# facebookresearch/multipathnet

Hardware: NVIDIA H100
Metric: proposals/sec (higher is better)
Workload: dtype fp32 (wgmma split emulation, fp32 accumulate: 3 bf16 products per MAC, 2 fp16 products in fc6/fc7)

## Files before the change

### include/mpn_abi.h

```cpp
#ifndef MPN_ABI_H
#define MPN_ABI_H
#include <stdint.h>
#ifdef __cplusplus
extern "C" {
#endif

typedef struct mpn_ctx mpn_ctx;
typedef struct mpn_model mpn_model;

int mpn_ctx_create(int device, void *cuda_stream, mpn_ctx **out);
int mpn_ctx_create_stream(int device, int priority, mpn_ctx **out);
void *mpn_ctx_stream(const mpn_ctx *ctx);
int mpn_ctx_wait_ctx(mpn_ctx *ctx, mpn_ctx *other);
void mpn_ctx_destroy(mpn_ctx *ctx);
const char *mpn_last_error(const mpn_ctx *ctx);
int mpn_ctx_synchronize(mpn_ctx *ctx);
int64_t mpn_ctx_launch_count(const mpn_ctx *ctx);
const char *mpn_version(void);
int mpn_ctx_set_option(mpn_ctx *ctx, const char *name, int64_t value);
int mpn_ctx_profile_begin(mpn_ctx *ctx);
int mpn_ctx_profile_end(mpn_ctx *ctx, double *ms_by_cat, int64_t *launches_by_cat);
int mpn_ctx_timeline_begin(mpn_ctx *ctx, int32_t max_launches);
int mpn_ctx_timeline_end(mpn_ctx *ctx, uint64_t *stamps_min, uint64_t *stamps_max, int32_t *n_launches);

int mpn_nms(mpn_ctx *ctx, const float *scored_boxes, int64_t N, float thr,
            int32_t *keep_idx, int64_t *n_keep);
int mpn_nms_batched(mpn_ctx *ctx, const float *scored_boxes, const int64_t *seg_offsets,
                    int64_t nseg, float thr, int32_t *keep_idx, int64_t *keep_counts);
int mpn_nms_batched_dev(mpn_ctx *ctx, const float *scored_boxes_dev, const int64_t *seg_offsets,
                        int64_t nseg, float thr, int32_t *keep_idx_dev, int32_t *keep_counts_dev);
int mpn_nms_dense(mpn_ctx *ctx, const float *scored_boxes, int64_t N, float thr,
                  int32_t *pick_idx, int64_t *n_pick);
int mpn_bbox_vote(mpn_ctx *ctx, const float *nms_boxes, int64_t K, const float *scored_boxes,
                  int64_t N, float thr, float *res);

int mpn_foveal(mpn_ctx *ctx, const float *rois, int64_t R, float *out);
int mpn_context_region(mpn_ctx *ctx, const float *rois, int64_t R, float scale, float *out);
int mpn_bbox_norm(mpn_ctx *ctx, float *deltas, int64_t R, int64_t C4, const float *mean4,
                  const float *std4);
int mpn_foveal_dev(mpn_ctx *ctx, const float *rois_dev, int64_t R, float *out_dev);
int mpn_context_region_dev(mpn_ctx *ctx, const float *rois_dev, int64_t R, float scale, float *out_dev);
int mpn_bbox_norm_dev(mpn_ctx *ctx, float *deltas_dev, int64_t R, int64_t C4, const float *mean4,
                      const float *std4);
int mpn_bbox_decode(mpn_ctx *ctx, const float *deltas, const float *boxes, int64_t R, int64_t C,
                    float *out);

int mpn_roi_pool(mpn_ctx *ctx, const float *fmap, int64_t N, int64_t C, int64_t H, int64_t W,
                 const float *rois, int64_t R, int32_t PW, int32_t PH, float spatial_scale,
                 int32_t variant, float *out, int32_t *argmax);
int mpn_roi_pool_dev(mpn_ctx *ctx, const float *fmap_dev, int64_t N, int64_t C, int64_t H,
                     int64_t W, const float *rois_dev, int64_t R, int32_t PW, int32_t PH,
                     float spatial_scale, int32_t variant, float *out_dev, int32_t *argmax_dev);
int mpn_roi_pool_backward(mpn_ctx *ctx, const float *grad_out, const int32_t *argmax, int64_t N,
                          int64_t C, int64_t H, int64_t W, const float *rois, int64_t R, int32_t PW,
                          int32_t PH, float spatial_scale, int32_t variant, float *grad_data);
int mpn_roi_pool_backward_dev(mpn_ctx *ctx, const float *grad_out_dev, const int32_t *argmax_dev,
                              int64_t N, int64_t C, int64_t H, int64_t W, const float *rois_dev,
                              int64_t R, int32_t PW, int32_t PH, float spatial_scale, int32_t variant,
                              float *grad_data_dev);

enum {
  MPN_LAYER_CONV = 1,
  MPN_LAYER_MAXPOOL = 2,
  MPN_LAYER_AVGPOOL = 3,
  MPN_LAYER_FLATTEN = 4
};
typedef struct mpn_layer {
  int32_t kind;
  int32_t in_slot, out_slot;
  int32_t cin, cout, kh, kw, stride, pad;
  int32_t relu;
  int32_t residual_slot;
  int32_t ceil_mode;
  int32_t weight, bias;
} mpn_layer;

typedef struct mpn_tower {
  int32_t region;
  int32_t n_levels;
  int32_t level_slot[3];
  float   level_scale[3];
  int32_t pooled_w, pooled_h;
  int32_t normalize;
  int32_t n_layers;
  int32_t first_layer;
  int32_t out_slot;
} mpn_tower;

typedef struct mpn_head {
  int32_t col_begin, col_len;
  int32_t cout;
  int32_t weight, bias;
} mpn_head;

typedef struct mpn_model_desc {
  int32_t n_trunk_layers;  const mpn_layer *trunk_layers;
  int32_t n_towers;        const mpn_tower *towers;
  int32_t n_tower_layers;  const mpn_layer *tower_layers;
  int32_t n_cls_heads;     const mpn_head *cls_heads;
  mpn_head bbox_head;
  int32_t num_classes;
  int32_t roi_variant;
  int32_t no_softmax;
  int32_t has_bbox_norm;
  float bbox_mean[4], bbox_std[4];
  int32_t max_rois;
  int32_t max_h, max_w;
} mpn_model_desc;

int mpn_model_create(mpn_ctx *ctx, const mpn_model_desc *desc, const float *const *weights,
                     const int64_t *n_elem, int32_t n_weights, mpn_model **out);
void mpn_model_destroy(mpn_model *m);

int mpn_model_trunk(mpn_model *m, const float *image, int32_t H, int32_t W);
int mpn_model_trunk_dev(mpn_model *m, const float *image_dev, int32_t H, int32_t W);
typedef struct mpn_image_transform {
  int32_t swap[3];
  float scale;
  float mean[3];
  float std[3];
  int32_t has_std;
} mpn_image_transform;
int mpn_get_images_size(int32_t H0, int32_t W0, double scale, double max_size, int32_t *h, int32_t *w, double *im_scale);
int mpn_get_images(mpn_ctx *ctx, const float *im, int32_t H0, int32_t W0, const mpn_image_transform *tf,
                   int32_t h, int32_t w, float *out);
int mpn_get_images_dev(mpn_ctx *ctx, const float *im_dev, int32_t H0, int32_t W0, const mpn_image_transform *tf,
                       int32_t h, int32_t w, float *out_dev);
int mpn_get_images_u8(mpn_ctx *ctx, const uint8_t *im_hwc, int32_t H0, int32_t W0, const mpn_image_transform *tf,
                      int32_t h, int32_t w, float *out);
int mpn_get_images_u8_dev(mpn_ctx *ctx, const uint8_t *im_hwc_dev, int32_t H0, int32_t W0, const mpn_image_transform *tf,
                          int32_t h, int32_t w, float *out_dev);
int mpn_get_images_u8_flip(mpn_ctx *ctx, const uint8_t *im_hwc, int32_t H0, int32_t W0, const mpn_image_transform *tf,
                           int32_t h, int32_t w, int32_t flip, float *out);
int mpn_get_images_u8_flip_dev(mpn_ctx *ctx, const uint8_t *im_hwc_dev, int32_t H0, int32_t W0, const mpn_image_transform *tf,
                               int32_t h, int32_t w, int32_t flip, float *out_dev);
int mpn_model_trunk_image(mpn_model *m, const float *im, int32_t H0, int32_t W0, const mpn_image_transform *tf,
                          double scale, double max_size, double *im_scale, int32_t *h, int32_t *w);
int mpn_model_heads(mpn_model *m, const float *rois, int64_t R, float *cls_out, float *bbox_out);
int mpn_model_heads_dev(mpn_model *m, const float *rois_dev, int64_t R, float *cls_out_dev,
                        float *bbox_out_dev);

int mpn_model_detect(mpn_model *m, const float *image, int32_t H, int32_t W, const float *boxes,
                     int64_t R, float im_scale, int32_t recompute_features, float *scores,
                     float *bboxes);
int mpn_model_detect_nms(mpn_model *m, const float *image, int32_t H, int32_t W,
                         const float *boxes, int64_t R, float im_scale, float W0, float H0,
                         float score_thresh, float nms_thr, float *scores, float *bboxes,
                         int32_t *keep_idx, int32_t *keep_counts);
int mpn_model_detect_nms_submit(mpn_model *m, const float *image, int32_t H, int32_t W,
                                const float *boxes, int64_t R, float im_scale, float W0, float H0,
                                float score_thresh, float nms_thr, float *scores, float *bboxes,
                                int32_t *keep_idx, int32_t *keep_counts, int32_t *ticket);
int mpn_model_detect_nms_submit_u8(mpn_model *m, const uint8_t *im_hwc, int32_t H0, int32_t W0,
                                   const mpn_image_transform *tf, double scale, double max_size, const float *boxes,
                                   int64_t R, float score_thresh, float nms_thr, float *scores, float *bboxes,
                                   int32_t *keep_idx, int32_t *keep_counts, int32_t *ticket);
int mpn_model_detect_nms_wait(mpn_model *m, int32_t ticket);
typedef struct mpn_test_opts {
  int32_t num_iter;
  int32_t use_rbox_scores;
  int32_t bbox_voting;
  float score_thresh;
  float nms_thr;
  float vote_thr;
  float vote_score_pow;
} mpn_test_opts;
int mpn_model_test_one(mpn_model *m, const float *image, int32_t H, int32_t W, const float *boxes, int64_t R,
                       float im_scale, float W0, float H0, const mpn_test_opts *opts, float *scores, float *bboxes,
                       int32_t *keep_idx, int32_t *keep_counts, float *voted);
int mpn_model_detect_nms_dev(mpn_model *m, const float *image_dev, int32_t H, int32_t W,
                             const float *boxes_dev, int64_t R, float im_scale, float W0, float H0,
                             float score_thresh, float nms_thr, float *scores_dev,
                             float *bboxes_dev, int32_t *keep_idx_dev, int32_t *keep_counts_dev);

int mpn_post_detect_dev(mpn_ctx *ctx, const float *scores_dev, const float *deltas_dev, const float *boxes_dev, int64_t R,
                        int32_t C, const float *mean4, const float *std4, float W0, float H0, float score_thresh,
                        float nms_thr, int32_t c_begin, int32_t c_end, float *bboxes_dev, int32_t *keep_idx_dev,
                        int32_t *keep_counts_dev);

enum { MPN_MAX_DET = 128, MPN_REC_FLOATS = 769, MPN_DIST_ID_BYTES = 128 };
int mpn_pack_detections_dev(mpn_ctx *ctx, const float *scores_dev, const float *bboxes_dev, int64_t R, int32_t C,
                            const int32_t *keep_idx_dev, const int32_t *keep_counts_dev, int64_t cap, int32_t top_k,
                            float *record_dev);
int mpn_pack_detections(mpn_ctx *ctx, const float *scores, const float *bboxes, int64_t R, int32_t C,
                        const int32_t *keep_idx, const int32_t *keep_counts, int64_t cap, int32_t top_k, float *record);
int mpn_select_boxes(mpn_ctx *ctx, const float *classes, const float *ys, int64_t R, int32_t C, const float *mean4,
                     const float *std4, float *out);
int mpn_select_boxes_dev(mpn_ctx *ctx, const float *classes_dev, const float *ys_dev, int64_t R, int32_t C,
                         const float *mean4, const float *std4, float *out_dev);
int mpn_model_set_detection_sink(mpn_model *m, float *records_dev, int64_t capacity, int32_t top_k);
int mpn_model_detection_sink_count(const mpn_model *m, int64_t *n_records);

int mpn_dist_unique_id(mpn_ctx *ctx, uint8_t *id);
int mpn_dist_init(mpn_ctx *ctx, const uint8_t *id, int32_t rank, int32_t world);
int mpn_dist_world(const mpn_ctx *ctx, int32_t *rank, int32_t *world);
int mpn_dist_all_gather_dev(mpn_ctx *ctx, const float *send_dev, int64_t n_floats, float *recv_dev);
int mpn_dist_all_gather(mpn_ctx *ctx, const float *send_dev, int64_t n_floats, float *recv_host);
int mpn_dist_destroy(mpn_ctx *ctx);
int mpn_dist_nccl_version(mpn_ctx *ctx, int32_t *version);

int mpn_coco_eval(mpn_ctx *ctx, int32_t n_images, const int64_t *image_ids, int32_t n_cats, const int64_t *cat_ids,
                  int64_t G, const int32_t *gt_img, const int32_t *gt_cat, const double *gt_box, const double *gt_area,
                  const int32_t *gt_crowd, int64_t D, const float *dets, double *precision, double *recall,
                  double *stats);

int mpn_model_get_pooled(mpn_model *m, int32_t tower, int64_t r0, int64_t n, float *out, int64_t capacity,
                         int64_t *R_total, int32_t *bins, int32_t *Ctot);
int mpn_model_get_trunk_slot(mpn_model *m, int32_t slot, float *out_nchw, int64_t capacity,
                             int32_t *C, int32_t *H, int32_t *W);
int mpn_model_get_slot_planes(mpn_model *m, int32_t tower, int32_t slot, int64_t r0, int64_t n, uint16_t *hi,
                              uint16_t *lo, uint8_t *q8, int32_t *e8, int64_t capacity, int32_t *fmt, int64_t *dims);
int mpn_model_get_head_outputs(mpn_model *m, float *cls_logits, float *bbox_raw, int64_t *R, int32_t *K);
int mpn_debug_detect_tail(mpn_ctx *ctx, const float *logits, int32_t K, int64_t R, int32_t C, int32_t do_softmax, const float *deltas,
                          const float *boxes, int32_t do_clamp, float W0, float H0, int32_t has_norm, const float *mean4,
                          const float *std4, float *scores, float *bboxes);
int mpn_model_set_conv_impl(mpn_model *m, int32_t impl);
int mpn_model_last_flops(const mpn_model *m, double *trunk_flops, double *head_flops);

int mpn_gemm_check(mpn_ctx *ctx, const float *A, const float *B, const float *bias, int64_t M,
                   int64_t N, int64_t K, int32_t relu, int32_t impl, float *C);
int mpn_gemm_bench(mpn_ctx *ctx, int64_t M, int64_t N, int64_t K, int32_t iters, double *ms_per_launch,
                   int32_t *bn, int32_t *cta_group, int32_t *splitk);
int mpn_conv_bench(mpn_ctx *ctx, int64_t N, int64_t Cin, int64_t H, int64_t W, int64_t Cout, int32_t k, int32_t stride,
                   int32_t pad, int32_t iters, double *ms_per_launch, int32_t *bn, int32_t *cta_group, int32_t *mode,
                   uint64_t *dbg16);
int mpn_debug_plan(int64_t N, int64_t Cin, int64_t H, int64_t W, int64_t Cout, int32_t k, int32_t stride, int32_t pad,
                   int32_t per_roi, int32_t sm_count, int32_t *out);
int mpn_debug_fp8(const float *h, int64_t n_samples, int64_t sample_elems, int32_t *e_out, uint8_t *q_out);
int mpn_conv_check(mpn_ctx *ctx, const float *x, int64_t N, int64_t Cin, int64_t H, int64_t W,
                   const float *w, const float *bias, int64_t Cout, int32_t kh, int32_t kw,
                   int32_t stride, int32_t pad, int32_t relu, int32_t impl, float *y);

typedef struct mpn_train_config {
  float lr, momentum, dampening, weight_decay;
  float dropout;
  float bbox_regression;
  uint64_t seed;
} mpn_train_config;
int mpn_train_check_fixed_bn(const mpn_model_desc *d, int32_t trunk_from, int32_t integral, int32_t n, const int32_t *weight,
                             char *msg, int32_t msg_cap);
int mpn_model_train_begin_fixed_bn(mpn_model *m, const mpn_train_config *cfg, int32_t trunk_from, int32_t integral, int32_t n,
                                   const int32_t *weight, const float *const *scale);
int mpn_train_check_desc(const mpn_model_desc *d, char *msg, int32_t msg_cap);
int mpn_train_check_trunk(const mpn_model_desc *d, int32_t trunk_from, char *msg, int32_t msg_cap);
int mpn_train_check_integral(const mpn_model_desc *d, int32_t trunk_from, char *msg, int32_t msg_cap);
int mpn_model_train_begin(mpn_model *m, const mpn_train_config *cfg);
int mpn_model_train_begin_trunk(mpn_model *m, const mpn_train_config *cfg, int32_t trunk_from);
int mpn_model_train_begin_integral(mpn_model *m, const mpn_train_config *cfg, int32_t trunk_from);
int mpn_model_train_step(mpn_model *m, int32_t n_images, const float *const *images, const int32_t *image_hw,
                         const int32_t *rois_per_image, const float *boxes, const int32_t *labels, const float *bbox_targets,
                         float *losses);
int mpn_model_train_step_dev(mpn_model *m, int32_t n_images, const float *const *images_dev, const int32_t *image_hw,
                             const int32_t *rois_per_image, const float *boxes_dev, const int32_t *labels_dev,
                             const float *bbox_targets_dev, float *losses_dev);
int mpn_model_train_phase_ms(mpn_model *m, float *ms);
int mpn_model_train_select_head(mpn_model *m, int32_t k);
int mpn_model_train_set_lr(mpn_model *m, float lr);
int mpn_model_train_decay(mpn_model *m, float factor);
int mpn_model_train_get(mpn_model *m, int32_t weight, int32_t what, float *out, int64_t capacity);
int mpn_model_train_dropout_mask(mpn_model *m, int32_t tower, int32_t layer, uint8_t *out, int64_t capacity, int64_t *n_out);
int mpn_model_train_relu_gate(mpn_model *m, int32_t tower, int32_t layer, uint8_t *out, int64_t capacity, int64_t *n_out);
int mpn_model_train_outputs(mpn_model *m, float *cls_logits, float *bbox_deltas);
int mpn_model_train_trunk_slot(mpn_model *m, int32_t image, int32_t slot, float *out_nchw, int64_t capacity, int32_t *C,
                               int32_t *H, int32_t *W);
int mpn_debug_roi_backward_nhwc(mpn_ctx *ctx, const uint16_t *hi, const uint16_t *lo, int32_t H, int32_t W, int32_t C, const float *rois,
                                int64_t R, int32_t PW, int32_t PH, float scale, int32_t variant, const float *grad_out, float *grad);
int mpn_debug_pool_backward(mpn_ctx *ctx, const uint16_t *y_hi, const uint16_t *y_lo, int32_t H, int32_t W, int32_t C, const float *grad_pool,
                            float *grad);
int mpn_debug_conv_backward(mpn_ctx *ctx, int32_t n_images, const int32_t *image_hw, int32_t cin, int32_t cout, int32_t k, int32_t stride,
                            const uint16_t *x_hi, const uint16_t *x_lo, const float *g, const float *w, float *dw, float *dx);
int mpn_model_train_end(mpn_model *m);
int mpn_debug_dropout(uint64_t seed, uint32_t step, int32_t tower, int32_t layer, uint64_t elem0, int64_t n, float p, uint8_t *out);
int mpn_debug_criteria(const float *x, const float *d, const int32_t *labels, const float *t, int64_t R, int32_t C, float bbox_w,
                       float *gx, float *gd, float *losses);
int mpn_debug_sgd(float *w, const float *g, float *buf, int64_t n, float lr, float momentum, float dampening, float wd, int32_t first);

typedef struct mpn_roidb mpn_roidb;
int mpn_roidb_create(mpn_ctx *ctx, int32_t n_images, const int64_t *ann_off, const double *ann_xywh, const double *ann_area,
                     const int32_t *ann_class, const int32_t *ann_flags, double min_area, const int64_t *prop_off,
                     const float *prop_box, const float *prop_score, int32_t best_number, double min_proposal_area,
                     int32_t num_classes, int32_t n_sets, const float *thresholds, mpn_roidb **out);
void mpn_roidb_destroy(mpn_roidb *db);
int mpn_roidb_counts(mpn_roidb *db, int32_t *counts, int64_t *n_rows);
int mpn_roidb_image_rows(mpn_roidb *db, int32_t image, float *boxes, float *overlap, int32_t *corr, int32_t *label, int64_t capacity,
                         int64_t *n_rows, int32_t *n_gt);
int mpn_roidb_list(mpn_roidb *db, int32_t set, int32_t kind, int32_t image, int32_t *rows, int64_t capacity, int64_t *n_out);
int mpn_roidb_regression_stats(mpn_roidb *db, int32_t set, int32_t n_first, float *mean, float *std_);
int mpn_sample_plan(const int32_t *n_bg, const int32_t *n_fg, int32_t n_images, uint64_t seed, uint32_t step, int32_t set, int32_t n_slots,
                    int32_t *image, int32_t *bg_src, int32_t *fg_src, int32_t *flip);
int mpn_integral_set(uint64_t seed, uint32_t step, int32_t n_sets, int32_t *set);
int mpn_train_images_size(int32_t H0, int32_t W0, double scale, double max_size, int32_t *h, int32_t *w, double *im_scale);
int mpn_roidb_sample_dev(mpn_roidb *db, int32_t set, uint64_t seed, uint32_t step, int32_t n_slots, const int32_t *bg_src,
                         const int32_t *fg_src, const int32_t *flip, const double *im_scale, const int32_t *width, int32_t bg_each,
                         int32_t fg_each, const float *mean, const float *std_, int32_t num_classes, float *boxes_dev,
                         int32_t *labels_dev, float *targets_dev, int32_t *rois_per_image);
int mpn_roidb_sample(mpn_roidb *db, int32_t set, uint64_t seed, uint32_t step, int32_t n_slots, const int32_t *plan,
                     const uint8_t *const *images_hwc, const int32_t *hw0, const mpn_image_transform *tf, double scale, double max_size,
                     int32_t bg_each, int32_t fg_each, const float *mean, const float *std_, int32_t num_classes, int32_t *image_hw,
                     int32_t *rois_per_image);
int mpn_roidb_batch_host(mpn_roidb *db, float *const *images, float *boxes, int32_t *labels, float *targets);
int mpn_model_train_step_batch(mpn_model *m, mpn_roidb *db, float *losses);
int mpn_debug_attach_proposals(int64_t n_ann, const double *ann_xywh, const double *ann_area, const int32_t *ann_class,
                               const int32_t *ann_flags, double min_area, int64_t n_prop, const float *prop_box, const float *prop_score,
                               int32_t best_number, double min_proposal_area, int32_t num_classes, float *boxes, float *overlap,
                               int32_t *corr, int32_t *label, int64_t capacity, int64_t *n_rows, int32_t *n_gt);
int mpn_debug_sample_rows(int64_t R, const float *rois, const float *gtboxes, const int32_t *labels, double im_scale, int32_t width,
                          int32_t flip, const float *mean, const float *std_, int32_t num_classes, float *boxes, float *targets);

int mpn_train_check_phase2(const mpn_model_desc *d, int32_t phase2_from, int32_t integral, char *msg, int32_t msg_cap);
int mpn_model_train_begin_phase2(mpn_model *m, const mpn_train_config *cfg, int32_t phase2_from, int32_t integral);
int mpn_model_train_phase2(mpn_model *m, float lr);

typedef struct mpn_train_state {
  int64_t step;
  float lr;
  int32_t head, last_head, phase2;
} mpn_train_state;
int mpn_model_train_set(mpn_model *m, int32_t weight, int32_t what, const float *src, int64_t n);
int mpn_model_train_get_state(mpn_model *m, mpn_train_state *out);
int mpn_model_train_set_state(mpn_model *m, const mpn_train_state *s);
int mpn_debug_roi_backward_jobs(mpn_ctx *ctx, const uint16_t *hi, const uint16_t *lo, int32_t H, int32_t W, int32_t C, const float *rois,
                                int64_t R, int32_t PW, int32_t PH, int32_t variant, int32_t n_jobs, const int32_t *region, const float *scale,
                                const int32_t *normalize, const int64_t *ld, const int32_t *ch_off, const float *const *grad_out, float *grad,
                                double *ab, int32_t *argmax);

#ifdef __cplusplus
}
#endif
#endif
```

### multipathnet_b200/_lib.py

```python
from __future__ import annotations

import ctypes as C
import os
from dataclasses import dataclass, field
from typing import List, Optional, Sequence

import numpy as np

_HERE = os.path.dirname(os.path.abspath(__file__))
LIB_PATH = os.path.join(_HERE, "libmpn_b200.so")
HEADER_PATH = os.path.join(os.path.dirname(_HERE), "include", "mpn_abi.h")

MPN_LAYER_CONV, MPN_LAYER_MAXPOOL, MPN_LAYER_AVGPOOL, MPN_LAYER_FLATTEN = 1, 2, 3, 4
MPN_MAX_DET, MPN_REC_FLOATS, MPN_DIST_ID_BYTES = 128, 769, 128
MPN_LAYER_LRN = 5


class MpnError(RuntimeError):
    pass


class CLayer(C.Structure):
    _fields_ = [(n, C.c_int32) for n in (
        "kind", "in_slot", "out_slot", "cin", "cout", "kh", "kw", "stride", "pad", "relu",
        "residual_slot", "ceil_mode", "weight", "bias")]


class CTower(C.Structure):
    _fields_ = [("region", C.c_int32), ("n_levels", C.c_int32), ("level_slot", C.c_int32 * 3),
                ("level_scale", C.c_float * 3), ("pooled_w", C.c_int32), ("pooled_h", C.c_int32),
                ("normalize", C.c_int32), ("n_layers", C.c_int32), ("first_layer", C.c_int32),
                ("out_slot", C.c_int32)]


class CHead(C.Structure):
    _fields_ = [(n, C.c_int32) for n in ("col_begin", "col_len", "cout", "weight", "bias")]


class CImageTransform(C.Structure):
    _fields_ = [("swap", C.c_int32 * 3), ("scale", C.c_float), ("mean", C.c_float * 3), ("std", C.c_float * 3), ("has_std", C.c_int32)]

    @staticmethod
    def of(kind: str) -> "CImageTransform":
        from . import workloads as wl
        t = CImageTransform()
        if kind == "ross":
            t.swap[:] = [3, 2, 1]; t.scale = 255.0; t.mean[:] = wl.ROSS_MEAN; t.std[:] = [1, 1, 1]; t.has_std = 0
        elif kind == "imagenet":
            t.swap[:] = [1, 2, 3]; t.scale = 1.0; t.mean[:] = wl.IMAGENET_MEAN; t.std[:] = wl.IMAGENET_STD; t.has_std = 1
        else:
            raise ValueError(f"unknown transformer {kind!r}")
        return t


class CTestOpts(C.Structure):
    _fields_ = [("num_iter", C.c_int32), ("use_rbox_scores", C.c_int32), ("bbox_voting", C.c_int32), ("score_thresh", C.c_float),
                ("nms_thr", C.c_float), ("vote_thr", C.c_float), ("vote_score_pow", C.c_float)]


class CModelDesc(C.Structure):
    _fields_ = [("n_trunk_layers", C.c_int32), ("trunk_layers", C.POINTER(CLayer)),
                ("n_towers", C.c_int32), ("towers", C.POINTER(CTower)),
                ("n_tower_layers", C.c_int32), ("tower_layers", C.POINTER(CLayer)),
                ("n_cls_heads", C.c_int32), ("cls_heads", C.POINTER(CHead)),
                ("bbox_head", CHead), ("num_classes", C.c_int32), ("roi_variant", C.c_int32),
                ("no_softmax", C.c_int32), ("has_bbox_norm", C.c_int32),
                ("bbox_mean", C.c_float * 4), ("bbox_std", C.c_float * 4),
                ("max_rois", C.c_int32), ("max_h", C.c_int32), ("max_w", C.c_int32)]


class CTrainConfig(C.Structure):
    _fields_ = [("lr", C.c_float), ("momentum", C.c_float), ("dampening", C.c_float), ("weight_decay", C.c_float),
                ("dropout", C.c_float), ("bbox_regression", C.c_float), ("seed", C.c_uint64)]


class CTrainState(C.Structure):
    _fields_ = [("step", C.c_int64), ("lr", C.c_float), ("head", C.c_int32), ("last_head", C.c_int32), ("phase2", C.c_int32)]


_f32p = C.POINTER(C.c_float)
_i32p = C.POINTER(C.c_int32)
_i64p = C.POINTER(C.c_int64)
_vp = C.c_void_p

SIGNATURES = {
    "mpn_ctx_create": (C.c_int, [C.c_int, _vp, C.POINTER(_vp)]),
    "mpn_ctx_create_stream": (C.c_int, [C.c_int, C.c_int, C.POINTER(_vp)]),
    "mpn_ctx_stream": (_vp, [_vp]),
    "mpn_ctx_wait_ctx": (C.c_int, [_vp, _vp]),
    "mpn_ctx_destroy": (None, [_vp]),
    "mpn_last_error": (C.c_char_p, [_vp]),
    "mpn_ctx_synchronize": (C.c_int, [_vp]),
    "mpn_ctx_launch_count": (C.c_int64, [_vp]),
    "mpn_version": (C.c_char_p, []),
    "mpn_ctx_set_option": (C.c_int, [_vp, C.c_char_p, C.c_int64]),
    "mpn_ctx_profile_begin": (C.c_int, [_vp]),
    "mpn_ctx_profile_end": (C.c_int, [_vp, C.POINTER(C.c_double), _i64p]),
    "mpn_ctx_timeline_begin": (C.c_int, [_vp, C.c_int32]),
    "mpn_ctx_timeline_end": (C.c_int, [_vp, C.POINTER(C.c_uint64), C.POINTER(C.c_uint64), _i32p]),
    "mpn_nms": (C.c_int, [_vp, _vp, C.c_int64, C.c_float, _vp, _i64p]),
    "mpn_nms_batched": (C.c_int, [_vp, _vp, _i64p, C.c_int64, C.c_float, _vp, _i64p]),
    "mpn_nms_batched_dev": (C.c_int, [_vp, _vp, _i64p, C.c_int64, C.c_float, _vp, _vp]),
    "mpn_nms_dense": (C.c_int, [_vp, _vp, C.c_int64, C.c_float, _vp, _i64p]),
    "mpn_bbox_vote": (C.c_int, [_vp, _vp, C.c_int64, _vp, C.c_int64, C.c_float, _vp]),
    "mpn_foveal": (C.c_int, [_vp, _vp, C.c_int64, _vp]),
    "mpn_context_region": (C.c_int, [_vp, _vp, C.c_int64, C.c_float, _vp]),
    "mpn_bbox_norm": (C.c_int, [_vp, _vp, C.c_int64, C.c_int64, _vp, _vp]),
    "mpn_foveal_dev": (C.c_int, [_vp, _vp, C.c_int64, _vp]),
    "mpn_context_region_dev": (C.c_int, [_vp, _vp, C.c_int64, C.c_float, _vp]),
    "mpn_bbox_norm_dev": (C.c_int, [_vp, _vp, C.c_int64, C.c_int64, _vp, _vp]),
    "mpn_bbox_decode": (C.c_int, [_vp, _vp, _vp, C.c_int64, C.c_int64, _vp]),
    "mpn_roi_pool": (C.c_int, [_vp, _vp, C.c_int64, C.c_int64, C.c_int64, C.c_int64, _vp, C.c_int64,
                               C.c_int32, C.c_int32, C.c_float, C.c_int32, _vp, _vp]),
    "mpn_roi_pool_dev": (C.c_int, [_vp, _vp, C.c_int64, C.c_int64, C.c_int64, C.c_int64, _vp, C.c_int64,
                                   C.c_int32, C.c_int32, C.c_float, C.c_int32, _vp, _vp]),
    "mpn_roi_pool_backward": (C.c_int, [_vp, _vp, _vp, C.c_int64, C.c_int64, C.c_int64, C.c_int64, _vp, C.c_int64,
                                        C.c_int32, C.c_int32, C.c_float, C.c_int32, _vp]),
    "mpn_roi_pool_backward_dev": (C.c_int, [_vp, _vp, _vp, C.c_int64, C.c_int64, C.c_int64, C.c_int64, _vp, C.c_int64,
                                            C.c_int32, C.c_int32, C.c_float, C.c_int32, _vp]),
    "mpn_get_images_size": (C.c_int, [C.c_int32, C.c_int32, C.c_double, C.c_double, _i32p, _i32p, C.POINTER(C.c_double)]),
    "mpn_get_images": (C.c_int, [_vp, _vp, C.c_int32, C.c_int32, _vp, C.c_int32, C.c_int32, _vp]),
    "mpn_get_images_dev": (C.c_int, [_vp, _vp, C.c_int32, C.c_int32, _vp, C.c_int32, C.c_int32, _vp]),
    "mpn_get_images_u8": (C.c_int, [_vp, _vp, C.c_int32, C.c_int32, _vp, C.c_int32, C.c_int32, _vp]),
    "mpn_get_images_u8_dev": (C.c_int, [_vp, _vp, C.c_int32, C.c_int32, _vp, C.c_int32, C.c_int32, _vp]),
    "mpn_get_images_u8_flip": (C.c_int, [_vp, _vp, C.c_int32, C.c_int32, _vp, C.c_int32, C.c_int32, C.c_int32, _vp]),
    "mpn_get_images_u8_flip_dev": (C.c_int, [_vp, _vp, C.c_int32, C.c_int32, _vp, C.c_int32, C.c_int32, C.c_int32, _vp]),
    "mpn_roidb_create": (C.c_int, [_vp, C.c_int32, _vp, _vp, _vp, _vp, _vp, C.c_double, _vp, _vp, _vp, C.c_int32, C.c_double,
                                   C.c_int32, C.c_int32, _vp, C.POINTER(_vp)]),
    "mpn_roidb_destroy": (None, [_vp]),
    "mpn_roidb_counts": (C.c_int, [_vp, _vp, _i64p]),
    "mpn_roidb_image_rows": (C.c_int, [_vp, C.c_int32, _vp, _vp, _vp, _vp, C.c_int64, _i64p, _i32p]),
    "mpn_roidb_list": (C.c_int, [_vp, C.c_int32, C.c_int32, C.c_int32, _vp, C.c_int64, _i64p]),
    "mpn_roidb_regression_stats": (C.c_int, [_vp, C.c_int32, C.c_int32, _vp, _vp]),
    "mpn_sample_plan": (C.c_int, [_vp, _vp, C.c_int32, C.c_uint64, C.c_uint32, C.c_int32, C.c_int32, _vp, _vp, _vp, _vp]),
    "mpn_integral_set": (C.c_int, [C.c_uint64, C.c_uint32, C.c_int32, _i32p]),
    "mpn_train_images_size": (C.c_int, [C.c_int32, C.c_int32, C.c_double, C.c_double, _i32p, _i32p, C.POINTER(C.c_double)]),
    "mpn_roidb_sample_dev": (C.c_int, [_vp, C.c_int32, C.c_uint64, C.c_uint32, C.c_int32, _vp, _vp, _vp, _vp, _vp, C.c_int32, C.c_int32,
                                       _vp, _vp, C.c_int32, _vp, _vp, _vp, _vp]),
    "mpn_roidb_sample": (C.c_int, [_vp, C.c_int32, C.c_uint64, C.c_uint32, C.c_int32, _vp, _vp, _vp, _vp, C.c_double, C.c_double,
                                   C.c_int32, C.c_int32, _vp, _vp, C.c_int32, _vp, _vp]),
    "mpn_roidb_batch_host": (C.c_int, [_vp, _vp, _vp, _vp, _vp]),
    "mpn_model_train_step_batch": (C.c_int, [_vp, _vp, _vp]),
    "mpn_debug_attach_proposals": (C.c_int, [C.c_int64, _vp, _vp, _vp, _vp, C.c_double, C.c_int64, _vp, _vp, C.c_int32, C.c_double,
                                             C.c_int32, _vp, _vp, _vp, _vp, C.c_int64, _i64p, _i32p]),
    "mpn_debug_sample_rows": (C.c_int, [C.c_int64, _vp, _vp, _vp, C.c_double, C.c_int32, C.c_int32, _vp, _vp, C.c_int32, _vp, _vp]),
    "mpn_model_detect_nms_submit_u8": (C.c_int, [_vp, _vp, C.c_int32, C.c_int32, _vp, C.c_double, C.c_double, _vp, C.c_int64, C.c_float, C.c_float,
                                                 _vp, _vp, _vp, _vp, _i32p]),
    "mpn_model_trunk_image": (C.c_int, [_vp, _vp, C.c_int32, C.c_int32, _vp, C.c_double, C.c_double, C.POINTER(C.c_double), _i32p, _i32p]),
    "mpn_model_create": (C.c_int, [_vp, C.POINTER(CModelDesc), C.POINTER(_vp), _i64p, C.c_int32, C.POINTER(_vp)]),
    "mpn_model_destroy": (None, [_vp]),
    "mpn_model_trunk": (C.c_int, [_vp, _vp, C.c_int32, C.c_int32]),
    "mpn_model_trunk_dev": (C.c_int, [_vp, _vp, C.c_int32, C.c_int32]),
    "mpn_model_heads": (C.c_int, [_vp, _vp, C.c_int64, _vp, _vp]),
    "mpn_model_heads_dev": (C.c_int, [_vp, _vp, C.c_int64, _vp, _vp]),
    "mpn_model_detect": (C.c_int, [_vp, _vp, C.c_int32, C.c_int32, _vp, C.c_int64, C.c_float, C.c_int32, _vp, _vp]),
    "mpn_model_detect_nms": (C.c_int, [_vp, _vp, C.c_int32, C.c_int32, _vp, C.c_int64, C.c_float, C.c_float,
                                       C.c_float, C.c_float, C.c_float, _vp, _vp, _vp, _vp]),
    "mpn_model_detect_nms_submit": (C.c_int, [_vp, _vp, C.c_int32, C.c_int32, _vp, C.c_int64, C.c_float, C.c_float,
                                              C.c_float, C.c_float, C.c_float, _vp, _vp, _vp, _vp, _i32p]),
    "mpn_model_detect_nms_wait": (C.c_int, [_vp, C.c_int32]),
    "mpn_model_test_one": (C.c_int, [_vp, _vp, C.c_int32, C.c_int32, _vp, C.c_int64, C.c_float, C.c_float, C.c_float, C.POINTER(CTestOpts),
                                     _vp, _vp, _vp, _vp, _vp]),
    "mpn_model_detect_nms_dev": (C.c_int, [_vp, _vp, C.c_int32, C.c_int32, _vp, C.c_int64, C.c_float, C.c_float,
                                           C.c_float, C.c_float, C.c_float, _vp, _vp, _vp, _vp]),
    "mpn_post_detect_dev": (C.c_int, [_vp, _vp, _vp, _vp, C.c_int64, C.c_int32, _vp, _vp, C.c_float, C.c_float, C.c_float, C.c_float,
                                      C.c_int32, C.c_int32, _vp, _vp, _vp]),
    "mpn_pack_detections_dev": (C.c_int, [_vp, _vp, _vp, C.c_int64, C.c_int32, _vp, _vp, C.c_int64, C.c_int32, _vp]),
    "mpn_pack_detections": (C.c_int, [_vp, _vp, _vp, C.c_int64, C.c_int32, _vp, _vp, C.c_int64, C.c_int32, _vp]),
    "mpn_select_boxes": (C.c_int, [_vp, _vp, _vp, C.c_int64, C.c_int32, _vp, _vp, _vp]),
    "mpn_select_boxes_dev": (C.c_int, [_vp, _vp, _vp, C.c_int64, C.c_int32, _vp, _vp, _vp]),
    "mpn_model_set_detection_sink": (C.c_int, [_vp, _vp, C.c_int64, C.c_int32]),
    "mpn_model_detection_sink_count": (C.c_int, [_vp, _i64p]),
    "mpn_dist_unique_id": (C.c_int, [_vp, _vp]),
    "mpn_dist_init": (C.c_int, [_vp, _vp, C.c_int32, C.c_int32]),
    "mpn_dist_world": (C.c_int, [_vp, _i32p, _i32p]),
    "mpn_dist_all_gather_dev": (C.c_int, [_vp, _vp, C.c_int64, _vp]),
    "mpn_dist_all_gather": (C.c_int, [_vp, _vp, C.c_int64, _vp]),
    "mpn_dist_destroy": (C.c_int, [_vp]),
    "mpn_dist_nccl_version": (C.c_int, [_vp, _i32p]),
    "mpn_coco_eval": (C.c_int, [_vp, C.c_int32, _vp, C.c_int32, _vp, C.c_int64, _vp, _vp, _vp, _vp, _vp, C.c_int64, _vp, _vp, _vp, _vp]),
    "mpn_model_get_pooled":(C.c_int, [_vp, C.c_int32, C.c_int64, C.c_int64, _vp, C.c_int64, _i64p, _i32p, _i32p]),
    "mpn_model_get_trunk_slot": (C.c_int, [_vp, C.c_int32, _vp, C.c_int64, _i32p, _i32p, _i32p]),
    "mpn_model_get_slot_planes": (C.c_int, [_vp, C.c_int32, C.c_int32, C.c_int64, C.c_int64, _vp, _vp, _vp, _vp, C.c_int64, _i32p, _i64p]),
    "mpn_model_get_head_outputs": (C.c_int, [_vp, _vp, _vp, _i64p, _i32p]),
    "mpn_debug_detect_tail": (C.c_int, [_vp, _vp, C.c_int32, C.c_int64, C.c_int32, C.c_int32, _vp, _vp, C.c_int32, C.c_float, C.c_float,
                                        C.c_int32, _vp, _vp, _vp, _vp]),
    "mpn_model_set_conv_impl": (C.c_int, [_vp, C.c_int32]),
    "mpn_model_last_flops": (C.c_int, [_vp, C.POINTER(C.c_double), C.POINTER(C.c_double)]),
    "mpn_gemm_bench": (C.c_int, [_vp, C.c_int64, C.c_int64, C.c_int64, C.c_int32, C.POINTER(C.c_double), _i32p, _i32p, _i32p]),
    "mpn_conv_bench": (C.c_int, [_vp, C.c_int64, C.c_int64, C.c_int64, C.c_int64, C.c_int64, C.c_int32, C.c_int32, C.c_int32, C.c_int32,
                                 C.POINTER(C.c_double), _i32p, _i32p, _i32p, C.POINTER(C.c_uint64)]),
    "mpn_debug_plan": (C.c_int, [C.c_int64, C.c_int64, C.c_int64, C.c_int64, C.c_int64, C.c_int32, C.c_int32, C.c_int32, C.c_int32, C.c_int32, _i32p]),
    "mpn_debug_fp8": (C.c_int, [_vp, C.c_int64, C.c_int64, _vp, _vp]),
    "mpn_gemm_check": (C.c_int, [_vp, _vp, _vp, _vp, C.c_int64, C.c_int64, C.c_int64, C.c_int32, C.c_int32, _vp]),
    "mpn_conv_check": (C.c_int, [_vp, _vp, C.c_int64, C.c_int64, C.c_int64, C.c_int64, _vp, _vp, C.c_int64,
                                 C.c_int32, C.c_int32, C.c_int32, C.c_int32, C.c_int32, C.c_int32, _vp]),
    "mpn_train_check_desc": (C.c_int, [C.POINTER(CModelDesc), C.c_char_p, C.c_int32]),
    "mpn_train_check_trunk": (C.c_int, [C.POINTER(CModelDesc), C.c_int32, C.c_char_p, C.c_int32]),
    "mpn_train_check_integral": (C.c_int, [C.POINTER(CModelDesc), C.c_int32, C.c_char_p, C.c_int32]),
    "mpn_model_train_begin": (C.c_int, [_vp, C.POINTER(CTrainConfig)]),
    "mpn_model_train_begin_trunk": (C.c_int, [_vp, C.POINTER(CTrainConfig), C.c_int32]),
    "mpn_model_train_begin_integral": (C.c_int, [_vp, C.POINTER(CTrainConfig), C.c_int32]),
    "mpn_train_check_fixed_bn": (C.c_int, [C.POINTER(CModelDesc), C.c_int32, C.c_int32, C.c_int32, _i32p, C.c_char_p, C.c_int32]),
    "mpn_model_train_begin_fixed_bn": (C.c_int, [_vp, C.POINTER(CTrainConfig), C.c_int32, C.c_int32, C.c_int32, _i32p, C.POINTER(_vp)]),
    "mpn_model_train_step": (C.c_int, [_vp, C.c_int32, C.POINTER(_vp), _i32p, _i32p, _vp, _vp, _vp, _vp]),
    "mpn_model_train_step_dev": (C.c_int, [_vp, C.c_int32, C.POINTER(_vp), _i32p, _i32p, _vp, _vp, _vp, _vp]),
    "mpn_model_train_phase_ms": (C.c_int, [_vp, _f32p]),
    "mpn_model_train_select_head": (C.c_int, [_vp, C.c_int32]),
    "mpn_model_train_set_lr": (C.c_int, [_vp, C.c_float]),
    "mpn_model_train_decay": (C.c_int, [_vp, C.c_float]),
    "mpn_model_train_get": (C.c_int, [_vp, C.c_int32, C.c_int32, _vp, C.c_int64]),
    "mpn_model_train_dropout_mask": (C.c_int, [_vp, C.c_int32, C.c_int32, _vp, C.c_int64, _i64p]),
    "mpn_model_train_relu_gate": (C.c_int, [_vp, C.c_int32, C.c_int32, _vp, C.c_int64, _i64p]),
    "mpn_model_train_outputs": (C.c_int, [_vp, _vp, _vp]),
    "mpn_model_train_trunk_slot": (C.c_int, [_vp, C.c_int32, C.c_int32, _vp, C.c_int64, _i32p, _i32p, _i32p]),
    "mpn_model_train_end": (C.c_int, [_vp]),
    "mpn_debug_roi_backward_nhwc": (C.c_int, [_vp, _vp, _vp, C.c_int32, C.c_int32, C.c_int32, _vp, C.c_int64, C.c_int32, C.c_int32, C.c_float,
                                              C.c_int32, _vp, _vp]),
    "mpn_train_check_phase2": (C.c_int, [C.POINTER(CModelDesc), C.c_int32, C.c_int32, C.c_char_p, C.c_int32]),
    "mpn_model_train_begin_phase2": (C.c_int, [_vp, C.POINTER(CTrainConfig), C.c_int32, C.c_int32]),
    "mpn_model_train_phase2": (C.c_int, [_vp, C.c_float]),
    "mpn_model_train_set": (C.c_int, [_vp, C.c_int32, C.c_int32, _vp, C.c_int64]),
    "mpn_model_train_get_state": (C.c_int, [_vp, C.POINTER(CTrainState)]),
    "mpn_model_train_set_state": (C.c_int, [_vp, C.POINTER(CTrainState)]),
    "mpn_debug_roi_backward_jobs": (C.c_int, [_vp, _vp, _vp, C.c_int32, C.c_int32, C.c_int32, _vp, C.c_int64, C.c_int32, C.c_int32, C.c_int32,
                                              C.c_int32, _i32p, _f32p, _i32p, _i64p, _i32p, C.POINTER(_vp), _vp, _vp, _vp]),
    "mpn_debug_pool_backward": (C.c_int, [_vp, _vp, _vp, C.c_int32, C.c_int32, C.c_int32, _vp, _vp]),
    "mpn_debug_conv_backward": (C.c_int, [_vp, C.c_int32, _i32p, C.c_int32, C.c_int32, C.c_int32, C.c_int32, _vp, _vp, _vp, _vp, _vp,
                                          _vp]),
    "mpn_debug_dropout": (C.c_int, [C.c_uint64, C.c_uint32, C.c_int32, C.c_int32, C.c_uint64, C.c_int64, C.c_float, _vp]),
    "mpn_debug_criteria": (C.c_int, [_vp, _vp, _vp, _vp, C.c_int64, C.c_int32, C.c_float, _vp, _vp, _vp]),
    "mpn_debug_sgd": (C.c_int, [_vp, _vp, _vp, C.c_int64, C.c_float, C.c_float, C.c_float, C.c_float, C.c_int32]),
}

_lib = None


def load_library():
    global _lib
    if _lib is not None:
        return _lib
    if not os.path.exists(LIB_PATH):
        raise MpnError(
            f"{LIB_PATH} is missing: build it with `make` (or `python -c 'import __graft_entry__ as g; g.build()'`). "
            "There is no CPU or PyTorch fallback for this path.")
    lib = C.CDLL(LIB_PATH)
    for name, (res, args) in SIGNATURES.items():
        fn = getattr(lib, name)
        fn.restype = res
        fn.argtypes = args
    _lib = lib
    return lib


def _ptr(a) -> Optional[int]:
    if a is None:
        return None
    if isinstance(a, int):
        return a
    if isinstance(a, np.ndarray):
        return a.ctypes.data
    if hasattr(a, "data_ptr"):
        return a.data_ptr()
    raise TypeError(f"cannot take the address of {type(a)}")


def _f32(a) -> np.ndarray:
    return np.ascontiguousarray(a, dtype=np.float32)


class Context:

    def __init__(self, device: int = 0, stream: Optional[int] = None, own_stream: bool = False, priority: int = 0):
        self.lib = load_library()
        h = _vp()
        if own_stream:
            rc = self.lib.mpn_ctx_create_stream(int(device), int(priority), C.byref(h))
        else:
            rc = self.lib.mpn_ctx_create(int(device), _vp(stream) if stream else None, C.byref(h))
        if rc != 0:
            raise MpnError(f"mpn_ctx_create failed ({rc}): {self.lib.mpn_last_error(None).decode()}")
        self.h = h
        self.device = device
        self._models = []

    def check(self, rc: int, what: str = ""):
        if rc != 0:
            raise MpnError(f"{what} failed ({rc}): {self.lib.mpn_last_error(self.h).decode()}")

    def synchronize(self):
        self.check(self.lib.mpn_ctx_synchronize(self.h), "synchronize")

    @property
    def stream_handle(self) -> int:
        return int(self.lib.mpn_ctx_stream(self.h) or 0)

    def wait_ctx(self, other: "Context"):
        self.check(self.lib.mpn_ctx_wait_ctx(self.h, other.h), "mpn_ctx_wait_ctx")

    def set_option(self, name: str, value: int):
        self.check(self.lib.mpn_ctx_set_option(self.h, name.encode(), int(value)), "mpn_ctx_set_option")

    @property
    def launch_count(self) -> int:
        return int(self.lib.mpn_ctx_launch_count(self.h))

    PROFILE_CATS = ("conv_gemm_tc", "conv_direct", "roi_pool", "nms", "elementwise", "pool", "fp8_quantize")

    def profile_begin(self):
        self.check(self.lib.mpn_ctx_profile_begin(self.h), "profile_begin")

    def profile_end(self):
        ms = (C.c_double * len(self.PROFILE_CATS))()
        n = (C.c_int64 * len(self.PROFILE_CATS))()
        self.check(self.lib.mpn_ctx_profile_end(self.h, ms, n), "profile_end")
        return {k: (ms[i], int(n[i])) for i, k in enumerate(self.PROFILE_CATS)}

    def close(self):
        if getattr(self, "h", None):
            for ref in list(getattr(self, "_models", [])):
                m = ref()
                if m is not None:
                    m.close()
            self._models = []
            self.lib.mpn_ctx_destroy(self.h)
            self.h = None

    def __del__(self):
        try:
            self.close()
        except Exception:
            pass

    def dist_unique_id(self) -> bytes:
        buf = (C.c_uint8 * MPN_DIST_ID_BYTES)()
        self.check(self.lib.mpn_dist_unique_id(self.h, buf), "mpn_dist_unique_id")
        return bytes(buf)

    def dist_init(self, unique_id: bytes, rank: int, world: int):
        assert len(unique_id) == MPN_DIST_ID_BYTES
        buf = (C.c_uint8 * MPN_DIST_ID_BYTES).from_buffer_copy(unique_id)
        self.check(self.lib.mpn_dist_init(self.h, buf, int(rank), int(world)), "mpn_dist_init")

    def dist_world(self):
        r, w = C.c_int32(), C.c_int32()
        self.check(self.lib.mpn_dist_world(self.h, C.byref(r), C.byref(w)), "mpn_dist_world")
        return r.value, w.value

    def dist_all_gather_dev(self, send_dev, n_floats: int, recv_dev):
        self.check(self.lib.mpn_dist_all_gather_dev(self.h, _ptr(send_dev), int(n_floats), _ptr(recv_dev)), "mpn_dist_all_gather_dev")

    def dist_all_gather(self, send_dev, n_floats: int) -> np.ndarray:
        _, w = self.dist_world()
        out = np.empty((w, int(n_floats)), np.float32)
        self.check(self.lib.mpn_dist_all_gather(self.h, _ptr(send_dev), int(n_floats), _ptr(out)), "mpn_dist_all_gather")
        return out

    def dist_destroy(self):
        self.check(self.lib.mpn_dist_destroy(self.h), "mpn_dist_destroy")

    def pack_detections(self, scores, bboxes, keep_idx, keep_counts, top_k: int = 100) -> np.ndarray:
        s, b = _f32(scores), _f32(bboxes)
        k = np.ascontiguousarray(keep_idx, dtype=np.int32); c = np.ascontiguousarray(keep_counts, dtype=np.int32)
        rec = np.empty(MPN_REC_FLOATS, np.float32)
        self.check(self.lib.mpn_pack_detections(self.h, _ptr(s), _ptr(b), s.shape[0], s.shape[1], _ptr(k), _ptr(c), k.shape[1],
                                                int(top_k), _ptr(rec)), "mpn_pack_detections")
        return rec

    def select_boxes(self, classes, ys, mean=None, std=None) -> np.ndarray:
        s, y = _f32(classes), _f32(ys)
        out = np.empty((s.shape[0], 4), np.float32)
        m = None if mean is None else _f32(mean).reshape(4)
        sd = None if std is None else _f32(std).reshape(4)
        self.check(self.lib.mpn_select_boxes(self.h, _ptr(s), _ptr(y), s.shape[0], s.shape[1], _ptr(m), _ptr(sd), _ptr(out)),
                   "mpn_select_boxes")
        return out

    def nms(self, scored_boxes, thr: float) -> np.ndarray:
        sb = _f32(scored_boxes).reshape(-1, 5)
        n = sb.shape[0]
        keep = np.empty(max(n, 1), dtype=np.int32)
        cnt = C.c_int64(0)
        self.check(self.lib.mpn_nms(self.h, _ptr(sb), n, float(thr), _ptr(keep), C.byref(cnt)), "mpn_nms")
        return keep[: cnt.value].copy()

    def nms_batched(self, scored_boxes, seg_offsets: Sequence[int], thr: float) -> List[np.ndarray]:
        sb = _f32(scored_boxes).reshape(-1, 5)
        offs = np.ascontiguousarray(seg_offsets, dtype=np.int64)
        nseg = len(offs) - 1
        keep = np.empty(max(sb.shape[0], 1), dtype=np.int32)
        counts = np.zeros(max(nseg, 1), dtype=np.int64)
        self.check(self.lib.mpn_nms_batched(self.h, _ptr(sb), offs.ctypes.data_as(_i64p), nseg, float(thr), _ptr(keep),
                                            counts.ctypes.data_as(_i64p)), "mpn_nms_batched")
        return [keep[offs[s]: offs[s] + counts[s]].copy() for s in range(nseg)]

    def nms_dense(self, scored_boxes, thr: float) -> np.ndarray:
        sb = _f32(scored_boxes).reshape(-1, 5)
        n = sb.shape[0]
        pick = np.empty(max(n, 1), dtype=np.int32)
        cnt = C.c_int64(0)
        self.check(self.lib.mpn_nms_dense(self.h, _ptr(sb), n, float(thr), _ptr(pick), C.byref(cnt)), "mpn_nms_dense")
        return pick[: cnt.value].copy()

    def bbox_vote(self, nms_boxes, scored_boxes, thr: float) -> np.ndarray:
        nb = _f32(nms_boxes).reshape(-1, 5)
        sb = _f32(scored_boxes).reshape(-1, 5)
        res = np.zeros_like(nb)
        self.check(self.lib.mpn_bbox_vote(self.h, _ptr(nb), nb.shape[0], _ptr(sb), sb.shape[0], float(thr), _ptr(res)),
                   "mpn_bbox_vote")
        return res

    def foveal(self, rois) -> np.ndarray:
        r = _f32(rois)
        out = np.empty((r.shape[0] * 4, 5), dtype=np.float32)
        self.check(self.lib.mpn_foveal(self.h, _ptr(r), r.shape[0], _ptr(out)), "mpn_foveal")
        return out

    def context_region(self, rois, scale: float) -> np.ndarray:
        r = _f32(rois)
        out = np.empty_like(r)
        self.check(self.lib.mpn_context_region(self.h, _ptr(r), r.shape[0], float(scale), _ptr(out)), "mpn_context_region")
        return out

    def foveal_dev(self, rois_dev, R: int, out_dev):
        self.check(self.lib.mpn_foveal_dev(self.h, _ptr(rois_dev), int(R), _ptr(out_dev)), "mpn_foveal_dev")

    def context_region_dev(self, rois_dev, R: int, scale: float, out_dev):
        self.check(self.lib.mpn_context_region_dev(self.h, _ptr(rois_dev), int(R), float(scale), _ptr(out_dev)), "mpn_context_region_dev")

    def bbox_norm_dev(self, deltas_dev, R: int, C4: int, mean, std):
        m, s = _f32(mean).reshape(4), _f32(std).reshape(4)
        self.check(self.lib.mpn_bbox_norm_dev(self.h, _ptr(deltas_dev), int(R), int(C4), _ptr(m), _ptr(s)), "mpn_bbox_norm_dev")

    def get_images(self, im, kind: str, scale: float = 600, max_size: float = 1000):
        im = _f32(im)
        if im.ndim != 3 or im.shape[0] != 3:
            raise ValueError("ImageTransformer expects a 3 x H x W image")
        h, w, s = C.c_int32(), C.c_int32(), C.c_double()
        self.check(self.lib.mpn_get_images_size(im.shape[1], im.shape[2], float(scale), float(max_size), C.byref(h), C.byref(w), C.byref(s)),
                   "mpn_get_images_size")
        out = np.empty((3, h.value, w.value), np.float32)
        tf = CImageTransform.of(kind)
        self.check(self.lib.mpn_get_images(self.h, _ptr(im), im.shape[1], im.shape[2], C.addressof(tf), h.value, w.value, _ptr(out)),
                   "mpn_get_images")
        return out, float(s.value)

    def get_images_u8(self, im_hwc_u8, kind: str, scale: float = 600, max_size: float = 1000):
        im = np.ascontiguousarray(im_hwc_u8, dtype=np.uint8)
        if im.ndim != 3 or im.shape[2] != 3:
            raise ValueError("expected an H x W x 3 uint8 image")
        h, w, s = C.c_int32(), C.c_int32(), C.c_double()
        self.check(self.lib.mpn_get_images_size(im.shape[0], im.shape[1], float(scale), float(max_size), C.byref(h), C.byref(w), C.byref(s)),
                   "mpn_get_images_size")
        out = np.empty((3, h.value, w.value), np.float32)
        tf = CImageTransform.of(kind)
        self.check(self.lib.mpn_get_images_u8(self.h, _ptr(im), im.shape[0], im.shape[1], C.addressof(tf), h.value, w.value, _ptr(out)),
                   "mpn_get_images_u8")
        return out, float(s.value)

    def bbox_norm(self, deltas, mean, std) -> np.ndarray:
        d = _f32(deltas).copy()
        m, s = _f32(mean).reshape(4), _f32(std).reshape(4)
        self.check(self.lib.mpn_bbox_norm(self.h, _ptr(d), d.shape[0], d.shape[1], _ptr(m), _ptr(s)), "mpn_bbox_norm")
        return d

    def bbox_decode(self, deltas, boxes) -> np.ndarray:
        d, b = _f32(deltas), _f32(boxes)
        out = np.empty_like(d)
        self.check(self.lib.mpn_bbox_decode(self.h, _ptr(d), _ptr(b), d.shape[0], d.shape[1] // 4, _ptr(out)), "mpn_bbox_decode")
        return out

    def roi_pool(self, fmap, rois, pw: int, ph: int, scale: float, variant: int = 2, with_argmax: bool = False):
        f, r = _f32(fmap), _f32(rois)
        n, c, h, w = f.shape
        out = np.empty((r.shape[0], c, ph, pw), dtype=np.float32)
        am = np.empty(out.shape, dtype=np.int32) if with_argmax else None
        self.check(self.lib.mpn_roi_pool(self.h, _ptr(f), n, c, h, w, _ptr(r), r.shape[0], pw, ph, float(scale), variant,
                                         _ptr(out), _ptr(am)), "mpn_roi_pool")
        return (out, am) if with_argmax else out

    def roi_pool_backward(self, grad_out, argmax, rois, data_shape, pw: int, ph: int, scale: float, variant: int = 2) -> np.ndarray:
        g, r = _f32(grad_out), _f32(rois)
        am = np.ascontiguousarray(argmax, dtype=np.int32)
        n, c, h, w = (int(s) for s in data_shape)
        if g.shape != (r.shape[0], c, ph, pw) or am.shape != g.shape:
            raise ValueError(f"grad_out and argmax must be {(r.shape[0], c, ph, pw)}, got {g.shape} and {am.shape}")
        out = np.empty((n, c, h, w), dtype=np.float32)
        self.check(self.lib.mpn_roi_pool_backward(self.h, _ptr(g), _ptr(am), n, c, h, w, _ptr(r), r.shape[0], pw, ph, float(scale),
                                                  variant, _ptr(out)), "mpn_roi_pool_backward")
        return out

    def roi_pool_backward_dev(self, grad_out_dev, argmax_dev, N: int, C_: int, H: int, W: int, rois_dev, R: int, pw: int, ph: int,
                              scale: float, variant: int, grad_data_dev):
        self.check(self.lib.mpn_roi_pool_backward_dev(self.h, _ptr(grad_out_dev), _ptr(argmax_dev), int(N), int(C_), int(H), int(W),
                                                      _ptr(rois_dev), int(R), int(pw), int(ph), float(scale), int(variant),
# ... 336 lines not shown
```

### multipathnet_b200/csrc/abi.cu

```cuda
#include "conv_gemm.cuh"
#include "roi.cuh"
#include <algorithm>
#include <mutex>

int mpn_nms_launch(mpn_ctx *, const float *, int, int, const int32_t *, const int32_t *, float, int32_t *, int32_t *);
int mpn_nms_dense_launch(mpn_ctx *, const float *, int, float, int32_t *, int32_t *);
int mpn_bbox_vote_launch(mpn_ctx *, const float *, int, const float *, int, float, float *);
int mpn_pack_detections_launch(mpn_ctx *, const float *, const float *, int, const int32_t *, const int32_t *, int, int, float *);
int mpn_gather_scored_range_launch(mpn_ctx *, const float *, const float *, int, int, int, int, float, float *, int32_t *, int32_t *);
int mpn_bbox_norm_decode_launch(mpn_ctx *, const float *, const float *, int64_t, int, int, float, float, float *, const float *, const float *);
int mpn_detect_tail_launch(mpn_ctx *, const float *, int64_t, int, int, int, float *, const float *, const float *, int, float, float,
                           float *, int, const float *, const float *);
int mpn_select_boxes_launch(mpn_ctx *, const float *, const float *, int64_t, int, const float *, const float *, float *);
int mpn_foveal_launch(mpn_ctx *, const float *, int64_t, float *);
int mpn_context_region_launch(mpn_ctx *, const float *, int64_t, float, float *);
int mpn_get_images_launch(mpn_ctx *, const float *, int32_t, int32_t, const mpn_image_transform *, int32_t, int32_t, float *);
int mpn_get_images_size_impl(int32_t, int32_t, double, double, int32_t *, int32_t *, double *);
int mpn_get_images_u8_launch(mpn_ctx *, const uint8_t *, int32_t, int32_t, const mpn_image_transform *, int32_t, int32_t, float *);
int mpn_get_images_u8_flip_launch(mpn_ctx *, const uint8_t *, int32_t, int32_t, const mpn_image_transform *, int32_t, int32_t, int32_t, float *);
int mpn_bbox_norm_launch(mpn_ctx *, float *, int64_t, int64_t, const float *, const float *);
int mpn_bbox_decode_launch(mpn_ctx *, const float *, const float *, int64_t, int, int, float, float, float *);
int mpn_split_rows_launch(mpn_ctx *, const float *, int64_t, int64_t, int64_t, __nv_bfloat16 *, __nv_bfloat16 *, int64_t);
int mpn_nchw_to_nhwc_split_launch(mpn_ctx *, const float *, int, int, int, int, DTensor &);
int mpn_nhwc_split_to_nchw_launch(mpn_ctx *, const DTensor &, float *);
// ... 386 lines not shown
  Arena a{ctx};
  const size_t bs = sizeof(float) * (size_t)R * C, bb = sizeof(float) * (size_t)R * 4 * C, bk = sizeof(int32_t) * (size_t)(C - 1) * cap,
               bc = sizeof(int32_t) * (size_t)(C - 1), br = sizeof(float) * MPN_REC_FLOATS;
  size_t o_s = a.reserve(bs), o_b = a.reserve(bb), o_k = a.reserve(bk), o_c = a.reserve(bc), o_r = a.reserve(br);
  MPN_TRY(a.commit());
  MPN_CUDA(ctx, cudaMemcpyAsync(a.at<float>(o_s), scores, bs, cudaMemcpyHostToDevice, ctx->stream));
  MPN_CUDA(ctx, cudaMemcpyAsync(a.at<float>(o_b), bboxes, bb, cudaMemcpyHostToDevice, ctx->stream));
  MPN_CUDA(ctx, cudaMemcpyAsync(a.at<int32_t>(o_k), keep_idx, bk, cudaMemcpyHostToDevice, ctx->stream));
  MPN_CUDA(ctx, cudaMemcpyAsync(a.at<int32_t>(o_c), keep_counts, bc, cudaMemcpyHostToDevice, ctx->stream));
  MPN_TRY(mpn_pack_detections_launch(ctx, a.at<float>(o_s), a.at<float>(o_b), C, a.at<int32_t>(o_k), a.at<int32_t>(o_c), (int)cap, top_k,
                                     a.at<float>(o_r)));
  MPN_CUDA(ctx, cudaMemcpyAsync(record, a.at<float>(o_r), br, cudaMemcpyDeviceToHost, ctx->stream));
  MPN_CUDA(ctx, cudaStreamSynchronize(ctx->stream));
  return MPN_OK;
}

int mpn_select_boxes_dev(mpn_ctx *ctx, const float *classes_dev, const float *ys_dev, int64_t R, int32_t C, const float *mean4,
                         const float *std4, float *out_dev) {
  if (!ctx) return MPN_ERR_ARG;
  MPN_CUDA(ctx, cudaSetDevice(ctx->device));
  MPN_CHECK_ARG(ctx, R >= 0 && C >= 1 && (R == 0 || (classes_dev && ys_dev && out_dev)), "buffers missing");
  MPN_CHECK_ARG(ctx, (mean4 == nullptr) == (std4 == nullptr), "mean4 and std4 go together");
  return mpn_select_boxes_launch(ctx, classes_dev, ys_dev, R, C, mean4, std4, out_dev);
}

int mpn_select_boxes(mpn_ctx *ctx, const float *classes, const float *ys, int64_t R, int32_t C, const float *mean4, const float *std4,
                     float *out) {
  if (!ctx) return MPN_ERR_ARG;
  MPN_CUDA(ctx, cudaSetDevice(ctx->device));
  MPN_CHECK_ARG(ctx, R >= 0 && C >= 1, "bad arguments");
  if (R == 0) return MPN_OK;
  MPN_CHECK_ARG(ctx, classes && ys && out, "buffers missing");
  Arena a{ctx};
  const size_t bs = sizeof(float) * (size_t)R * C, bb = sizeof(float) * (size_t)R * 4 * C, bo = sizeof(float) * (size_t)R * 4;
  size_t o_s = a.reserve(bs), o_b = a.reserve(bb), o_o = a.reserve(bo);
  MPN_TRY(a.commit());
  MPN_CUDA(ctx, cudaMemcpyAsync(a.at<float>(o_s), classes, bs, cudaMemcpyHostToDevice, ctx->stream));
  MPN_CUDA(ctx, cudaMemcpyAsync(a.at<float>(o_b), ys, bb, cudaMemcpyHostToDevice, ctx->stream));
  MPN_TRY(mpn_select_boxes_dev(ctx, a.at<float>(o_s), a.at<float>(o_b), R, C, mean4, std4, a.at<float>(o_o)));
  MPN_CUDA(ctx, cudaMemcpyAsync(out, a.at<float>(o_o), bo, cudaMemcpyDeviceToHost, ctx->stream));
  MPN_CUDA(ctx, cudaStreamSynchronize(ctx->stream));
  return MPN_OK;
}

static int unary_rois(mpn_ctx *ctx, const float *in, int64_t R, int64_t out_rows_per_in, float *out,
                      int (*launch)(mpn_ctx *, const float *, int64_t, float, float *), float param) {
  if (!ctx) return MPN_ERR_ARG;
  MPN_CUDA(ctx, cudaSetDevice(ctx->device));
  MPN_CHECK_ARG(ctx, R >= 0, "bad R");
  if (R == 0) return MPN_OK;
  MPN_CHECK_ARG(ctx, in && out, "buffers missing");
  Arena a{ctx};
  size_t o_i = a.reserve(sizeof(float) * 5 * (size_t)R), o_o = a.reserve(sizeof(float) * 5 * (size_t)(R * out_rows_per_in));
  MPN_TRY(a.commit());
  MPN_CUDA(ctx, cudaMemcpyAsync(a.at<float>(o_i), in, sizeof(float) * 5 * (size_t)R, cudaMemcpyHostToDevice, ctx->stream));
  MPN_TRY(launch(ctx, a.at<float>(o_i), R, param, a.at<float>(o_o)));
  MPN_CUDA(ctx, cudaMemcpyAsync(out, a.at<float>(o_o), sizeof(float) * 5 * (size_t)(R * out_rows_per_in), cudaMemcpyDeviceToHost, ctx->stream));
  MPN_CUDA(ctx, cudaStreamSynchronize(ctx->stream));
  return MPN_OK;
}
static int foveal_adapter(mpn_ctx *c, const float *i, int64_t R, float, float *o) { return mpn_foveal_launch(c, i, R, o); }

int mpn_foveal(mpn_ctx *ctx, const float *rois, int64_t R, float *out) { return unary_rois(ctx, rois, R, 4, out, foveal_adapter, 0.f); }
int mpn_context_region(mpn_ctx *ctx, const float *rois, int64_t R, float scale, float *out) {
  return unary_rois(ctx, rois, R, 1, out, mpn_context_region_launch, scale);
}

int mpn_foveal_dev(mpn_ctx *ctx, const float *rois_dev, int64_t R, float *out_dev) {
  if (!ctx) return MPN_ERR_ARG;
  MPN_CUDA(ctx, cudaSetDevice(ctx->device));
  MPN_CHECK_ARG(ctx, R >= 0, "bad R");
  if (R == 0) return MPN_OK;
  MPN_CHECK_ARG(ctx, rois_dev && out_dev, "buffers missing");
  return mpn_foveal_launch(ctx, rois_dev, R, out_dev);
}
int mpn_context_region_dev(mpn_ctx *ctx, const float *rois_dev, int64_t R, float scale, float *out_dev) {
  if (!ctx) return MPN_ERR_ARG;
  MPN_CUDA(ctx, cudaSetDevice(ctx->device));
  MPN_CHECK_ARG(ctx, R >= 0, "bad R");
  if (R == 0) return MPN_OK;
  MPN_CHECK_ARG(ctx, rois_dev && out_dev, "buffers missing");
  return mpn_context_region_launch(ctx, rois_dev, R, scale, out_dev);
}
int mpn_bbox_norm_dev(mpn_ctx *ctx, float *deltas_dev, int64_t R, int64_t C4, const float *mean4, const float *std4) {
  if (!ctx) return MPN_ERR_ARG;
  MPN_CUDA(ctx, cudaSetDevice(ctx->device));
  MPN_CHECK_ARG(ctx, R >= 0 && C4 > 0 && C4 % 4 == 0, "BBoxNorm: input:size(2) % 4 == 0 required (BBoxNorm.lua:19)");
  if (R == 0) return MPN_OK;
  MPN_CHECK_ARG(ctx, deltas_dev && mean4 && std4, "buffers missing");
  return mpn_bbox_norm_launch(ctx, deltas_dev, R, C4, mean4, std4);
}

int mpn_get_images_size(int32_t H0, int32_t W0, double scale, double max_size, int32_t *h, int32_t *w, double *im_scale) {
  return mpn_get_images_size_impl(H0, W0, scale, max_size, h, w, im_scale);
}
int mpn_get_images_dev(mpn_ctx *ctx, const float *im_dev, int32_t H0, int32_t W0, const mpn_image_transform *tf,
                       int32_t h, int32_t w, float *out_dev) {
  if (!ctx) return MPN_ERR_ARG;
  MPN_CUDA(ctx, cudaSetDevice(ctx->device));
  return mpn_get_images_launch(ctx, im_dev, H0, W0, tf, h, w, out_dev);
}
int mpn_get_images_u8_dev(mpn_ctx *ctx, const uint8_t *im_hwc_dev, int32_t H0, int32_t W0, const mpn_image_transform *tf,
                          int32_t h, int32_t w, float *out_dev) {
  if (!ctx) return MPN_ERR_ARG;
  MPN_CUDA(ctx, cudaSetDevice(ctx->device));
  return mpn_get_images_u8_launch(ctx, im_hwc_dev, H0, W0, tf, h, w, out_dev);
}
int mpn_get_images_u8(mpn_ctx *ctx, const uint8_t *im_hwc, int32_t H0, int32_t W0, const mpn_image_transform *tf,
                      int32_t h, int32_t w, float *out) {
  return mpn_get_images_u8_flip(ctx, im_hwc, H0, W0, tf, h, w, 0, out);
}
int mpn_get_images_u8_flip_dev(mpn_ctx *ctx, const uint8_t *im_hwc_dev, int32_t H0, int32_t W0, const mpn_image_transform *tf,
                               int32_t h, int32_t w, int32_t flip, float *out_dev) {
  if (!ctx) return MPN_ERR_ARG;
  MPN_CUDA(ctx, cudaSetDevice(ctx->device));
  return mpn_get_images_u8_flip_launch(ctx, im_hwc_dev, H0, W0, tf, h, w, flip, out_dev);
}
int mpn_get_images_u8_flip(mpn_ctx *ctx, const uint8_t *im_hwc, int32_t H0, int32_t W0, const mpn_image_transform *tf,
                           int32_t h, int32_t w, int32_t flip, float *out) {
  if (!ctx) return MPN_ERR_ARG;
  MPN_CUDA(ctx, cudaSetDevice(ctx->device));
  MPN_CHECK_ARG(ctx, im_hwc && out && tf && H0 > 0 && W0 > 0 && h > 0 && w > 0, "getImages: buffers missing or bad sizes");
  Arena a{ctx};
  const size_t bi = (size_t)H0 * W0 * 3, bo = sizeof(float) * 3 * (size_t)h * w;
  size_t o_i = a.reserve(bi), o_o = a.reserve(bo);
  MPN_TRY(a.commit());
  MPN_CUDA(ctx, cudaMemcpyAsync(a.at<uint8_t>(o_i), im_hwc, bi, cudaMemcpyHostToDevice, ctx->stream));
  MPN_TRY(mpn_get_images_u8_flip_launch(ctx, a.at<uint8_t>(o_i), H0, W0, tf, h, w, flip, a.at<float>(o_o)));
  MPN_CUDA(ctx, cudaMemcpyAsync(out, a.at<float>(o_o), bo, cudaMemcpyDeviceToHost, ctx->stream));
  MPN_CUDA(ctx, cudaStreamSynchronize(ctx->stream));
  return MPN_OK;
}
int mpn_get_images(mpn_ctx *ctx, const float *im, int32_t H0, int32_t W0, const mpn_image_transform *tf,
                   int32_t h, int32_t w, float *out) {
  if (!ctx) return MPN_ERR_ARG;
  MPN_CUDA(ctx, cudaSetDevice(ctx->device));
  MPN_CHECK_ARG(ctx, im && out && tf && H0 > 0 && W0 > 0 && h > 0 && w > 0, "getImages: buffers missing or bad sizes");
  Arena a{ctx};
  const size_t bi = sizeof(float) * 3 * (size_t)H0 * W0, bo = sizeof(float) * 3 * (size_t)h * w;
  size_t o_i = a.reserve(bi), o_o = a.reserve(bo);
  MPN_TRY(a.commit());
  MPN_CUDA(ctx, cudaMemcpyAsync(a.at<float>(o_i), im, bi, cudaMemcpyHostToDevice, ctx->stream));
  MPN_TRY(mpn_get_images_launch(ctx, a.at<float>(o_i), H0, W0, tf, h, w, a.at<float>(o_o)));
  MPN_CUDA(ctx, cudaMemcpyAsync(out, a.at<float>(o_o), bo, cudaMemcpyDeviceToHost, ctx->stream));
  MPN_CUDA(ctx, cudaStreamSynchronize(ctx->stream));
  return MPN_OK;
}

int mpn_bbox_norm(mpn_ctx *ctx, float *deltas, int64_t R, int64_t C4, const float *mean4, const float *std4) {
  if (!ctx) return MPN_ERR_ARG;
  MPN_CUDA(ctx, cudaSetDevice(ctx->device));
  MPN_CHECK_ARG(ctx, R >= 0 && C4 > 0 && C4 % 4 == 0, "BBoxNorm: input:size(2) % 4 == 0 required (BBoxNorm.lua:19)");
  if (R == 0) return MPN_OK;
  MPN_CHECK_ARG(ctx, deltas && mean4 && std4, "buffers missing");
  Arena a{ctx};
  size_t o = a.reserve(sizeof(float) * (size_t)(R * C4));
  MPN_TRY(a.commit());
  MPN_CUDA(ctx, cudaMemcpyAsync(a.at<float>(o), deltas, sizeof(float) * (size_t)(R * C4), cudaMemcpyHostToDevice, ctx->stream));
  MPN_TRY(mpn_bbox_norm_launch(ctx, a.at<float>(o), R, C4, mean4, std4));
  MPN_CUDA(ctx, cudaMemcpyAsync(deltas, a.at<float>(o), sizeof(float) * (size_t)(R * C4), cudaMemcpyDeviceToHost, ctx->stream));
  MPN_CUDA(ctx, cudaStreamSynchronize(ctx->stream));
  return MPN_OK;
}

int mpn_bbox_decode(mpn_ctx *ctx, const float *deltas, const float *boxes, int64_t R, int64_t C, float *out) {
  if (!ctx) return MPN_ERR_ARG;
  MPN_CUDA(ctx, cudaSetDevice(ctx->device));
  MPN_CHECK_ARG(ctx, R >= 0 && C > 0, "bad arguments");
  if (R == 0) return MPN_OK;
  MPN_CHECK_ARG(ctx, deltas && boxes && out, "buffers missing");
  Arena a{ctx};
  size_t o_d = a.reserve(sizeof(float) * 4 * (size_t)(R * C)), o_b = a.reserve(sizeof(float) * 4 * (size_t)R),
         o_o = a.reserve(sizeof(float) * 4 * (size_t)(R * C));
  MPN_TRY(a.commit());
  MPN_CUDA(ctx, cudaMemcpyAsync(a.at<float>(o_d), deltas, sizeof(float) * 4 * (size_t)(R * C), cudaMemcpyHostToDevice, ctx->stream));
  MPN_CUDA(ctx, cudaMemcpyAsync(a.at<float>(o_b), boxes, sizeof(float) * 4 * (size_t)R, cudaMemcpyHostToDevice, ctx->stream));
  MPN_TRY(mpn_bbox_decode_launch(ctx, a.at<float>(o_d), a.at<float>(o_b), R, (int)C, 0, 0.f, 0.f, a.at<float>(o_o)));
  MPN_CUDA(ctx, cudaMemcpyAsync(out, a.at<float>(o_o), sizeof(float) * 4 * (size_t)(R * C), cudaMemcpyDeviceToHost, ctx->stream));
  MPN_CUDA(ctx, cudaStreamSynchronize(ctx->stream));
  return MPN_OK;
}

int mpn_roi_pool_dev(mpn_ctx *ctx, const float *fmap_dev, int64_t N, int64_t C, int64_t H, int64_t W,
                     const float *rois_dev, int64_t R, int32_t PW, int32_t PH, float spatial_scale, int32_t variant,
                     float *out_dev, int32_t *argmax_dev) {
  if (!ctx) return MPN_ERR_ARG;
  MPN_CUDA(ctx, cudaSetDevice(ctx->device));
  MPN_CHECK_ARG(ctx, N > 0 && C > 0 && H > 0 && W > 0 && R >= 0 && PW > 0 && PH > 0, "bad geometry");
  MPN_CHECK_ARG(ctx, variant == 1 || variant == 2, "variant must be 1 or 2");
  return mpn_roi_pool_nchw_launch(ctx, fmap_dev, N, C, H, W, rois_dev, R, PW, PH, spatial_scale, variant, out_dev, argmax_dev);
}

int mpn_roi_pool(mpn_ctx *ctx, const float *fmap, int64_t N, int64_t C, int64_t H, int64_t W, const float *rois,
                 int64_t R, int32_t PW, int32_t PH, float spatial_scale, int32_t variant, float *out, int32_t *argmax) {
  if (!ctx) return MPN_ERR_ARG;
  MPN_CUDA(ctx, cudaSetDevice(ctx->device));
  MPN_CHECK_ARG(ctx, N > 0 && C > 0 && H > 0 && W > 0 && R >= 0 && PW > 0 && PH > 0, "bad geometry");
  if (R == 0) return MPN_OK;
  MPN_CHECK_ARG(ctx, fmap && rois && out, "buffers missing");
  for (int64_t r = 0; r < R; ++r) {
    const float b = rois[5 * r];
    MPN_CHECK_ARG(ctx, b >= 1.f && b <= (float)N, "ROI batch index out of range (1-based, ImageDetect.lua:69)");
  }
  const size_t nf = (size_t)(N * C * H * W), no = (size_t)(R * C * PH * PW);
  Arena a{ctx};
  size_t o_f = a.reserve(sizeof(float) * nf), o_r = a.reserve(sizeof(float) * 5 * (size_t)R), o_o = a.reserve(sizeof(float) * no),
         o_a = a.reserve(sizeof(int32_t) * no);
  MPN_TRY(a.commit());
  MPN_CUDA(ctx, cudaMemcpyAsync(a.at<float>(o_f), fmap, sizeof(float) * nf, cudaMemcpyHostToDevice, ctx->stream));
  MPN_CUDA(ctx, cudaMemcpyAsync(a.at<float>(o_r), rois, sizeof(float) * 5 * (size_t)R, cudaMemcpyHostToDevice, ctx->stream));
  MPN_TRY(mpn_roi_pool_dev(ctx, a.at<float>(o_f), N, C, H, W, a.at<float>(o_r), R, PW, PH, spatial_scale, variant,
                           a.at<float>(o_o), argmax ? a.at<int32_t>(o_a) : nullptr));
  MPN_CUDA(ctx, cudaMemcpyAsync(out, a.at<float>(o_o), sizeof(float) * no, cudaMemcpyDeviceToHost, ctx->stream));
  if (argmax) MPN_CUDA(ctx, cudaMemcpyAsync(argmax, a.at<int32_t>(o_a), sizeof(int32_t) * no, cudaMemcpyDeviceToHost, ctx->stream));
  MPN_CUDA(ctx, cudaStreamSynchronize(ctx->stream));
  return MPN_OK;
}

int mpn_roi_pool_backward_dev(mpn_ctx *ctx, const float *grad_out_dev, const int32_t *argmax_dev, int64_t N, int64_t C,
                              int64_t H, int64_t W, const float *rois_dev, int64_t R, int32_t PW, int32_t PH,
                              float spatial_scale, int32_t variant, float *grad_data_dev) {
  if (!ctx) return MPN_ERR_ARG;
  MPN_CUDA(ctx, cudaSetDevice(ctx->device));
  MPN_CHECK_ARG(ctx, N > 0 && C > 0 && H > 0 && W > 0 && R >= 0 && PW > 0 && PH > 0, "bad geometry");
  MPN_CHECK_ARG(ctx, variant == 1 || variant == 2, "variant must be 1 or 2");
  MPN_CHECK_ARG(ctx, grad_data_dev && (R == 0 || (grad_out_dev && argmax_dev && rois_dev)), "buffers missing");
  return mpn_roi_pool_backward_nchw_launch(ctx, grad_out_dev, argmax_dev, N, C, H, W, rois_dev, R, PW, PH, spatial_scale,
                                           variant, grad_data_dev);
}

int mpn_roi_pool_backward(mpn_ctx *ctx, const float *grad_out, const int32_t *argmax, int64_t N, int64_t C, int64_t H,
                          int64_t W, const float *rois, int64_t R, int32_t PW, int32_t PH, float spatial_scale,
                          int32_t variant, float *grad_data) {
  if (!ctx) return MPN_ERR_ARG;
  MPN_CUDA(ctx, cudaSetDevice(ctx->device));
  MPN_CHECK_ARG(ctx, N > 0 && C > 0 && H > 0 && W > 0 && R >= 0 && PW > 0 && PH > 0, "bad geometry");
  MPN_CHECK_ARG(ctx, variant == 1 || variant == 2, "variant must be 1 or 2");
  MPN_CHECK_ARG(ctx, grad_data && (R == 0 || (grad_out && argmax && rois)), "buffers missing");
  for (int64_t r = 0; r < R; ++r) {
    const float b = rois[5 * r];
    MPN_CHECK_ARG(ctx, b >= 1.f && b <= (float)N, "ROI batch index out of range (1-based, ImageDetect.lua:69)");
  }
  const size_t nd = (size_t)(N * C * H * W), ng = (size_t)(R * C * PH * PW);
  Arena a{ctx};
  size_t o_g = a.reserve(sizeof(float) * ng), o_a = a.reserve(sizeof(int32_t) * ng), o_r = a.reserve(sizeof(float) * 5 * (size_t)R),
         o_d = a.reserve(sizeof(float) * nd);
  MPN_TRY(a.commit());
  if (R > 0) {
    MPN_CUDA(ctx, cudaMemcpyAsync(a.at<float>(o_g), grad_out, sizeof(float) * ng, cudaMemcpyHostToDevice, ctx->stream));
    MPN_CUDA(ctx, cudaMemcpyAsync(a.at<int32_t>(o_a), argmax, sizeof(int32_t) * ng, cudaMemcpyHostToDevice, ctx->stream));
    MPN_CUDA(ctx, cudaMemcpyAsync(a.at<float>(o_r), rois, sizeof(float) * 5 * (size_t)R, cudaMemcpyHostToDevice, ctx->stream));
  }
  MPN_TRY(mpn_roi_pool_backward_dev(ctx, a.at<float>(o_g), a.at<int32_t>(o_a), N, C, H, W, a.at<float>(o_r), R, PW, PH,
                                    spatial_scale, variant, a.at<float>(o_d)));
  MPN_CUDA(ctx, cudaMemcpyAsync(grad_data, a.at<float>(o_d), sizeof(float) * nd, cudaMemcpyDeviceToHost, ctx->stream));
  MPN_CUDA(ctx, cudaStreamSynchronize(ctx->stream));
  return MPN_OK;
}

int mpn_conv_check(mpn_ctx *ctx, const float *x, int64_t N, int64_t Cin, int64_t H, int64_t W, const float *w,
                   const float *bias, int64_t Cout, int32_t kh, int32_t kw, int32_t stride, int32_t pad, int32_t relu,
                   int32_t impl, float *y) {
  if (!ctx) return MPN_ERR_ARG;
  MPN_CUDA(ctx, cudaSetDevice(ctx->device));
  MPN_CHECK_ARG(ctx, x && w && y && N > 0 && Cin > 0 && Cout > 0 && H > 0 && W > 0, "bad arguments");
  const int64_t Ho = (H + 2 * pad - kh) / stride + 1, Wo = (W + 2 * pad - kw) / stride + 1;
  MPN_CHECK_ARG(ctx, Ho > 0 && Wo > 0, "empty output");
  MPN_CHECK_ARG(ctx, !(ctx->opt_fp8 == 1 && ctx->opt_bf16 == 1), "the \"fp8\" and \"bf16\" options are both on");
  const size_t nx = (size_t)(N * Cin * H * W), nw = (size_t)(Cout * Cin * kh * kw), ny = (size_t)(N * Cout * Ho * Wo);
  Arena a{ctx};
  size_t o_x = a.reserve(4 * nx), o_w = a.reserve(4 * nw), o_b = a.reserve(4 * (size_t)Cout), o_y = a.reserve(4 * ny),
         o_xh = a.reserve(2 * nx), o_xl = a.reserve(2 * nx), o_wh = a.reserve(2 * nw), o_wl = a.reserve(2 * nw),
         o_yh = a.reserve(2 * ny), o_yl = a.reserve(2 * ny),
         o_x8 = a.reserve(nx), o_xe = a.reserve(4 * (size_t)N), o_w8 = a.reserve(nw), o_we = a.reserve(4 * (size_t)(Cout + 127) / 128 * 128);
  MPN_TRY(a.commit());
  MPN_CUDA(ctx, cudaMemcpyAsync(a.at<float>(o_x), x, 4 * nx, cudaMemcpyHostToDevice, ctx->stream));
  MPN_CUDA(ctx, cudaMemcpyAsync(a.at<float>(o_w), w, 4 * nw, cudaMemcpyHostToDevice, ctx->stream));
  if (bias) MPN_CUDA(ctx, cudaMemcpyAsync(a.at<float>(o_b), bias, 4 * (size_t)Cout, cudaMemcpyHostToDevice, ctx->stream));
  DTensor ty; ty.hi = a.at<__nv_bfloat16>(o_yh); ty.lo = a.at<__nv_bfloat16>(o_yl); ty.N = N; ty.H = Ho; ty.W = Wo; ty.C = Cout; ty.ld = Cout;
  if (impl == 2) {
    MPN_TRY(conv_direct_nchw_launch(ctx, a.at<float>(o_x), (int)N, (int)Cin, (int)H, (int)W, a.at<float>(o_w),
                                    bias ? a.at<float>(o_b) : nullptr, (int)Cout, kh, kw, stride, pad, relu, ty, w, bias));
  } else {
    DTensor tx; tx.hi = a.at<__nv_bfloat16>(o_xh); tx.lo = a.at<__nv_bfloat16>(o_xl); tx.N = N; tx.H = H; tx.W = W; tx.C = Cin; tx.ld = Cin;
    MPN_TRY(mpn_nchw_to_nhwc_split_launch(ctx, a.at<float>(o_x), (int)N, (int)Cin, (int)H, (int)W, tx));
    MPN_TRY(mpn_weight_permute_split_launch(ctx, a.at<float>(o_w), Cout, (int)Cin, kh, kw, a.at<__nv_bfloat16>(o_wh), a.at<__nv_bfloat16>(o_wl)));
    ConvProblem p; p.x = tx; p.w_hi = a.at<__nv_bfloat16>(o_wh); p.w_lo = a.at<__nv_bfloat16>(o_wl);
    p.bias = bias ? a.at<float>(o_b) : nullptr; p.Cout = (int)Cout; p.kh = kh; p.kw = kw; p.stride = stride; p.pad = pad; p.relu = relu;
    p.y = ty; p.bf16 = ctx->opt_bf16 == 1 ? 1 : 0;
    if (ctx->opt_fp8 == 1) {
      p.fp8 = 1;
      p.x8 = a.at<uint8_t>(o_x8); p.x8_exp = a.at<int>(o_xe); p.w8 = a.at<uint8_t>(o_w8); p.w8_exp = a.at<int>(o_we);
      MPN_TRY(mpn_fp8_quantize_launch(ctx, tx, a.at<uint8_t>(o_x8), a.at<int>(o_xe)));
      MPN_TRY(mpn_fp8_weight_launch(ctx, p.w_hi, Cout, (int64_t)Cin * kh * kw, (Cout + 127) / 128 * 128, a.at<uint8_t>(o_w8), a.at<int>(o_we)));
    }
    if (impl == 1) { MPN_TRY(conv_ref_launch(ctx, p)); }
    else { ConvPlan pl; MPN_TRY(conv_tc_plan(ctx, p, pl)); MPN_TRY(conv_tc_launch(ctx, p, pl)); }
  }
  MPN_TRY(mpn_nhwc_split_to_nchw_launch(ctx, ty, a.at<float>(o_y)));
  MPN_CUDA(ctx, cudaMemcpyAsync(y, a.at<float>(o_y), 4 * ny, cudaMemcpyDeviceToHost, ctx->stream));
  if (ctx->opt_fp8 == 1) MPN_TRY(mpn_ovf_copy_async(ctx, ctx->stream));
  MPN_CUDA(ctx, cudaStreamSynchronize(ctx->stream));
  return ctx->opt_fp8 == 1 ? mpn_ovf_test(ctx) : MPN_OK;
}

int mpn_gemm_bench(mpn_ctx *ctx, int64_t M, int64_t N, int64_t K, int32_t iters, double *ms_per_launch, int32_t *bn,
                   int32_t *cta_group, int32_t *splitk) {
  if (!ctx) return MPN_ERR_ARG;
  MPN_CUDA(ctx, cudaSetDevice(ctx->device));
  MPN_CHECK_ARG(ctx, M > 0 && N > 0 && K > 0 && K % 64 == 0 && iters > 0 && ms_per_launch, "bad arguments");
  const size_t na = (size_t)(M * K), nb = (size_t)(N * K), nc = (size_t)(M * N);
  Arena a{ctx};
  size_t o_ah = a.reserve(2 * na), o_al = a.reserve(2 * na), o_bh = a.reserve(2 * nb), o_bl = a.reserve(2 * nb),
         o_ch = a.reserve(2 * nc + 64), o_cl = a.reserve(2 * nc + 64);
  MPN_TRY(a.commit());
  MPN_CUDA(ctx, cudaMemsetAsync(a.at<char>(o_ah), 0x3c, 2 * na, ctx->stream));
  MPN_CUDA(ctx, cudaMemsetAsync(a.at<char>(o_al), 0x30, 2 * na, ctx->stream));
  MPN_CUDA(ctx, cudaMemsetAsync(a.at<char>(o_bh), 0x3c, 2 * nb, ctx->stream));
  MPN_CUDA(ctx, cudaMemsetAsync(a.at<char>(o_bl), 0x30, 2 * nb, ctx->stream));
  ConvProblem p;
  p.x.hi = a.at<__nv_bfloat16>(o_ah); p.x.lo = a.at<__nv_bfloat16>(o_al); p.x.N = M; p.x.H = 1; p.x.W = 1; p.x.C = K; p.x.ld = K;
  p.w_hi = a.at<__nv_bfloat16>(o_bh); p.w_lo = a.at<__nv_bfloat16>(o_bl); p.Cout = (int)N; p.relu = 1;
  p.bf16 = ctx->opt_bf16 == 1 ? 1 : 0;
  const int64_t Npad = (N + 7) / 8 * 8;
  (void)Npad;
  if (N % 8 == 0) { p.y.hi = a.at<__nv_bfloat16>(o_ch); p.y.lo = a.at<__nv_bfloat16>(o_cl); }
  else { p.y.f32 = a.at<float>(o_ch); }
  p.y.N = M; p.y.H = 1; p.y.W = 1; p.y.C = N; p.y.ld = N; p.y_f32_ld = N;
  if (!(N % 8 == 0)) MPN_CHECK_ARG(ctx, 4 * nc <= 2 * (2 * nc + 64), "internal");
  ConvPlan pl;
  MPN_TRY(conv_tc_plan(ctx, p, pl));
  if (bn) *bn = pl.BN; if (cta_group) *cta_group = 1; if (splitk) *splitk = pl.splitk;
  for (int i = 0; i < 3; ++i) MPN_TRY(conv_tc_launch(ctx, p, pl));
  cudaEvent_t e0, e1;
  MPN_CUDA(ctx, cudaEventCreate(&e0)); MPN_CUDA(ctx, cudaEventCreate(&e1));
  MPN_CUDA(ctx, cudaEventRecord(e0, ctx->stream));
  for (int i = 0; i < iters; ++i) MPN_TRY(conv_tc_launch(ctx, p, pl));
  MPN_CUDA(ctx, cudaEventRecord(e1, ctx->stream));
  MPN_CUDA(ctx, cudaEventSynchronize(e1));
  float ms = 0.f;
  MPN_CUDA(ctx, cudaEventElapsedTime(&ms, e0, e1));
  cudaEventDestroy(e0); cudaEventDestroy(e1);
  *ms_per_launch = (double)ms / iters;
  return MPN_OK;
}

int mpn_conv_bench(mpn_ctx *ctx, int64_t N, int64_t Cin, int64_t H, int64_t W, int64_t Cout, int32_t k, int32_t stride,
                   int32_t pad, int32_t iters, double *ms_per_launch, int32_t *bn, int32_t *cta_group, int32_t *mode,
                   uint64_t *dbg16) {
  if (!ctx) return MPN_ERR_ARG;
  MPN_CUDA(ctx, cudaSetDevice(ctx->device));
  MPN_CHECK_ARG(ctx, N > 0 && Cin % 64 == 0 && Cout % 8 == 0 && iters > 0 && ms_per_launch, "bad arguments");
  const int64_t Ho = (H + 2 * pad - k) / stride + 1, Wo = (W + 2 * pad - k) / stride + 1;
  const size_t nx = (size_t)(N * H * W * Cin), nw = (size_t)(Cout * Cin * k * k), ny = (size_t)(N * Ho * Wo * Cout);
  Arena a{ctx};
  size_t o_xh = a.reserve(2 * nx), o_xl = a.reserve(2 * nx), o_wh = a.reserve(2 * nw), o_wl = a.reserve(2 * nw),
         o_yh = a.reserve(2 * ny), o_yl = a.reserve(2 * ny);
  MPN_TRY(a.commit());
  MPN_CUDA(ctx, cudaMemsetAsync(a.at<char>(o_xh), 0x3c, 2 * nx, ctx->stream));
  MPN_CUDA(ctx, cudaMemsetAsync(a.at<char>(o_xl), 0x30, 2 * nx, ctx->stream));
  MPN_CUDA(ctx, cudaMemsetAsync(a.at<char>(o_wh), 0x3c, 2 * nw, ctx->stream));
  MPN_CUDA(ctx, cudaMemsetAsync(a.at<char>(o_wl), 0x30, 2 * nw, ctx->stream));
  ConvProblem p;
  p.x.hi = a.at<__nv_bfloat16>(o_xh); p.x.lo = a.at<__nv_bfloat16>(o_xl); p.x.N = N; p.x.H = H; p.x.W = W; p.x.C = Cin; p.x.ld = Cin;
  p.w_hi = a.at<__nv_bfloat16>(o_wh); p.w_lo = a.at<__nv_bfloat16>(o_wl); p.Cout = (int)Cout; p.kh = k; p.kw = k; p.stride = stride; p.pad = pad; p.relu = 1;
  p.bf16 = ctx->opt_bf16 == 1 ? 1 : 0;
  p.y.hi = a.at<__nv_bfloat16>(o_yh); p.y.lo = a.at<__nv_bfloat16>(o_yl); p.y.N = N; p.y.H = Ho; p.y.W = Wo; p.y.C = Cout; p.y.ld = Cout;
  ConvPlan pl;
  MPN_TRY(conv_tc_plan(ctx, p, pl));
  if (bn) *bn = pl.BN; if (cta_group) *cta_group = 1; if (mode) *mode = pl.mode;
  for (int i = 0; i < 3; ++i) MPN_TRY(conv_tc_launch(ctx, p, pl));
  cudaEvent_t e0, e1;
  MPN_CUDA(ctx, cudaEventCreate(&e0)); MPN_CUDA(ctx, cudaEventCreate(&e1));
  MPN_CUDA(ctx, cudaEventRecord(e0, ctx->stream));
  for (int i = 0; i < iters; ++i) MPN_TRY(conv_tc_launch(ctx, p, pl));
  MPN_CUDA(ctx, cudaEventRecord(e1, ctx->stream));
  MPN_CUDA(ctx, cudaEventSynchronize(e1));
  float ms = 0.f;
  MPN_CUDA(ctx, cudaEventElapsedTime(&ms, e0, e1));
  cudaEventDestroy(e0); cudaEventDestroy(e1);
  *ms_per_launch = (double)ms / iters;
  if (dbg16) memset(dbg16, 0, 128);
  return MPN_OK;
}

int mpn_gemm_check(mpn_ctx *ctx, const float *A, const float *B, const float *bias, int64_t M, int64_t N, int64_t K,
                   int32_t relu, int32_t impl, float *C) {
  if (!ctx) return MPN_ERR_ARG;
  MPN_CUDA(ctx, cudaSetDevice(ctx->device));
  MPN_CHECK_ARG(ctx, A && B && C && M > 0 && N > 0 && K > 0, "bad arguments");
  MPN_CHECK_ARG(ctx, !(ctx->opt_fp8 == 1 && ctx->opt_bf16 == 1), "the \"fp8\" and \"bf16\" options are both on");
  const size_t na = (size_t)(M * K), nb = (size_t)(N * K), nc = (size_t)(M * N);
  Arena a{ctx};
  size_t o_a = a.reserve(4 * na), o_b = a.reserve(4 * nb), o_bias = a.reserve(4 * (size_t)N), o_c = a.reserve(4 * nc),
         o_ah = a.reserve(2 * na), o_al = a.reserve(2 * na), o_bh = a.reserve(2 * nb), o_bl = a.reserve(2 * nb),
         o_a8 = a.reserve(na), o_ae = a.reserve(4 * (size_t)M), o_b8 = a.reserve(nb), o_be = a.reserve(4 * (size_t)(N + 127) / 128 * 128);
  MPN_TRY(a.commit());
  MPN_CUDA(ctx, cudaMemcpyAsync(a.at<float>(o_a), A, 4 * na, cudaMemcpyHostToDevice, ctx->stream));
  MPN_CUDA(ctx, cudaMemcpyAsync(a.at<float>(o_b), B, 4 * nb, cudaMemcpyHostToDevice, ctx->stream));
  if (bias) MPN_CUDA(ctx, cudaMemcpyAsync(a.at<float>(o_bias), bias, 4 * (size_t)N, cudaMemcpyHostToDevice, ctx->stream));
  MPN_TRY(mpn_split_rows_launch(ctx, a.at<float>(o_a), M, K, K, a.at<__nv_bfloat16>(o_ah), a.at<__nv_bfloat16>(o_al), K));
  MPN_TRY(mpn_split_rows_launch(ctx, a.at<float>(o_b), N, K, K, a.at<__nv_bfloat16>(o_bh), a.at<__nv_bfloat16>(o_bl), K));
  ConvProblem p;
  p.x.hi = a.at<__nv_bfloat16>(o_ah); p.x.lo = a.at<__nv_bfloat16>(o_al); p.x.N = M; p.x.H = 1; p.x.W = 1; p.x.C = K; p.x.ld = K;
  p.w_hi = a.at<__nv_bfloat16>(o_bh); p.w_lo = a.at<__nv_bfloat16>(o_bl); p.bias = bias ? a.at<float>(o_bias) : nullptr;
  p.Cout = (int)N; p.relu = relu; p.bf16 = ctx->opt_bf16 == 1 ? 1 : 0;
  p.m_invariant = 1;
  p.y.f32 = a.at<float>(o_c); p.y.N = M; p.y.H = 1; p.y.W = 1; p.y.C = N; p.y.ld = N; p.y_f32_ld = N;
  if (ctx->opt_fp8 == 1 && impl != 2) {
    p.fp8 = 1;
    p.x8 = a.at<uint8_t>(o_a8); p.x8_exp = a.at<int>(o_ae); p.w8 = a.at<uint8_t>(o_b8); p.w8_exp = a.at<int>(o_be);
    MPN_TRY(mpn_fp8_quantize_launch(ctx, p.x, a.at<uint8_t>(o_a8), a.at<int>(o_ae)));
    MPN_TRY(mpn_fp8_weight_launch(ctx, p.w_hi, N, K, (N + 127) / 128 * 128, a.at<uint8_t>(o_b8), a.at<int>(o_be)));
  }
  if (impl == 1) { MPN_TRY(conv_ref_launch(ctx, p)); }
  else {
    if (impl == 2) {
      float amax = 0.f;
      MPN_TRY(mpn_absmax(ctx, a.at<float>(o_b), (int64_t)nb, &amax));
      int e = 0;
      if (amax > 0.f) { (void)frexpf(amax, &e); e = 14 - e; }
      const float sc = ldexpf(1.0f, e);
      MPN_TRY(mpn_weight_permute_half_launch(ctx, a.at<float>(o_b), N, (int)K, 1, 1, sc, a.at<void>(o_bh)));
      p.w16 = a.at<void>(o_bh); p.w16_inv_scale = 1.0f / sc; p.w_hi = p.w_lo = nullptr;
      MPN_TRY(mpn_split_rows_f16_launch(ctx, a.at<float>(o_a), M, K, K, a.at<__nv_bfloat16>(o_ah), a.at<__nv_bfloat16>(o_al), K));
      p.x.fmt = 1; p.bf16 = 0;
    }
    ConvPlan pl; MPN_TRY(conv_tc_plan(ctx, p, pl)); MPN_TRY(conv_tc_launch(ctx, p, pl));
  }
  MPN_CUDA(ctx, cudaMemcpyAsync(C, a.at<float>(o_c), 4 * nc, cudaMemcpyDeviceToHost, ctx->stream));
  if (ctx->opt_fp8 == 1) MPN_TRY(mpn_ovf_copy_async(ctx, ctx->stream));
  MPN_CUDA(ctx, cudaStreamSynchronize(ctx->stream));
  return ctx->opt_fp8 == 1 ? mpn_ovf_test(ctx) : MPN_OK;
}

}
```

### multipathnet_b200/csrc/common.cuh

```cuda
#pragma once
#include <utility>
#include <stdlib.h>
#include <cuda_runtime.h>
#include <cuda_bf16.h>
#include <cuda_fp16.h>
#include <stdint.h>
#include <stdio.h>
#include <string.h>
#include <string>
#include <vector>
#include "../../include/mpn_abi.h"

struct mpn_ctx {
  int device = 0;
  cudaStream_t stream = nullptr;
  int sm_count = 132;
  std::string err;
  int64_t launches = 0;
  void *scratch = nullptr; size_t scratch_bytes = 0;
  void *scratch2 = nullptr; size_t scratch2_bytes = 0;
  void *scratch3 = nullptr; size_t scratch3_bytes = 0;
  void *scratch4 = nullptr; size_t scratch4_bytes = 0;
  void *small_dev = nullptr;
  int profiling = 0;
  struct ProfRec { int cat; cudaEvent_t a, b; };
  std::vector<ProfRec> prof;
  std::vector<cudaEvent_t> ev_pool;
  uint8_t tc_attr_set[32] = {0};
  void *nms_tie_ptr = nullptr; int nms_tie_n = 0;
  unsigned long long *tl_min = nullptr, *tl_max = nullptr; int tl_cap = 0, tl_n = 0, tl_on = 0;
  int opt_fc_w16 = -1;
  int opt_bf16 = -1;
  int opt_fp8 = -1;
  unsigned *ovf_dev = nullptr; unsigned *ovf_host = nullptr;
  void *dist_comm = nullptr; int dist_rank = 0, dist_world = 1; int64_t collectives = 0;
  int own_stream = 0;
  cudaEvent_t join_ev = nullptr;
  float *u8_lut_dev = nullptr;
};

enum { MPN_CAT_CONV_TC = 0, MPN_CAT_CONV_DIRECT = 1, MPN_CAT_ROI = 2, MPN_CAT_NMS = 3, MPN_CAT_ELTWISE = 4, MPN_CAT_POOL = 5,
       MPN_CAT_FP8_QUANT = 6, MPN_NCAT = 7 };

struct MpnProfScope {
  mpn_ctx *ctx; int idx = -1;
  MpnProfScope(mpn_ctx *c, int cat) : ctx(c) {
    if (!c->profiling) return;
    auto get = [&]() { cudaEvent_t e; if (c->ev_pool.empty()) cudaEventCreate(&e); else { e = c->ev_pool.back(); c->ev_pool.pop_back(); } return e; };
    mpn_ctx::ProfRec r{cat, get(), get()};
    cudaEventRecord(r.a, c->stream);
    c->prof.push_back(r); idx = (int)c->prof.size() - 1;
  }
  ~MpnProfScope() { if (idx >= 0) cudaEventRecord(ctx->prof[idx].b, ctx->stream); }
};

#define MPN_OK 0
#define MPN_ERR_ARG (-1)
#define MPN_ERR_CUDA (-2)
#define MPN_ERR_STATE (-3)

inline int mpn_fail(mpn_ctx *ctx, int code, const std::string &msg) {
  if (ctx) ctx->err = msg;
  return code;
}

#define MPN_CUDA(ctx, expr)                                                         \
  do {                                                                              \
    cudaError_t e__ = (expr);                                                       \
    if (e__ != cudaSuccess) {                                                       \
      char b__[512];                                                                \
      snprintf(b__, sizeof b__, "CUDA error %s at %s:%d: %s", cudaGetErrorName(e__), \
               __FILE__, __LINE__, cudaGetErrorString(e__));                        \
      cudaGetLastError();                                                           \
      return mpn_fail((ctx), MPN_ERR_CUDA, b__);                                    \
    }                                                                               \
  } while (0)

#define MPN_CHECK_ARG(ctx, cond, msg)                                   \
  do {                                                                  \
    if (!(cond)) return mpn_fail((ctx), MPN_ERR_ARG, std::string(msg)); \
  } while (0)

#define MPN_TRY(expr)           \
  do {                          \
    int r__ = (expr);           \
    if (r__ != MPN_OK) return r__; \
  } while (0)

#define MPN_LAUNCHED(ctx)                 \
  do {                                    \
    (ctx)->launches++;                    \
    MPN_CUDA((ctx), cudaGetLastError());  \
  } while (0)

#define MPN_PDL_SYNC()                                                  \
  do {                                                                  \
    asm volatile("griddepcontrol.wait;" ::: "memory");                  \
    asm volatile("griddepcontrol.launch_dependents;" ::: "memory");     \
  } while (0)
inline bool mpn_pdl_enabled() {
  static const int on = [] { const char *e = getenv("MPN_TC_PDL"); return (e && e[0] == '0') ? 0 : 1; }();
  return on != 0;
}
template <typename... KArgs, typename... Args>
inline cudaError_t mpn_launch_pdl(mpn_ctx *ctx, void (*kern)(KArgs...), dim3 grid, dim3 block, size_t smem, Args &&...args) {
  cudaLaunchConfig_t cfg = {};
  cfg.gridDim = grid; cfg.blockDim = block; cfg.dynamicSmemBytes = smem; cfg.stream = ctx->stream;
  cudaLaunchAttribute at[1];
  at[0].id = cudaLaunchAttributeProgrammaticStreamSerialization;
  at[0].val.programmaticStreamSerializationAllowed = 1;
  cfg.attrs = at; cfg.numAttrs = mpn_pdl_enabled() ? 1 : 0;
  return cudaLaunchKernelEx(&cfg, kern, std::forward<Args>(args)...);
}

int mpn_ovf_flag(mpn_ctx *ctx, unsigned **flag_dev);
int mpn_ovf_copy_async(mpn_ctx *ctx, cudaStream_t stream);
int mpn_ovf_test(mpn_ctx *ctx);
int mpn_scratch(mpn_ctx *ctx, size_t bytes, void **out);
int mpn_scratch2(mpn_ctx *ctx, size_t bytes, void **out);
int mpn_scratch3(mpn_ctx *ctx, size_t bytes, void **out);
int mpn_scratch4(mpn_ctx *ctx, size_t bytes, void **out);

static inline int64_t ceil_div64(int64_t a, int64_t b) { return (a + b - 1) / b; }

__device__ __forceinline__ void split_bf16(float x, __nv_bfloat16 &hi, __nv_bfloat16 &lo) {
  hi = __float2bfloat16_rn(x);
  lo = __float2bfloat16_rn(x - __bfloat162float(hi));
}
__device__ __forceinline__ void split_bf16x2(float x0, float x1, uint32_t &hi2, uint32_t &lo2) {
  const __nv_bfloat162 h = __floats2bfloat162_rn(x0, x1);
  hi2 = *reinterpret_cast<const uint32_t *>(&h);
  const float r0 = x0 - __uint_as_float(hi2 << 16), r1 = x1 - __uint_as_float(hi2 & 0xffff0000u);
  const __nv_bfloat162 l = __floats2bfloat162_rn(r0, r1);
  lo2 = *reinterpret_cast<const uint32_t *>(&l);
}
__device__ __forceinline__ void split_f16x2(float x0, float x1, uint32_t &hi2, uint32_t &lo2, unsigned *ovf) {
  const float c0 = fminf(fmaxf(x0, -65504.f), 65504.f), c1 = fminf(fmaxf(x1, -65504.f), 65504.f);
  if (ovf && (c0 != x0 || c1 != x1)) atomicOr(ovf, 1u);
  const __half2 h = __floats2half2_rn(c0, c1);
  hi2 = *reinterpret_cast<const uint32_t *>(&h);
  const float2 hf = __half22float2(h);
  const __half2 l = __floats2half2_rn(c0 - hf.x, c1 - hf.y);
  lo2 = *reinterpret_cast<const uint32_t *>(&l);
}
__device__ __forceinline__ void split_x2(int fmt, float x0, float x1, uint32_t &hi2, uint32_t &lo2, unsigned *ovf) {
  if (fmt) split_f16x2(x0, x1, hi2, lo2, ovf);
  else split_bf16x2(x0, x1, hi2, lo2);
}
__device__ __forceinline__ float join_planes(int fmt, uint16_t hi, uint16_t lo) {
  if (fmt) return __half2float(__ushort_as_half(hi)) + __half2float(__ushort_as_half(lo));
  return __uint_as_float((uint32_t)hi << 16) + __uint_as_float((uint32_t)lo << 16);
}
__device__ __forceinline__ float join_bf16(__nv_bfloat16 hi, __nv_bfloat16 lo) {
  return __bfloat162float(hi) + __bfloat162float(lo);
}
__device__ __forceinline__ float bf16_bits_to_float(uint32_t b16) { return __uint_as_float(b16 << 16); }
__device__ __forceinline__ float2 bf16x2_to_float2(uint32_t v) {
  return make_float2(__uint_as_float(v << 16), __uint_as_float(v & 0xffff0000u));
}
__device__ __forceinline__ uint32_t pack_bf16x2(__nv_bfloat16 a, __nv_bfloat16 b) {
  return (uint32_t)__bfloat16_as_ushort(a) | ((uint32_t)__bfloat16_as_ushort(b) << 16);
}

struct DTensor {
  __nv_bfloat16 *hi = nullptr, *lo = nullptr;
  int fmt = 0;
  float *f32 = nullptr;
  int64_t N = 0, H = 0, W = 0, C = 0, ld = 0;
  int64_t pixels() const { return N * H * W; }
};
```

### multipathnet_b200/csrc/conv_gemm.cuh

```cuda
#pragma once
#include "common.cuh"
#include <cuda.h>

struct OutSeg { int c0, c1; float *ptr; long long ld; };
struct OutScatter { int n = 0; OutSeg seg[8]; };

enum class OperandScheme : int { BF16X3 = 0, FP16X2 = 1, BF16X1 = 2, FP8X1 = 3 };

struct ConvProblem {
  DTensor x;
  const __nv_bfloat16 *w_hi = nullptr, *w_lo = nullptr;
  const float *bias = nullptr;
  int Cout = 0, kh = 1, kw = 1, stride = 1, pad = 0;
  int relu = 0;
  DTensor res;
  DTensor y;
  int64_t y_f32_ld = 0;
  DTensor pool;
  int pool_only = 0;
  int m_invariant = 0;
  const void *w16 = nullptr; float w16_inv_scale = 1.f;
  int bf16 = 0;
  int fp8 = 0;
  const uint8_t *x8 = nullptr; const int *x8_exp = nullptr;
  const uint8_t *w8 = nullptr; const int *w8_exp = nullptr;
  OutScatter scatter;
  int wide_k_split = 0;
};

struct ConvPlan {
  CUtensorMap tmA_hi, tmA_lo, tmB_hi, tmB_lo;
  int BN = 0;
  int tn = 0, th = 0, tw = 0;
  int tiles_img = 0, tiles_h = 0, tiles_w = 0, tiles_n = 0;
  int splitk = 1, kb_per_split = 0;
  int mode = 0;
  int flat = 0;
  OperandScheme ops = OperandScheme::BF16X3;
  int valid = 0;
};

int conv_tc_plan(mpn_ctx *ctx, const ConvProblem &p, ConvPlan &plan);
int conv_tc_launch(mpn_ctx *ctx, const ConvProblem &p, const ConvPlan &plan);
int conv_ref_launch(mpn_ctx *ctx, const ConvProblem &p);
int conv_direct_nchw_launch(mpn_ctx *ctx, const float *x_nchw, int N, int Cin, int H, int W, const float *w,
                            const float *bias, int Cout, int kh, int kw, int stride, int pad, int relu,
                            DTensor &y, const float *w_host = nullptr, const float *bias_host = nullptr);
int conv1_tc_launch(mpn_ctx *ctx, const float *x_nchw, int N, int H, int W, const float *w_dev, const float *bias_dev, int relu,
                    DTensor &y);
double conv_flops(const ConvProblem &p);
int mpn_fp8_quantize_launch(mpn_ctx *ctx, const DTensor &x, uint8_t *q8, int *exps);
int mpn_fp8_weight_launch(mpn_ctx *ctx, const __nv_bfloat16 *w_hi, int64_t rows, int64_t K, int64_t rows_pad, uint8_t *q8, int *exps);
```

### multipathnet_b200/csrc/gemm_tc.cu

```cuda
#include "conv_gemm.cuh"
#include "wgmma.cuh"
#include "fp8_e4m3.cuh"
#include <algorithm>
#include <stdlib.h>
#include <string.h>

namespace {

constexpr int BM = 128;
constexpr int BK = 64;
constexpr int TC_THREADS = 384;
constexpr int CONS_THREADS = 256;
constexpr int A_TILE_BYTES = BM * BK * 2;
constexpr int SMEM_BUDGET = 196608;

__host__ __device__ constexpr int a_planes(OperandScheme ops) { return (ops == OperandScheme::BF16X1 || ops == OperandScheme::FP8X1) ? 1 : 2; }
__host__ __device__ constexpr int b_planes(OperandScheme ops) { return ops == OperandScheme::BF16X3 ? 2 : 1; }
__host__ __device__ constexpr int elem_bytes(OperandScheme ops) { return ops == OperandScheme::FP8X1 ? 1 : 2; }
__host__ __device__ constexpr int row_bytes(int BN, OperandScheme ops) { return (ops == OperandScheme::FP8X1 || BN == 256) ? 64 : 128; }
__host__ __device__ constexpr int stage_k(int BN, OperandScheme ops) { return row_bytes(BN, ops) / elem_bytes(ops); }
__host__ __device__ constexpr int kb_steps(int BN, OperandScheme ops) { return BK / stage_k(BN, ops); }
__host__ __device__ constexpr int a_tile_bytes(int BN, OperandScheme ops) { return BM * row_bytes(BN, ops); }
__host__ __device__ constexpr int stage_bytes(int BN, OperandScheme ops = OperandScheme::BF16X3) {
  return (a_planes(ops) * BM + b_planes(ops) * BN) * row_bytes(BN, ops);
}
__host__ __device__ constexpr int max_stages(int BN, OperandScheme ops) { return row_bytes(BN, ops) == 64 ? 8 : 4; }
__host__ __device__ constexpr int num_stages(int BN, OperandScheme ops = OperandScheme::BF16X3) {
  return (SMEM_BUDGET / stage_bytes(BN, ops)) > max_stages(BN, ops) ? max_stages(BN, ops) : (SMEM_BUDGET / stage_bytes(BN, ops));
}
constexpr int EPI_WARP_BYTES = 16 * 128;
constexpr int EPI_BYTES = (CONS_THREADS / 32) * EPI_WARP_BYTES;
__host__ __device__ constexpr int tc_smem_bytes(int BN, OperandScheme ops) {
  return num_stages(BN, ops) * stage_bytes(BN, ops) + EPI_BYTES + 1024  + 256 ;
}

struct TcParams {
  int N, Ho, Wo, Cout;
  int kh, kw, stride, pad;
  int cblocks;
  int tn, th, tw;
  int tiles_img, tiles_h, tiles_w, tiles_n;
  int units;
  const float *bias;
  const __nv_bfloat16 *res_hi, *res_lo; long long res_ld;
  __nv_bfloat16 *out_hi, *out_lo; long long out_ld;
  float *out_f32; long long out_f32_ld;
  __nv_bfloat16 *pool_hi, *pool_lo; long long pool_ld; int Hp, Wp;
  int relu;
  int splitk, kb_per_split;
  long long split_stride;
  unsigned long long *tl_min, *tl_max;
  float acc_scale;
  int out_fmt;
  unsigned *ovf;
  const int *a_exp, *b_exp; long long sample_pix;
};

__device__ __forceinline__ unsigned long long gtimer() {
  unsigned long long t; asm volatile("mov.u64 %0, %%globaltimer;" : "=l"(t)); return t;
}
__device__ __forceinline__ void tl_min_stamp(const unsigned long long *base_, int i) {
  if (base_) atomicMin(const_cast<unsigned long long *>(base_) + i, gtimer());
}
__device__ __forceinline__ void tl_max_stamp(const unsigned long long *base_, int i) {
  if (base_) atomicMax(const_cast<unsigned long long *>(base_) + i, gtimer());
}
__device__ __forceinline__ uint32_t smem_u32(const void *p) { return (uint32_t)__cvta_generic_to_shared(p); }
__device__ __forceinline__ void mbar_init(uint32_t bar, uint32_t count) {
  asm volatile("mbarrier.init.shared::cta.b64 [%0], %1;" ::"r"(bar), "r"(count) : "memory");
}
__device__ __forceinline__ void mbar_expect_tx(uint32_t bar, uint32_t bytes) {
  asm volatile("mbarrier.arrive.expect_tx.shared::cta.b64 _, [%0], %1;" ::"r"(bar), "r"(bytes) : "memory");
}
__device__ __forceinline__ void mbar_arrive(uint32_t bar) {
  asm volatile("mbarrier.arrive.shared::cta.b64 _, [%0];" ::"r"(bar) : "memory");
}
__device__ __forceinline__ void mbar_wait(uint32_t bar, uint32_t parity) {
  uint32_t done;
  uint32_t spins = 0;
  do {
    asm volatile(
        "{\n\t.reg .pred p;\n\t"
        "mbarrier.try_wait.parity.shared::cta.b64 p, [%1], %2;\n\t"
        "selp.u32 %0, 1, 0, p;\n\t}"
        : "=r"(done) : "r"(bar), "r"(parity) : "memory");
    if (!done && ++spins == (1u << 26)) __trap();
  } while (!done);
}
__device__ __forceinline__ void tma_load_4d(uint32_t dst, const CUtensorMap *tm, uint32_t bar, int c0, int c1,
                                            int c2, int c3) {
  asm volatile(
      "cp.async.bulk.tensor.4d.shared::cluster.global.mbarrier::complete_tx::bytes [%0], [%1, {%3, %4, %5, %6}], [%2];"
      ::"r"(dst), "l"(reinterpret_cast<uint64_t>(tm)), "r"(bar), "r"(c0), "r"(c1), "r"(c2), "r"(c3) : "memory");
}
__device__ __forceinline__ void tma_load_2d(uint32_t dst, const CUtensorMap *tm, uint32_t bar, int c0, int c1) {
  asm volatile(
      "cp.async.bulk.tensor.2d.shared::cluster.global.mbarrier::complete_tx::bytes [%0], [%1, {%3, %4}], [%2];"
      ::"r"(dst), "l"(reinterpret_cast<uint64_t>(tm)), "r"(bar), "r"(c0), "r"(c1) : "memory");
}
__device__ __forceinline__ void prefetch_tmap(const CUtensorMap *tm) {
  asm volatile("prefetch.tensormap [%0];" ::"l"(reinterpret_cast<uint64_t>(tm)) : "memory");
}

__device__ __forceinline__ uint64_t make_smem_desc(uint32_t saddr) {
  uint64_t d = 0;
  d |= (uint64_t)((saddr & 0x3FFFFu) >> 4);
  d |= (uint64_t)1 << 16;
  d |= (uint64_t)(1024 >> 4) << 32;
  d |= (uint64_t)1 << 62;
  return d;
}

__device__ __forceinline__ uint64_t make_smem_desc_64b(uint32_t saddr) {
  uint64_t d = 0;
  d |= (uint64_t)((saddr & 0x3FFFFu) >> 4);
  d |= (uint64_t)1 << 16;
  d |= (uint64_t)(512 >> 4) << 32;
  d |= (uint64_t)2 << 62;
  return d;
}

template <int BN, OperandScheme OPS>
__device__ __forceinline__ void mma_kstep(float (&acc)[BN / 2], uint64_t a_hi, uint64_t a_lo, uint64_t b_hi, uint64_t b_lo, bool first) {
  constexpr bool F16 = (OPS == OperandScheme::FP16X2);
#pragma unroll
  for (int k = 0; k < stage_k(BN, OPS) / 16; ++k) {
    const uint64_t adv = (uint64_t)((k * 16 * 2) >> 4);
    const uint32_t later = (first && k == 0) ? 0u : 1u;
    if constexpr (OPS == OperandScheme::BF16X1) {
      wgmma_nk16<BN, false>(acc, a_hi + adv, b_hi + adv, later);
    } else {
      wgmma_nk16<BN, F16>(acc, a_lo + adv, b_hi + adv, later);
      if (!F16) wgmma_nk16<BN, F16>(acc, a_hi + adv, b_lo + adv, 1u);
      wgmma_nk16<BN, F16>(acc, a_hi + adv, b_hi + adv, 1u);
    }
  }
}

struct UnitPos { int nt, twi, thi, tni, split; };
__device__ __forceinline__ UnitPos unit_pos(const TcParams &p, int unit) {
  UnitPos u;
  const int tile = unit / p.splitk;
  u.split = unit - tile * p.splitk;
  u.nt = tile % p.tiles_n;
  const int mt = tile / p.tiles_n;
  u.twi = mt % p.tiles_w; u.thi = (mt / p.tiles_w) % p.tiles_h; u.tni = mt / (p.tiles_w * p.tiles_h);
  return u;
}
__device__ __forceinline__ long long row_pixel(const TcParams &p, const UnitPos &u, int row, bool &ok, int *whn = nullptr) {
  const int lw = __ffs(p.tw) - 1, lh = __ffs(p.th) - 1;
  const int wl = row & (p.tw - 1), hl = (row >> lw) & (p.th - 1), nl = row >> (lw + lh);
  const int wo = u.twi * p.tw + wl, ho = u.thi * p.th + hl, n = u.tni * p.tn + nl;
  ok = (wo < p.Wo) && (ho < p.Ho) && (n < p.N);
  if (whn) { whn[0] = wo; whn[1] = ho; whn[2] = n; }
  return ((long long)n * p.Ho + ho) * p.Wo + wo;
}

__device__ __forceinline__ void store_plane_chunk(uint32_t so, const uint32_t (&v)[16], __nv_bfloat16 *out, long long ld,
                                                  const TcParams &p, const UnitPos &u, int rbase, int col0, int lane) {
  const int r = lane >> 2;
  const uint32_t wr = so + (uint32_t)(r * 128 + 4 * (lane & 3));
  __syncwarp();
#pragma unroll
  for (int j = 0; j < 8; ++j) {
    const uint32_t a = wr + (uint32_t)((j ^ r) * 16);
    asm volatile("st.shared.b32 [%0], %1;" ::"r"(a), "r"(v[j]) : "memory");
    asm volatile("st.shared.b32 [%0], %1;" ::"r"(a + 8 * 128), "r"(v[8 + j]) : "memory");
  }
  __syncwarp();
  const int row0 = lane >> 3, ch = lane & 7;
  const uint32_t rd0 = so + (uint32_t)(row0 * 128 + ((ch ^ row0) * 16)), rd1 = so + (uint32_t)(row0 * 128 + ((ch ^ row0 ^ 4) * 16));
  const bool col_ok = col0 + 8 * ch < p.Cout;
#pragma unroll
  for (int q = 0; q < 4; ++q) {
    uint4 d;
    asm volatile("ld.shared.v4.b32 {%0, %1, %2, %3}, [%4];" : "=r"(d.x), "=r"(d.y), "=r"(d.z), "=r"(d.w)
                 : "r"(((q & 1) ? rd1 : rd0) + (uint32_t)(q * 4 * 128)) : "memory");
    bool ok;
    const long long pix = row_pixel(p, u, rbase + 4 * q + row0, ok);
    if (ok && col_ok) *reinterpret_cast<uint4 *>(out + pix * ld + col0 + 8 * ch) = d;
  }
}

template <int BN, OperandScheme OPS>
__device__ __forceinline__ void tile_epilogue(const TcParams &p, const UnitPos &u, float (&acc)[BN / 2], int g, int wq,
                                              int lane, uint32_t so) {
  const int rbase = 64 * g + 16 * wq;
  const int c0 = 2 * (lane & 3);
  bool fok[2]; long long fpix[2];
#pragma unroll
  for (int i = 0; i < 2; ++i) fpix[i] = row_pixel(p, u, rbase + (lane >> 2) + 8 * i, fok[i]);
  int ea[2] = {0, 0};
  if constexpr (OPS == OperandScheme::FP8X1) {
#pragma unroll
    for (int i = 0; i < 2; ++i) ea[i] = fok[i] ? __ldg(p.a_exp + fpix[i] / p.sample_pix) : 0;
  }
  const bool pool = (p.pool_hi != nullptr);
  bool pok = false; long long ppix = 0;
  if (pool) {
    int whn[3];
    row_pixel(p, u, rbase + 2 * (lane >> 3), pok, whn);
    ppix = ((long long)whn[2] * p.Hp + (whn[1] >> 1)) * p.Wp + (whn[0] >> 1);
  }
  float *const out_f32 = p.out_f32 ? p.out_f32 + (long long)u.split * p.split_stride : nullptr;
#pragma unroll 1
  for (int m = 0; m < BN / 64; ++m) {
    const int col0 = u.nt * BN + 64 * m;
    if (col0 >= p.Cout) break;
    float *f = acc;
#pragma unroll
    for (int j = 0; j < 8; ++j) {
      const int c = col0 + 8 * j + c0;
      const bool full8 = col0 + 8 * j + 8 <= p.Cout;
      float b[2] = {0.f, 0.f};
      int eb[2] = {0, 0};
#pragma unroll
      for (int k = 0; k < 2; ++k) {
        if (p.bias && c + k < p.Cout) b[k] = __ldg(p.bias + c + k);
        if constexpr (OPS == OperandScheme::FP8X1) eb[k] = __ldg(p.b_exp + c + k);
      }
#pragma unroll
      for (int i = 0; i < 2; ++i) {
        float &f0 = f[4 * j + 2 * i], &f1 = f[4 * j + 2 * i + 1];
        if constexpr (OPS == OperandScheme::FP16X2) { f0 *= p.acc_scale; f1 *= p.acc_scale; }
        if constexpr (OPS == OperandScheme::FP8X1) {
          f0 *= mpn_fp8::pow2(-(ea[i] + eb[0])); f1 *= mpn_fp8::pow2(-(ea[i] + eb[1]));
        }
        if (p.bias) {
          if (c < p.Cout) f0 += b[0];
          if (c + 1 < p.Cout) f1 += b[1];
        }
        if (p.res_hi && full8 && fok[i]) {
          const float2 x = bf16x2_to_float2(*reinterpret_cast<const uint32_t *>(p.res_hi + fpix[i] * p.res_ld + c));
          const float2 y = bf16x2_to_float2(*reinterpret_cast<const uint32_t *>(p.res_lo + fpix[i] * p.res_ld + c));
          f0 += x.x + y.x; f1 += x.y + y.y;
        }
        if (p.relu) { f0 = fmaxf(f0, 0.f); f1 = fmaxf(f1, 0.f); }
        if (out_f32 && fok[i]) {
          float *o = out_f32 + fpix[i] * p.out_f32_ld + c;
          if (c < p.Cout) o[0] = f0;
          if (c + 1 < p.Cout) o[1] = f1;
        }
      }
    }
    float mx[16];
    if (pool) {
#pragma unroll
      for (int j = 0; j < 8; ++j)
#pragma unroll
        for (int k = 0; k < 2; ++k) {
          float top = fok[0] ? f[4 * j + k] : -INFINITY, bot = fok[1] ? f[4 * j + 2 + k] : -INFINITY;
          top = fmaxf(top, __shfl_xor_sync(0xffffffffu, top, 4));
          bot = fmaxf(bot, __shfl_xor_sync(0xffffffffu, bot, 4));
          mx[2 * j + k] = fmaxf(top, bot);
        }
    }
#pragma unroll 1
    for (int plane = 0; plane < 2; ++plane) {
      if (p.out_hi) {
        uint32_t v[16];
#pragma unroll
        for (int j = 0; j < 8; ++j)
#pragma unroll
          for (int i = 0; i < 2; ++i) {
            uint32_t hi2 = 0, lo2 = 0;
            if (fok[i]) split_x2(p.out_fmt, f[4 * j + 2 * i], f[4 * j + 2 * i + 1], hi2, lo2, p.ovf);
            v[8 * i + j] = plane ? lo2 : hi2;
          }
        store_plane_chunk(so, v, plane ? p.out_lo : p.out_hi, p.out_ld, p, u, rbase, col0, lane);
      }
      if (pool) {
        const int pr = lane >> 3;
        __syncwarp();
        if (!(lane & 4) && fok[0]) {
#pragma unroll
          for (int j = 0; j < 8; ++j) {
            uint32_t hi2, lo2;
            split_x2(p.out_fmt, mx[2 * j], mx[2 * j + 1], hi2, lo2, p.ovf);
            const uint32_t a = so + (uint32_t)(pr * 128 + ((j ^ pr) * 16) + 4 * (lane & 3));
            asm volatile("st.shared.b32 [%0], %1;" ::"r"(a), "r"(plane ? lo2 : hi2) : "memory");
          }
        }
        __syncwarp();
        const int ch = lane & 7;
        uint4 d;
        asm volatile("ld.shared.v4.b32 {%0, %1, %2, %3}, [%4];" : "=r"(d.x), "=r"(d.y), "=r"(d.z), "=r"(d.w)
                     : "r"(so + (uint32_t)(pr * 128 + ((ch ^ pr) * 16))) : "memory");
        if (pok && col0 + 8 * ch < p.Cout)
          *reinterpret_cast<uint4 *>((plane ? p.pool_lo : p.pool_hi) + ppix * p.pool_ld + col0 + 8 * ch) = d;
      }
    }
#pragma unroll
    for (int k = 0; k + 32 < BN / 2; ++k) acc[k] = acc[k + 32];
  }
}

template <int BN, OperandScheme OPS = OperandScheme::BF16X3>
__global__ void __launch_bounds__(TC_THREADS, 1)
conv_gemm_tc_kernel(const __grid_constant__ CUtensorMap tmA_hi, const __grid_constant__ CUtensorMap tmA_lo,
                    const __grid_constant__ CUtensorMap tmB_hi, const __grid_constant__ CUtensorMap tmB_lo,
                    const TcParams p) {
  constexpr int S = num_stages(BN, OPS);
  constexpr int STAGE = stage_bytes(BN, OPS);
  constexpr int A_TILE = a_tile_bytes(BN, OPS);
  constexpr int B_TILE_BYTES = BN * row_bytes(BN, OPS);
  constexpr int B_OFF = a_planes(OPS) * A_TILE;
  constexpr int KSTEPS = kb_steps(BN, OPS);
  static_assert(S >= 2 && 2 * S * 8 <= 256, "ring depth: at least two stages, barriers in their 256 bytes");
  extern __shared__ uint8_t smem_raw[];
  uint8_t *smem = reinterpret_cast<uint8_t *>((reinterpret_cast<uintptr_t>(smem_raw) + 1023) & ~(uintptr_t)1023);
  uint64_t *bars = reinterpret_cast<uint64_t *>(smem + (size_t)S * STAGE + EPI_BYTES);
  const uint32_t smem_base = smem_u32(smem);
  const uint32_t bar_base = smem_u32(bars);
  auto full_bar = [&](int s) { return bar_base + 8u * s; };
  auto empty_bar = [&](int s) { return bar_base + 8u * (S + s); };

  const int tid = threadIdx.x, lane = tid & 31;
  const int num_kb = p.kh * p.kw * p.cblocks;

  if (tid == 0) {
    tl_min_stamp(p.tl_min, 0);
    if (a_planes(OPS) == 1) { prefetch_tmap(&tmA_hi); prefetch_tmap(&tmB_hi); }
    else { prefetch_tmap(&tmA_hi); prefetch_tmap(&tmA_lo); prefetch_tmap(&tmB_hi); prefetch_tmap(&tmB_lo); }
    for (int s = 0; s < S; ++s) { mbar_init(full_bar(s), 1); mbar_init(empty_bar(s), CONS_THREADS / 32); }
    asm volatile("fence.mbarrier_init.release.cluster;" ::: "memory");
  }
  __syncthreads();
  asm volatile("griddepcontrol.wait;" ::: "memory");
  asm volatile("griddepcontrol.launch_dependents;" ::: "memory");
  if (tid == 0) tl_min_stamp(p.tl_min, 1);

  if (tid < 128) {
    asm volatile("setmaxnreg.dec.sync.aligned.u32 24;" ::: "memory");
    if (tid == 0) {
      int it = 0;
      for (int unit = (int)blockIdx.x; unit < p.units; unit += (int)gridDim.x) {
        const UnitPos u = unit_pos(p, unit);
        const int kb0 = u.split * p.kb_per_split, kb1 = min(num_kb, kb0 + p.kb_per_split);
        const int w_in0 = u.twi * p.tw * p.stride - p.pad, h_in0 = u.thi * p.th * p.stride - p.pad, n0 = u.tni * p.tn;
        const int b_row0 = u.nt * BN;
        for (int kb = kb0; kb < kb1; ++kb) {
          const int tap = kb / p.cblocks, cb = kb - tap * p.cblocks;
          const int khi = tap / p.kw, kwi = tap - khi * p.kw;
#pragma unroll
          for (int h = 0; h < KSTEPS; ++h, ++it) {
            const int s = it % S; const uint32_t ph = (uint32_t)(it / S) & 1u;
            const int ka = cb * BK + h * stage_k(BN, OPS), kk = kb * BK + h * stage_k(BN, OPS);
            mbar_wait(empty_bar(s), ph ^ 1u);
            const uint32_t sa = smem_base + (uint32_t)s * STAGE;
            mbar_expect_tx(full_bar(s), (uint32_t)STAGE);
            tma_load_4d(sa, &tmA_hi, full_bar(s), ka, w_in0 + kwi, h_in0 + khi, n0);
            if (a_planes(OPS) == 2) tma_load_4d(sa + A_TILE, &tmA_lo, full_bar(s), ka, w_in0 + kwi, h_in0 + khi, n0);
            tma_load_2d(sa + B_OFF, &tmB_hi, full_bar(s), kk, b_row0);
            if (b_planes(OPS) == 2) tma_load_2d(sa + B_OFF + B_TILE_BYTES, &tmB_lo, full_bar(s), kk, b_row0);
          }
        }
      }
    }
    return;
  }

  asm volatile("setmaxnreg.inc.sync.aligned.u32 240;" ::: "memory");
  const int e = tid - 128;
  const int g = e >> 7, wq = (e >> 5) & 3;
  const uint32_t so = smem_base + (uint32_t)(S * STAGE + (e >> 5) * EPI_WARP_BYTES);
  int it = 0;
  for (int unit = (int)blockIdx.x; unit < p.units; unit += (int)gridDim.x) {
    const UnitPos u = unit_pos(p, unit);
    const int kb0 = u.split * p.kb_per_split, kb1 = min(num_kb, kb0 + p.kb_per_split);
    float acc[BN / 2];
#pragma unroll
    for (int i = 0; i < BN / 2; ++i) acc[i] = 0.f;
    if constexpr (OPS == OperandScheme::FP8X1) {
      float part[BN / 2];
#pragma unroll
      for (int i = 0; i < BN / 2; ++i) part[i] = 0.f;
      for (int kb = kb0; kb < kb1; ++kb, ++it) {
        const int s = it % S; const uint32_t ph = (uint32_t)(it / S) & 1u;
        mbar_wait(full_bar(s), ph);
        if (it == 0 && e == 0) tl_min_stamp(p.tl_min, 2);
        const uint32_t sa = smem_base + (uint32_t)s * STAGE;
        const uint64_t a8 = make_smem_desc_64b(sa + (uint32_t)g * (A_TILE / 2));
        const uint64_t b8 = make_smem_desc_64b(sa + B_OFF);
#pragma unroll
        for (int k = 0; k < BK / 32; ++k) {
          wgmma_fence_acc(part);
          wgmma_fence();
          wgmma_e4m3_nk32<BN>(part, a8 + (uint64_t)(2 * k), b8 + (uint64_t)(2 * k), 0u);
          wgmma_commit();
          wgmma_wait<0>();
          wgmma_fence_acc(part);
#pragma unroll
          for (int i = 0; i < BN / 2; ++i) acc[i] += part[i];
        }
        if (lane == 0) mbar_arrive(empty_bar(s));
      }
    } else {
      const int steps = (kb1 - kb0) * KSTEPS;
      for (int i = 0; i < steps; ++i, ++it) {
        const int s = it % S; const uint32_t ph = (uint32_t)(it / S) & 1u;
        mbar_wait(full_bar(s), ph);
        if (it == 0 && e == 0) tl_min_stamp(p.tl_min, 2);
        const uint32_t sa = smem_base + (uint32_t)s * STAGE;
        auto desc = [](uint32_t a) { return row_bytes(BN, OPS) == 64 ? make_smem_desc_64b(a) : make_smem_desc(a); };
        const uint64_t a_hi = desc(sa + (uint32_t)g * (A_TILE / 2));
        const uint64_t a_lo = desc(sa + A_TILE + (uint32_t)g * (A_TILE / 2));
        const uint64_t b_hi = desc(sa + B_OFF);
        const uint64_t b_lo = desc(sa + B_OFF + B_TILE_BYTES);
        wgmma_fence_acc(acc);
        wgmma_fence();
        mma_kstep<BN, OPS>(acc, a_hi, a_lo, b_hi, b_lo, i == 0);
        wgmma_commit();
        wgmma_wait<1>();
        wgmma_fence_acc(acc);
        if (i > 0 && lane == 0) mbar_arrive(empty_bar((it - 1) % S));
      }
      wgmma_wait<0>();
      wgmma_fence_acc(acc);
      if (lane == 0) mbar_arrive(empty_bar((it - 1) % S));
    }
    if (e == 0) tl_max_stamp(p.tl_max, 0);
    const uint32_t t_epi = (p.tl_max && e == 0) ? (uint32_t)gtimer() : 0u;
    tile_epilogue<BN, OPS>(p, u, acc, g, wq, lane, so);
    if (e == 0) {
      tl_max_stamp(p.tl_max, 1);
      if (p.tl_max) atomicAdd(p.tl_max + 3, (unsigned long long)((uint32_t)gtimer() - t_epi));
    }
  }
}


constexpr int C1_THREADS = 256;
constexpr int C1_A_BYTES = 2 * A_TILE_BYTES;
constexpr int C1_B_BYTES = 2 * 64 * 128;
constexpr int C1_OUT_WARP = 16 * 128;
constexpr int C1_SMEM = 2 * C1_A_BYTES + C1_B_BYTES + (C1_THREADS / 32) * C1_OUT_WARP + 1024;

__device__ __forceinline__ void conv1_gather(const float *__restrict__ x, int pix, int pixels, int H, int W, int bhalf,
                                             float (&in)[16]) {
#pragma unroll
  for (int k = 0; k < 16; ++k) in[k] = 0.f;
  if (pix < pixels) {
    const int HW = H * W;
    const int n = pix / HW, rem = pix - n * HW;
    const int ho = rem / W, wo = rem - ho * W;
    const float *x0 = x + ((size_t)n * 3 * HW + (size_t)(ho - 1) * W + (wo - 1));
    const bool rok[3] = {ho >= 1, true, ho + 1 < H}, cok[3] = {wo >= 1, true, wo + 1 < W};
#pragma unroll
    for (int k = 0; k < 16; ++k) {
      const int kk = 16 * bhalf + k;
      if (kk < 27) {
        const int ci = kk / 9, r = (kk / 3) % 3, q = kk % 3;
        in[k] = (rok[r] && cok[q]) ? __ldg(x0 + ci * HW + r * W + q) : 0.f;
      }
    }
  }
}

__device__ __forceinline__ void conv1_store_plane(uint32_t so, const uint32_t (&v)[16], __nv_bfloat16 *out, int pix0,
                                                  int pixels, int lane) {
  const int r = lane >> 2;
  const uint32_t wr = so + (uint32_t)(r * 128 + 4 * (lane & 3));
  __syncwarp();
#pragma unroll
  for (int j = 0; j < 8; ++j) {
    const uint32_t a = wr + (uint32_t)((j ^ r) * 16);
    asm volatile("st.shared.b32 [%0], %1;" ::"r"(a), "r"(v[j]) : "memory");
    asm volatile("st.shared.b32 [%0], %1;" ::"r"(a + 8 * 128), "r"(v[8 + j]) : "memory");
  }
  __syncwarp();
  const int row0 = lane >> 3, ch = lane & 7;
  const uint32_t rd0 = so + (uint32_t)(row0 * 128 + ((ch ^ row0) * 16)), rd1 = so + (uint32_t)(row0 * 128 + ((ch ^ row0 ^ 4) * 16));
  __nv_bfloat16 *o = out + (size_t)(pix0 + row0) * 64 + ch * 8;
#pragma unroll
  for (int q = 0; q < 4; ++q) {
    uint4 d;
    asm volatile("ld.shared.v4.b32 {%0, %1, %2, %3}, [%4];" : "=r"(d.x), "=r"(d.y), "=r"(d.z), "=r"(d.w)
                 : "r"(((q & 1) ? rd1 : rd0) + (uint32_t)(q * 4 * 128)) : "memory");
    if (pix0 + row0 + 4 * q < pixels) *reinterpret_cast<uint4 *>(o + q * 4 * 64) = d;
  }
}

__global__ void __launch_bounds__(C1_THREADS, 2)
conv1_tc_kernel(const float *__restrict__ x, int N, int H, int W, const float *__restrict__ w, const float *__restrict__ bias,
                int relu, __nv_bfloat16 *__restrict__ out_hi, __nv_bfloat16 *__restrict__ out_lo) {
  extern __shared__ uint8_t smem_raw[];
  uint8_t *smem = reinterpret_cast<uint8_t *>((reinterpret_cast<uintptr_t>(smem_raw) + 1023) & ~(uintptr_t)1023);
  uint8_t *sB = smem + 2 * C1_A_BYTES;
  const int tid = threadIdx.x, lane = tid & 31, warp = tid >> 5;
  const uint32_t so = smem_u32(sB + C1_B_BYTES) + (uint32_t)(warp * C1_OUT_WARP);
  const uint32_t b_base = smem_u32(sB);
  const int g = tid >> 7;
  const int pixels = N * H * W;
  const int total_tiles = (pixels + BM - 1) / BM;
  asm volatile("griddepcontrol.wait;" ::: "memory");
  asm volatile("griddepcontrol.launch_dependents;" ::: "memory");
  const int c0 = 2 * (lane & 3);
  for (int i = tid; i < 64 * 4; i += C1_THREADS) {
    const int row = i >> 2, j = i & 3;
    uint32_t hh[4], ll[4];
#pragma unroll
    for (int q = 0; q < 4; ++q) {
      const int k0 = j * 8 + 2 * q;
      const float v0 = (k0 < 27) ? __ldg(w + row * 27 + k0) : 0.f, v1 = (k0 + 1 < 27) ? __ldg(w + row * 27 + k0 + 1) : 0.f;
      split_bf16x2(v0, v1, hh[q], ll[q]);
    }
    const uint32_t off = (uint32_t)row * 128u + (uint32_t)((j ^ (row & 7)) * 16);
    *reinterpret_cast<uint4 *>(sB + off) = make_uint4(hh[0], hh[1], hh[2], hh[3]);
    *reinterpret_cast<uint4 *>(sB + 64 * 128 + off) = make_uint4(ll[0], ll[1], ll[2], ll[3]);
  }
  const int brow = tid & 127, bhalf = tid >> 7;
  float in[16];
  conv1_gather(x, (int)blockIdx.x * BM + brow, pixels, H, W, bhalf, in);
  for (int tile = blockIdx.x, it = 0; tile < total_tiles; tile += gridDim.x, ++it) {
    uint8_t *sa = smem + (it & 1) * C1_A_BYTES;
    uint8_t *pa = sa + (size_t)brow * 128;
#pragma unroll
    for (int jj = 0; jj < 2; ++jj) {
      const int j = 2 * bhalf + jj;
      uint32_t hh[4], ll[4];
#pragma unroll
      for (int q = 0; q < 4; ++q) split_bf16x2(in[jj * 8 + 2 * q], in[jj * 8 + 2 * q + 1], hh[q], ll[q]);
      const int pj = (j ^ (brow & 7)) * 16;
      *reinterpret_cast<uint4 *>(pa + pj) = make_uint4(hh[0], hh[1], hh[2], hh[3]);
      *reinterpret_cast<uint4 *>(pa + A_TILE_BYTES + pj) = make_uint4(ll[0], ll[1], ll[2], ll[3]);
    }
    asm volatile("fence.proxy.async.shared::cta;" ::: "memory");
    __syncthreads();
    float acc[32];
#pragma unroll
    for (int i = 0; i < 32; ++i) acc[i] = 0.f;
    const uint32_t a_base = smem_u32(sa);
    const uint64_t a_hi = make_smem_desc(a_base + (uint32_t)g * (A_TILE_BYTES / 2));
    const uint64_t a_lo = make_smem_desc(a_base + A_TILE_BYTES + (uint32_t)g * (A_TILE_BYTES / 2));
    const uint64_t b_hi = make_smem_desc(b_base), b_lo = make_smem_desc(b_base + 64 * 128);
    wgmma_fence_acc(acc);
    wgmma_fence();
#pragma unroll
    for (int k = 0; k < 2; ++k) {
      const uint64_t adv = (uint64_t)((k * 16 * 2) >> 4);
      wgmma_nk16<64, false>(acc, a_lo + adv, b_hi + adv, k ? 1u : 0u);
      wgmma_nk16<64, false>(acc, a_hi + adv, b_lo + adv, 1u);
      wgmma_nk16<64, false>(acc, a_hi + adv, b_hi + adv, 1u);
    }
    wgmma_commit();
    const int next = tile + (int)gridDim.x;
    conv1_gather(x, next < total_tiles ? next * BM + brow : pixels, pixels, H, W, bhalf, in);
    wgmma_wait<0>();
    wgmma_fence_acc(acc);
#pragma unroll
    for (int j = 0; j < 8; ++j) {
      const float2 b = __ldg(reinterpret_cast<const float2 *>(bias + 8 * j + c0));
#pragma unroll
      for (int h = 0; h < 2; ++h) {
        float &f0 = acc[4 * j + 2 * h], &f1 = acc[4 * j + 2 * h + 1];
        f0 += b.x; f1 += b.y;
        if (relu) { f0 = fmaxf(f0, 0.f); f1 = fmaxf(f1, 0.f); }
      }
    }
    const int pix0 = tile * BM + 64 * g + 16 * (warp & 3);
#pragma unroll 1
    for (int plane = 0; plane < 2; ++plane) {
      uint32_t v[16];
#pragma unroll
      for (int j = 0; j < 8; ++j)
#pragma unroll
        for (int h = 0; h < 2; ++h) {
          uint32_t hi2, lo2;
          split_bf16x2(acc[4 * j + 2 * h], acc[4 * j + 2 * h + 1], hi2, lo2);
          v[8 * h + j] = plane ? lo2 : hi2;
        }
      conv1_store_plane(so, v, plane ? out_lo : out_hi, pix0, pixels, lane);
    }
  }
}

struct ReduceParams {
  const float *ws; long long split_stride; int splitk; long long pixels; int Cout;
  const float *bias; const __nv_bfloat16 *res_hi, *res_lo; long long res_ld; int relu;
  __nv_bfloat16 *out_hi, *out_lo; long long out_ld; float *out_f32; long long out_f32_ld;
  OutScatter scatter;
};
__global__ void __launch_bounds__(256) splitk_reduce_kernel(const ReduceParams r) {
  MPN_PDL_SYNC();
  const long long idx = (long long)blockIdx.x * blockDim.x + threadIdx.x;
  if (idx >= r.pixels * r.Cout) return;
  const long long pix = idx / r.Cout; const int c = (int)(idx - pix * r.Cout);
  float acc = 0.f;
  for (int s = 0; s < r.splitk; ++s) acc += r.ws[(long long)s * r.split_stride + idx];
  if (r.bias) acc += __ldg(r.bias + c);
  if (r.res_hi) acc += join_bf16(r.res_hi[pix * r.res_ld + c], r.res_lo[pix * r.res_ld + c]);
  if (r.relu) acc = fmaxf(acc, 0.f);
  if (r.out_hi) { __nv_bfloat16 h, l; split_bf16(acc, h, l); r.out_hi[pix * r.out_ld + c] = h; r.out_lo[pix * r.out_ld + c] = l; }
  if (r.scatter.n > 0) {
#pragma unroll 1
    for (int g = 0; g < r.scatter.n; ++g)
      if (c >= r.scatter.seg[g].c0 && c < r.scatter.seg[g].c1) { r.scatter.seg[g].ptr[pix * r.scatter.seg[g].ld + (c - r.scatter.seg[g].c0)] = acc; break; }
  } else if (r.out_f32) r.out_f32[pix * r.out_f32_ld + c] = acc;
}

typedef CUresult (*PFN_encodeTiled)(CUtensorMap *, CUtensorMapDataType, cuuint32_t, void *, const cuuint64_t *,
                                    const cuuint64_t *, const cuuint32_t *, const cuuint32_t *, CUtensorMapInterleave,
                                    CUtensorMapSwizzle, CUtensorMapL2promotion, CUtensorMapFloatOOBfill);
PFN_encodeTiled get_encode_fn() {
  static PFN_encodeTiled fn = nullptr;
  if (!fn) {
    void *p = nullptr; cudaDriverEntryPointQueryResult q;
    if (cudaGetDriverEntryPoint("cuTensorMapEncodeTiled", &p, cudaEnableDefault, &q) == cudaSuccess &&
        q == cudaDriverEntryPointSuccess)
      fn = reinterpret_cast<PFN_encodeTiled>(p);
  }
  return fn;
}

int encode_map(mpn_ctx *ctx, CUtensorMap *tm, const void *base, int rank, const cuuint64_t *dims,
               const cuuint64_t *strides_bytes , const cuuint32_t *box, const cuuint32_t *estr, int BN, OperandScheme ops) {
  const bool fp8 = ops == OperandScheme::FP8X1;
  PFN_encodeTiled fn = get_encode_fn();
  if (!fn) return mpn_fail(ctx, MPN_ERR_CUDA, "cuTensorMapEncodeTiled entry point unavailable");
  CUresult r = fn(tm, fp8 ? CU_TENSOR_MAP_DATA_TYPE_UINT8 : CU_TENSOR_MAP_DATA_TYPE_BFLOAT16, (cuuint32_t)rank, const_cast<void *>(base), dims,
                  strides_bytes, box, estr, CU_TENSOR_MAP_INTERLEAVE_NONE, row_bytes(BN, ops) == 64 ? CU_TENSOR_MAP_SWIZZLE_64B : CU_TENSOR_MAP_SWIZZLE_128B,
                  CU_TENSOR_MAP_L2_PROMOTION_L2_256B, CU_TENSOR_MAP_FLOAT_OOB_FILL_NONE);
  if (r != CUDA_SUCCESS) {
    char b[256];
    snprintf(b, sizeof b, "cuTensorMapEncodeTiled failed (%d): rank %d dims %llu %llu box %u %u", (int)r, rank,
             (unsigned long long)dims[0], (unsigned long long)dims[1], box[0], box[1]);
    return mpn_fail(ctx, MPN_ERR_CUDA, b);
  }
  return MPN_OK;
}

inline bool tc_use_pdl() {
  static const int on = [] { const char *e = getenv("MPN_TC_PDL"); return (e && e[0] == '0') ? 0 : 1; }();
  return on != 0;
}

template <int BN, OperandScheme OPS = OperandScheme::BF16X3>
int launch_bn(mpn_ctx *ctx, const ConvPlan &pl, const TcParams &tp) {
  const int smem = tc_smem_bytes(BN, OPS);
  constexpr int bslot = BN == 256 ? 2 : (BN == 128 ? 1 : 0);
  constexpr int slot = OPS == OperandScheme::FP16X2 ? 3 : (OPS == OperandScheme::BF16X1 ? 5 + bslot
                                                         : (OPS == OperandScheme::FP8X1 ? 8 + bslot : bslot));
  if (!ctx->tc_attr_set[slot]) {
    MPN_CUDA(ctx, cudaFuncSetAttribute(conv_gemm_tc_kernel<BN, OPS>, cudaFuncAttributeMaxDynamicSharedMemorySize, smem));
    ctx->tc_attr_set[slot] = 1;
  }
  const long long units = (long long)pl.tiles_img * pl.tiles_h * pl.tiles_w * pl.tiles_n * pl.splitk;
  MPN_CHECK_ARG(ctx, units > 0 && units < (1ll << 31), "conv_tc: grid size out of range");
  TcParams tpu = tp;
  tpu.units = (int)units;
  cudaLaunchConfig_t cfg = {};
  cfg.gridDim = dim3((unsigned)std::min<long long>(units, ctx->sm_count));
  cfg.blockDim = dim3(TC_THREADS); cfg.dynamicSmemBytes = (size_t)smem; cfg.stream = ctx->stream;
  cudaLaunchAttribute attr[1];
  int na = 0;
  if (tc_use_pdl()) {
    attr[na].id = cudaLaunchAttributeProgrammaticStreamSerialization;
    attr[na].val.programmaticStreamSerializationAllowed = 1;
    ++na;
  }
  cfg.attrs = attr; cfg.numAttrs = na;
  MPN_CUDA(ctx, cudaLaunchKernelEx(&cfg, conv_gemm_tc_kernel<BN, OPS>, pl.tmA_hi, pl.tmA_lo, pl.tmB_hi, pl.tmB_lo, tpu));
  MPN_LAUNCHED(ctx);
  return MPN_OK;
}

int launch_ops(mpn_ctx *ctx, const ConvPlan &pl, const TcParams &tp) {
  if (pl.ops == OperandScheme::FP16X2) return launch_bn<256, OperandScheme::FP16X2>(ctx, pl, tp);
  if (pl.ops == OperandScheme::FP8X1)
    return pl.BN == 128 ? launch_bn<128, OperandScheme::FP8X1>(ctx, pl, tp) : launch_bn<64, OperandScheme::FP8X1>(ctx, pl, tp);
  if (pl.ops == OperandScheme::BF16X1) {
    switch (pl.BN) {
      case 256: return launch_bn<256, OperandScheme::BF16X1>(ctx, pl, tp);
      case 128: return launch_bn<128, OperandScheme::BF16X1>(ctx, pl, tp);
      default: return launch_bn<64, OperandScheme::BF16X1>(ctx, pl, tp);
    }
  }
  switch (pl.BN) {
    case 256: return launch_bn<256>(ctx, pl, tp);
    case 128: return launch_bn<128>(ctx, pl, tp);
    default: return launch_bn<64>(ctx, pl, tp);
  }
}

}

int conv1_tc_launch(mpn_ctx *ctx, const float *x_nchw, int N, int H, int W, const float *w_dev, const float *bias_dev, int relu,
                    DTensor &y) {
  MPN_CHECK_ARG(ctx, y.hi && y.lo && y.C == 64 && y.ld % 8 == 0, "conv1_tc: output must be 64-channel split planes");
  MPN_CHECK_ARG(ctx, bias_dev, "conv1_tc: bias missing");
  MPN_CHECK_ARG(ctx, y.ld == 64 && (long long)N * H * W < (1ll << 31) - 256, "conv1_tc: dense 64-channel output and < 2^31 pixels");
  if (!ctx->tc_attr_set[4]) {
    MPN_CUDA(ctx, cudaFuncSetAttribute(conv1_tc_kernel, cudaFuncAttributeMaxDynamicSharedMemorySize, C1_SMEM));
    ctx->tc_attr_set[4] = 1;
  }
  const long long tiles = ((long long)N * H * W + BM - 1) / BM;
  cudaLaunchConfig_t cfg = {};
  cfg.gridDim = dim3((unsigned)std::min<long long>(tiles, 2ll * ctx->sm_count)); cfg.blockDim = dim3(C1_THREADS);
  cfg.dynamicSmemBytes = (size_t)C1_SMEM; cfg.stream = ctx->stream;
  cudaLaunchAttribute attr[1];
  int na = 0;
  if (tc_use_pdl()) { attr[na].id = cudaLaunchAttributeProgrammaticStreamSerialization; attr[na].val.programmaticStreamSerializationAllowed = 1; ++na; }
  cfg.attrs = attr; cfg.numAttrs = na;
  MPN_CUDA(ctx, cudaLaunchKernelEx(&cfg, conv1_tc_kernel, x_nchw, N, H, W, w_dev, bias_dev, relu, y.hi, y.lo));
  MPN_LAUNCHED(ctx);
  return MPN_OK;
}

double conv_flops(const ConvProblem &p) {
  const double Ho = (double)p.y.H, Wo = (double)p.y.W;
  return 2.0 * (double)p.x.C * p.Cout * p.kh * p.kw * Ho * Wo * (double)p.y.N;
}

static int conv_tc_plan_impl(mpn_ctx *ctx, int sm_count, const ConvProblem &p, ConvPlan &pl, bool choose_only) {
  pl.valid = 0;
  MPN_CHECK_ARG(ctx, choose_only || (p.x.hi && p.x.lo && ((p.w_hi && p.w_lo) || p.w16)), "conv_tc: operands must be split-bf16 (or an fp16 weight plane)");
  MPN_CHECK_ARG(ctx, !(p.w16 && p.bf16), "conv_tc: the bf16 numerics do not take an fp16 weight plane");
  MPN_CHECK_ARG(ctx, !(p.fp8 && (p.w16 || p.bf16)), "conv_tc: the fp8 numerics take neither an fp16 weight plane nor the bf16 numerics");
  MPN_CHECK_ARG(ctx, choose_only || !p.fp8 || (p.x8 && p.x8_exp && p.w8 && p.w8_exp), "conv_tc: the fp8 numerics need e4m3 planes and exponents");
  pl.ops = p.w16 ? OperandScheme::FP16X2 : (p.fp8 ? OperandScheme::FP8X1 : (p.bf16 ? OperandScheme::BF16X1 : OperandScheme::BF16X3));
  const bool w16 = pl.ops == OperandScheme::FP16X2, fp8 = pl.ops == OperandScheme::FP8X1;
  MPN_CHECK_ARG(ctx, choose_only || (p.x.fmt == 1) == w16, "conv_tc: fp16 activation planes go with the fp16 weight plane (and only with it)");
  MPN_CHECK_ARG(ctx, p.x.C % BK == 0, "conv_tc: Cin must be a multiple of 64");
  MPN_CHECK_ARG(ctx, p.x.ld % 8 == 0, "conv_tc: input pixel stride must be a multiple of 8 elements");
  MPN_CHECK_ARG(ctx, p.stride >= 1 && p.stride <= 2, "conv_tc: stride must be 1 or 2");
  const int Ho = (int)p.y.H, Wo = (int)p.y.W, N = (int)p.y.N;
  pl.flat = (p.kh == 1 && p.kw == 1 && p.stride == 1 && p.pad == 0) ? 1 : 0;
  pl.mode = 0; pl.splitk = 1;
  cuuint64_t dims[4], strides[3]; cuuint32_t box[4], estr[4];
  int gtn = 1, gth = 1, gtw = BM;
  if (!pl.flat) {
    double best = -1.0;
    for (int tw = 1; tw <= 128; tw <<= 1)
      for (int th = 1; th * tw <= 128; th <<= 1) {
        const int tn = 128 / (tw * th);
        if (tw * p.stride > 256 || th * p.stride > 256) continue;
        const long long tiles = (long long)((Wo + tw - 1) / tw) * ((Ho + th - 1) / th) * ((N + tn - 1) / tn);
        const double util = (double)N * Ho * Wo / (double)(tiles * 128) + 1e-6 * tw;
        if (util > best) { best = util; gtn = tn; gth = th; gtw = tw; }
      }
  }
  const long long P = (long long)p.x.N * p.x.H * p.x.W;
  {
    const bool r3_ok = (p.kh == 3 && p.kw == 3 && p.stride == 1 && p.pad == 1);
    const char *env3 = getenv("MPN_TC_R3");
    const char *env3m = getenv("MPN_TC_R3_MINPIX");
    const long long r3_minpix = env3m ? atoll(env3m) : 0;
    pl.mode = (r3_ok && !(env3 && env3[0] == '0') && P >= r3_minpix) ? 1 : 0;
  }
  const long long tiles_m = pl.flat ? (P + BM - 1) / BM
                                    : (pl.mode ? (long long)((Wo + 7) / 8) * ((Ho + 15) / 16) * N
                                               : (long long)((Wo + gtw - 1) / gtw) * ((Ho + gth - 1) / gth) * ((N + gtn - 1) / gtn));
  {
    const int taps = p.kh * p.kw;
    const double kblocks = (double)taps * (double)(p.x.C / BK);
    double best = 1e300; int best_bn = 64;
    for (int bi = 0; bi < 3; ++bi) {
      const int bn = bi == 0 ? 256 : (bi == 1 ? 128 : 64);
      if (w16 && bn != 256) continue;
      if (fp8 && bn == 256) continue;
      if (!p.m_invariant && bn > 64 && bn > ((p.Cout + 63) / 64) * 64) continue;
      const int roi_bn = p.Cout > 128 ? 256 : (p.Cout > 64 ? 128 : 64);
      if (p.m_invariant && bn != (fp8 ? std::min(roi_bn, 128) : roi_bn)) continue;
      const long long units = tiles_m * ((p.Cout + bn - 1) / bn);
      const long long rounds = (units + sm_count - 1) / sm_count;
      const double mma = (w16 ? 2.0 : (pl.ops == OperandScheme::BF16X1 ? 1.0 : (fp8 ? 0.5 : 3.0))) * 128.0 * bn * 64.0 / 1024.0;
      const double ingest = ((double)a_planes(pl.ops) * 128 + (double)b_planes(pl.ops) * bn) * (fp8 ? 64.0 : 128.0) / 48.0;
      const double cost = (double)rounds * (kblocks * std::max(mma, ingest) + 1500.0 + 8.0 * bn);
      if (cost < best * 0.999) { best = cost; best_bn = bn; }
    }
    pl.BN = best_bn;
    pl.tiles_n = (p.Cout + pl.BN - 1) / pl.BN;
  }
  if (pl.flat) {
    pl.tn = 1; pl.th = 1; pl.tw = BM;
    pl.tiles_img = 1; pl.tiles_h = 1; pl.tiles_w = (int)((P + BM - 1) / BM);
    dims[0] = (cuuint64_t)p.x.C; dims[1] = (cuuint64_t)P; dims[2] = 1; dims[3] = 1;
    strides[0] = (cuuint64_t)p.x.ld * 2; strides[1] = (cuuint64_t)P * p.x.ld * 2; strides[2] = strides[1];
    box[0] = (cuuint32_t)stage_k(pl.BN, pl.ops); box[1] = BM; box[2] = 1; box[3] = 1;
    estr[0] = estr[1] = estr[2] = estr[3] = 1;
  } else {
    if (pl.mode == 1) { pl.tn = 1; pl.th = 16; pl.tw = 8; }
    else { pl.tn = gtn; pl.th = gth; pl.tw = gtw; }
    pl.tiles_w = (Wo + pl.tw - 1) / pl.tw; pl.tiles_h = (Ho + pl.th - 1) / pl.th; pl.tiles_img = (N + pl.tn - 1) / pl.tn;
    dims[0] = (cuuint64_t)p.x.C; dims[1] = (cuuint64_t)p.x.W; dims[2] = (cuuint64_t)p.x.H; dims[3] = (cuuint64_t)p.x.N;
    strides[0] = (cuuint64_t)p.x.ld * 2; strides[1] = (cuuint64_t)p.x.W * p.x.ld * 2;
    strides[2] = (cuuint64_t)p.x.H * p.x.W * p.x.ld * 2;
    box[0] = (cuuint32_t)stage_k(pl.BN, pl.ops); box[1] = (cuuint32_t)(pl.tw * p.stride); box[2] = (cuuint32_t)(pl.th * p.stride); box[3] = (cuuint32_t)pl.tn;
    estr[0] = 1; estr[1] = (cuuint32_t)p.stride; estr[2] = (cuuint32_t)p.stride; estr[3] = 1;
  }
  {
    const long long units = tiles_m * pl.tiles_n;
    const long long num_kb = (long long)p.kh * p.kw * (p.x.C / BK);
    long long sk = std::min<long long>(num_kb / 8, 8);
    if (p.m_invariant) { if (!(pl.flat && p.Cout <= 128) || sk < 2) sk = 1; }
    else if (p.wide_k_split && pl.flat && num_kb >= 256)
      sk = std::max<long long>({1, std::min<long long>(sm_count / units, num_kb / 8), (num_kb + 31) / 32});
    else if (pl.mode == 1 || sk < 2 || units * sk > sm_count) sk = 1;
    const char *env2 = getenv("MPN_TC_SPLITK");
    if (env2 && env2[0] == '0') sk = 1;
    pl.splitk = (int)std::max<long long>(sk, 1);
    pl.kb_per_split = (int)((num_kb + pl.splitk - 1) / pl.splitk);
    pl.splitk = (int)((num_kb + pl.kb_per_split - 1) / pl.kb_per_split);
  }
  if (choose_only) return MPN_OK;
  const long long Ktot = (long long)p.kh * p.kw * p.x.C;
  cuuint64_t bd[2] = {(cuuint64_t)Ktot, (cuuint64_t)p.Cout}, bs[1] = {(cuuint64_t)Ktot * 2};
  cuuint32_t bb[2] = {(cuuint32_t)stage_k(pl.BN, pl.ops), (cuuint32_t)pl.BN}, be[2] = {1, 1};
  if (fp8) {
    const cuuint64_t C8 = (cuuint64_t)p.x.C;
    if (pl.flat) { strides[0] = C8; strides[1] = (cuuint64_t)P * C8; strides[2] = strides[1]; }
    else { strides[0] = C8; strides[1] = (cuuint64_t)p.x.W * C8; strides[2] = (cuuint64_t)p.x.H * p.x.W * C8; }
    bs[0] = (cuuint64_t)Ktot;
    MPN_TRY(encode_map(ctx, &pl.tmA_hi, p.x8, 4, dims, strides, box, estr, pl.BN, pl.ops));
    MPN_TRY(encode_map(ctx, &pl.tmB_hi, p.w8, 2, bd, bs, bb, be, pl.BN, pl.ops));
    pl.tmA_lo = pl.tmA_hi; pl.tmB_lo = pl.tmB_hi;
    pl.valid = 1;
    return MPN_OK;
  }
  MPN_TRY(encode_map(ctx, &pl.tmA_hi, p.x.hi, 4, dims, strides, box, estr, pl.BN, pl.ops));
  if (a_planes(pl.ops) == 2) { MPN_TRY(encode_map(ctx, &pl.tmA_lo, p.x.lo, 4, dims, strides, box, estr, pl.BN, pl.ops)); }
  else pl.tmA_lo = pl.tmA_hi;
  if (w16) {
    MPN_CHECK_ARG(ctx, pl.mode == 0 && pl.flat && pl.splitk == 1 && pl.BN == 256, "conv_tc: the fp16-weight path is for wide flat GEMMs without split-K");
    MPN_TRY(encode_map(ctx, &pl.tmB_hi, p.w16, 2, bd, bs, bb, be, pl.BN, pl.ops));
    pl.tmB_lo = pl.tmB_hi;
  } else {
    MPN_TRY(encode_map(ctx, &pl.tmB_hi, p.w_hi, 2, bd, bs, bb, be, pl.BN, pl.ops));
    if (b_planes(pl.ops) == 2) { MPN_TRY(encode_map(ctx, &pl.tmB_lo, p.w_lo, 2, bd, bs, bb, be, pl.BN, pl.ops)); }
    else pl.tmB_lo = pl.tmB_hi;
  }
  pl.valid = 1;
  return MPN_OK;
}

int conv_tc_plan(mpn_ctx *ctx, const ConvProblem &p, ConvPlan &pl) { return conv_tc_plan_impl(ctx, ctx->sm_count, p, pl, false); }

int conv_tc_launch(mpn_ctx *ctx, const ConvProblem &p, const ConvPlan &pl) {
  MpnProfScope prof_scope__(ctx, MPN_CAT_CONV_TC);
  MPN_CHECK_ARG(ctx, pl.valid, "conv_tc_launch: invalid plan");
  TcParams tp;
  memset(&tp, 0, sizeof(tp));
  if (pl.flat) { tp.N = 1; tp.Ho = 1; tp.Wo = (int)(p.y.N * p.y.H * p.y.W); }
  else { tp.N = (int)p.y.N; tp.Ho = (int)p.y.H; tp.Wo = (int)p.y.W; }
  tp.Cout = p.Cout; tp.kh = p.kh; tp.kw = p.kw; tp.stride = p.stride; tp.pad = p.pad;
  tp.cblocks = (int)(p.x.C / BK);
  tp.tn = pl.tn; tp.th = pl.th; tp.tw = pl.tw;
  tp.tiles_img = pl.tiles_img; tp.tiles_h = pl.tiles_h; tp.tiles_w = pl.tiles_w; tp.tiles_n = pl.tiles_n;
  tp.bias = p.bias;
  tp.res_hi = p.res.hi; tp.res_lo = p.res.lo; tp.res_ld = p.res.ld;
  tp.out_hi = p.y.hi; tp.out_lo = p.y.lo; tp.out_ld = p.y.ld;
  tp.out_f32 = p.y.f32; tp.out_f32_ld = p.y_f32_ld;
  tp.relu = p.relu;
  tp.splitk = pl.splitk; tp.kb_per_split = pl.kb_per_split; tp.split_stride = 0;
  tp.acc_scale = pl.ops == OperandScheme::FP16X2 ? p.w16_inv_scale : 1.f;
  tp.out_fmt = p.y.fmt; tp.ovf = nullptr;
  if (p.y.fmt) MPN_TRY(mpn_ovf_flag(ctx, &tp.ovf));
  if (pl.ops == OperandScheme::FP8X1) { tp.a_exp = p.x8_exp; tp.b_exp = p.w8_exp; tp.sample_pix = p.y.H * p.y.W; }
  MPN_CHECK_ARG(ctx, !p.pool.hi || p.pool.fmt == p.y.fmt, "conv_tc: pooled output must share the output's plane format");
  MPN_CHECK_ARG(ctx, !(p.y.fmt && pl.splitk > 1), "conv_tc: fp16 output planes are not written by the split-K reduce");
  MPN_CHECK_ARG(ctx, !p.res.hi || p.res.fmt == 0, "conv_tc: residual inputs are bf16 split planes");
  if (ctx->tl_on && ctx->tl_n < ctx->tl_cap) { tp.tl_min = ctx->tl_min + 4 * ctx->tl_n; tp.tl_max = ctx->tl_max + 4 * ctx->tl_n; ++ctx->tl_n; }
  if (p.pool.hi) {
    MPN_CHECK_ARG(ctx, pl.mode == 1 && pl.splitk == 1 && !p.res.hi && p.Cout % 8 == 0 && p.pool.ld % 8 == 0,
                  "conv_tc: fused pooling needs the 3x3 kernel, no residual, Cout multiple of 8");
    MPN_CHECK_ARG(ctx, p.pool.H == (p.y.H + 1) / 2 && p.pool.W == (p.y.W + 1) / 2 && p.pool.N == p.y.N, "conv_tc: pooled geometry mismatch");
    tp.pool_hi = p.pool.hi; tp.pool_lo = p.pool.lo; tp.pool_ld = p.pool.ld; tp.Hp = (int)p.pool.H; tp.Wp = (int)p.pool.W;
    if (p.pool_only) { tp.out_hi = tp.out_lo = nullptr; tp.out_f32 = nullptr; }
  }
  if (p.y.hi) MPN_CHECK_ARG(ctx, p.Cout % 8 == 0 && p.y.ld % 8 == 0, "conv_tc: split output needs Cout, ld multiples of 8");
  MPN_CHECK_ARG(ctx, p.scatter.n == 0 || pl.splitk > 1, "conv_tc: scattered outputs need a split-K plan");
  if (pl.splitk > 1) {
    const long long pixels = (long long)p.y.N * p.y.H * p.y.W;
    float *ws = nullptr;
    MPN_TRY(mpn_scratch3(ctx, sizeof(float) * (size_t)pl.splitk * pixels * p.Cout, (void **)&ws));
    tp.bias = nullptr; tp.res_hi = tp.res_lo = nullptr; tp.relu = 0; tp.out_hi = tp.out_lo = nullptr;
    tp.out_f32 = ws; tp.out_f32_ld = p.Cout; tp.split_stride = pixels * p.Cout;
    MPN_TRY(launch_ops(ctx, pl, tp));
    ReduceParams r;
    r.ws = ws; r.split_stride = tp.split_stride; r.splitk = pl.splitk; r.pixels = pixels; r.Cout = p.Cout;
    r.bias = p.bias; r.res_hi = p.res.hi; r.res_lo = p.res.lo; r.res_ld = p.res.ld; r.relu = p.relu;
    r.out_hi = p.y.hi; r.out_lo = p.y.lo; r.out_ld = p.y.ld; r.out_f32 = p.y.f32; r.out_f32_ld = p.y_f32_ld;
    r.scatter = p.scatter;
    const long long total = pixels * p.Cout;
    MPN_CUDA(ctx, mpn_launch_pdl(ctx, splitk_reduce_kernel, dim3((unsigned)((total + 255) / 256)), dim3(256), 0, r));
    MPN_LAUNCHED(ctx);
    return MPN_OK;
  }
  return launch_ops(ctx, pl, tp);
}

extern "C" int mpn_debug_plan(int64_t N, int64_t Cin, int64_t H, int64_t W, int64_t Cout, int32_t k, int32_t stride, int32_t pad,
                              int32_t per_roi, int32_t sm_count, int32_t *out) {
  if (!out || N <= 0 || Cin <= 0 || Cin % 64 || H <= 0 || W <= 0 || Cout <= 0 || k <= 0 || stride < 1 || stride > 2 || pad < 0 || sm_count < 2)
    return MPN_ERR_ARG;
  ConvProblem p;
  p.x.N = N; p.x.H = H; p.x.W = W; p.x.C = Cin; p.x.ld = Cin;
  p.Cout = (int)Cout; p.kh = p.kw = k; p.stride = stride; p.pad = pad; p.m_invariant = per_roi ? 1 : 0;
  p.y.N = N; p.y.H = (H + 2 * pad - k) / stride + 1; p.y.W = (W + 2 * pad - k) / stride + 1; p.y.C = Cout; p.y.ld = Cout;
  if (p.y.H <= 0 || p.y.W <= 0) return MPN_ERR_ARG;
  ConvPlan pl;
  const int rc = conv_tc_plan_impl(nullptr, sm_count, p, pl, true);
  if (rc != MPN_OK) return rc;
  out[0] = pl.mode; out[1] = 1; out[2] = pl.BN; out[3] = pl.splitk; out[4] = 0; out[5] = pl.tn; out[6] = pl.th; out[7] = pl.tw;
  return MPN_OK;
}
```

Baseline: 414,400.

## Pair CTAs in clusters and multicast shared weight tiles via TMA

Adds a cluster-of-two CTA mode for flat, non-split-K conv GEMMs. Each CTA in the pair loads half of the B (weight) tile and multicasts it to both CTAs, so every weight byte is fetched from L2/global once for two M tiles. Empty barriers now count consumers from both CTAs, and an idle rank still takes part in the pipeline when M tiles are odd. The mode is on by default when the plan qualifies. It adds cluster synchronisation and cross-CTA coupling, which can stall a CTA on its partner and limits scheduling to pairs.

```diff
diff --git a/include/mpn_abi.h b/include/mpn_abi.h
--- a/include/mpn_abi.h
+++ b/include/mpn_abi.h
@@ -226,6 +226,13 @@
                    uint64_t *dbg16);
 int mpn_debug_plan(int64_t N, int64_t Cin, int64_t H, int64_t W, int64_t Cout, int32_t k, int32_t stride, int32_t pad,
                    int32_t per_roi, int32_t sm_count, int32_t *out);
+int mpn_debug_plan_pair(int64_t N, int64_t Cin, int64_t H, int64_t W, int64_t Cout, int32_t k, int32_t stride, int32_t pad,
+                        int32_t per_roi, int32_t sm_count, int32_t *out);
+int mpn_debug_pair_schedule(int64_t N, int64_t Cin, int64_t H, int64_t W, int64_t Cout, int32_t k, int32_t stride, int32_t pad,
+                            int32_t per_roi, int32_t sm_count, int32_t scheme, int32_t clusters, int64_t *out);
+int mpn_debug_engine_pair(mpn_ctx *ctx, int32_t pair, int32_t op, const float *x, int64_t N, int64_t Cin, int64_t H, int64_t W,
+                          const float *w, const float *bias, int64_t Cout, int32_t k, int32_t stride, int32_t pad, int32_t relu,
+                          float *y, float *y_pool, int32_t *plan_out);
 int mpn_debug_fp8(const float *h, int64_t n_samples, int64_t sample_elems, int32_t *e_out, uint8_t *q_out);
 int mpn_conv_check(mpn_ctx *ctx, const float *x, int64_t N, int64_t Cin, int64_t H, int64_t W,
                    const float *w, const float *bias, int64_t Cout, int32_t kh, int32_t kw,
diff --git a/multipathnet_b200/_lib.py b/multipathnet_b200/_lib.py
--- a/multipathnet_b200/_lib.py
+++ b/multipathnet_b200/_lib.py
@@ -191,6 +191,11 @@
     "mpn_conv_bench": (C.c_int, [_vp, C.c_int64, C.c_int64, C.c_int64, C.c_int64, C.c_int64, C.c_int32, C.c_int32, C.c_int32, C.c_int32,
                                  C.POINTER(C.c_double), _i32p, _i32p, _i32p, C.POINTER(C.c_uint64)]),
     "mpn_debug_plan": (C.c_int, [C.c_int64, C.c_int64, C.c_int64, C.c_int64, C.c_int64, C.c_int32, C.c_int32, C.c_int32, C.c_int32, C.c_int32, _i32p]),
+    "mpn_debug_plan_pair": (C.c_int, [C.c_int64, C.c_int64, C.c_int64, C.c_int64, C.c_int64, C.c_int32, C.c_int32, C.c_int32, C.c_int32, C.c_int32, _i32p]),
+    "mpn_debug_pair_schedule": (C.c_int, [C.c_int64, C.c_int64, C.c_int64, C.c_int64, C.c_int64, C.c_int32, C.c_int32, C.c_int32, C.c_int32,
+                                          C.c_int32, C.c_int32, C.c_int32, _i64p]),
+    "mpn_debug_engine_pair": (C.c_int, [_vp, C.c_int32, C.c_int32, _vp, C.c_int64, C.c_int64, C.c_int64, C.c_int64, _vp, _vp, C.c_int64,
+                                        C.c_int32, C.c_int32, C.c_int32, C.c_int32, _vp, _vp, _i32p]),
     "mpn_debug_fp8": (C.c_int, [_vp, C.c_int64, C.c_int64, _vp, _vp]),
     "mpn_gemm_check": (C.c_int, [_vp, _vp, _vp, _vp, C.c_int64, C.c_int64, C.c_int64, C.c_int32, C.c_int32, _vp]),
     "mpn_conv_check": (C.c_int, [_vp, _vp, C.c_int64, C.c_int64, C.c_int64, C.c_int64, _vp, _vp, C.c_int64,
diff --git a/multipathnet_b200/csrc/abi.cu b/multipathnet_b200/csrc/abi.cu
--- a/multipathnet_b200/csrc/abi.cu
+++ b/multipathnet_b200/csrc/abi.cu
@@ -712,6 +712,78 @@
   if (ctx->opt_fp8 == 1) MPN_TRY(mpn_ovf_copy_async(ctx, ctx->stream));
   MPN_CUDA(ctx, cudaStreamSynchronize(ctx->stream));
   return ctx->opt_fp8 == 1 ? mpn_ovf_test(ctx) : MPN_OK;
+}
+
+int mpn_debug_engine_pair(mpn_ctx *ctx, int32_t pair, int32_t op, const float *x, int64_t N, int64_t Cin, int64_t H, int64_t W,
+                          const float *w, const float *bias, int64_t Cout, int32_t k, int32_t stride, int32_t pad, int32_t relu,
+                          float *y, float *y_pool, int32_t *plan_out) {
+  if (!ctx) return MPN_ERR_ARG;
+  MPN_CUDA(ctx, cudaSetDevice(ctx->device));
+  MPN_CHECK_ARG(ctx, x && w && y && N > 0 && Cin > 0 && Cout > 0 && H > 0 && W > 0 && k > 0 && op >= 0 && op <= 2, "bad arguments");
+  MPN_CHECK_ARG(ctx, op != 2 || (k == 1 && H == 1 && W == 1 && stride == 1 && pad == 0), "the fp16-weight GEMM is a 1x1 convolution of rows");
+  MPN_CHECK_ARG(ctx, !y_pool || op == 0, "the fused pool writes split planes (op 0)");
+  MPN_CHECK_ARG(ctx, !(ctx->opt_fp8 == 1 && ctx->opt_bf16 == 1), "the \"fp8\" and \"bf16\" options are both on");
+  const int64_t Ho = (H + 2 * pad - k) / stride + 1, Wo = (W + 2 * pad - k) / stride + 1;
+  MPN_CHECK_ARG(ctx, Ho > 0 && Wo > 0, "empty output");
+  const int64_t Hp = (Ho + 1) / 2, Wp = (Wo + 1) / 2;
+  const size_t nx = (size_t)(N * Cin * H * W), nw = (size_t)(Cout * Cin * k * k), ny = (size_t)(N * Cout * Ho * Wo),
+               np = (size_t)(N * Cout * Hp * Wp);
+  Arena a{ctx};
+  size_t o_x = a.reserve(4 * nx), o_w = a.reserve(4 * nw), o_b = a.reserve(4 * (size_t)Cout), o_y = a.reserve(4 * ny),
+         o_xh = a.reserve(2 * nx), o_xl = a.reserve(2 * nx), o_wh = a.reserve(2 * nw), o_wl = a.reserve(2 * nw),
+         o_yh = a.reserve(2 * ny), o_yl = a.reserve(2 * ny), o_ph = a.reserve(2 * np), o_pl = a.reserve(2 * np), o_p = a.reserve(4 * np),
+         o_x8 = a.reserve(nx), o_xe = a.reserve(4 * (size_t)N), o_w8 = a.reserve(nw), o_we = a.reserve(4 * (size_t)(Cout + 127) / 128 * 128);
+  MPN_TRY(a.commit());
+  MPN_CUDA(ctx, cudaMemcpyAsync(a.at<float>(o_x), x, 4 * nx, cudaMemcpyHostToDevice, ctx->stream));
+  MPN_CUDA(ctx, cudaMemcpyAsync(a.at<float>(o_w), w, 4 * nw, cudaMemcpyHostToDevice, ctx->stream));
+  if (bias) MPN_CUDA(ctx, cudaMemcpyAsync(a.at<float>(o_b), bias, 4 * (size_t)Cout, cudaMemcpyHostToDevice, ctx->stream));
+  DTensor tx; tx.hi = a.at<__nv_bfloat16>(o_xh); tx.lo = a.at<__nv_bfloat16>(o_xl); tx.N = N; tx.H = H; tx.W = W; tx.C = Cin; tx.ld = Cin;
+  DTensor ty; ty.N = N; ty.H = Ho; ty.W = Wo; ty.C = Cout; ty.ld = Cout;
+  ConvProblem p;
+  p.bias = bias ? a.at<float>(o_b) : nullptr; p.Cout = (int)Cout; p.kh = p.kw = k; p.stride = stride; p.pad = pad; p.relu = relu;
+  if (op == 2) {
+    MPN_TRY(mpn_split_rows_f16_launch(ctx, a.at<float>(o_x), N, Cin, Cin, tx.hi, tx.lo, Cin));
+    tx.fmt = 1;
+    float amax = 0.f;
+    MPN_TRY(mpn_absmax(ctx, a.at<float>(o_w), (int64_t)nw, &amax));
+    int e = 0;
+    if (amax > 0.f) { (void)frexpf(amax, &e); e = 14 - e; }
+    const float sc = ldexpf(1.0f, e);
+    MPN_TRY(mpn_weight_permute_half_launch(ctx, a.at<float>(o_w), Cout, (int)Cin, 1, 1, sc, a.at<void>(o_wh)));
+    p.x = tx; p.w16 = a.at<void>(o_wh); p.w16_inv_scale = 1.0f / sc; p.m_invariant = 1;
+    ty.f32 = a.at<float>(o_y); p.y = ty; p.y_f32_ld = Cout;
+  } else {
+    MPN_TRY(mpn_nchw_to_nhwc_split_launch(ctx, a.at<float>(o_x), (int)N, (int)Cin, (int)H, (int)W, tx));
+    MPN_TRY(mpn_weight_permute_split_launch(ctx, a.at<float>(o_w), Cout, (int)Cin, k, k, a.at<__nv_bfloat16>(o_wh), a.at<__nv_bfloat16>(o_wl)));
+    p.x = tx; p.w_hi = a.at<__nv_bfloat16>(o_wh); p.w_lo = a.at<__nv_bfloat16>(o_wl);
+    p.bf16 = ctx->opt_bf16 == 1 ? 1 : 0;
+    if (op == 0) { ty.hi = a.at<__nv_bfloat16>(o_yh); ty.lo = a.at<__nv_bfloat16>(o_yl); }
+    else { ty.f32 = a.at<float>(o_y); p.y_f32_ld = Cout; }
+    p.y = ty;
+    if (y_pool) {
+      DTensor tp; tp.hi = a.at<__nv_bfloat16>(o_ph); tp.lo = a.at<__nv_bfloat16>(o_pl); tp.N = N; tp.H = Hp; tp.W = Wp; tp.C = Cout; tp.ld = Cout;
+      p.pool = tp;
+    }
+    if (ctx->opt_fp8 == 1) {
+      p.fp8 = 1;
+      p.x8 = a.at<uint8_t>(o_x8); p.x8_exp = a.at<int>(o_xe); p.w8 = a.at<uint8_t>(o_w8); p.w8_exp = a.at<int>(o_we);
+      MPN_TRY(mpn_fp8_quantize_launch(ctx, tx, a.at<uint8_t>(o_x8), a.at<int>(o_xe)));
+      MPN_TRY(mpn_fp8_weight_launch(ctx, p.w_hi, Cout, (int64_t)Cin * k * k, (Cout + 127) / 128 * 128, a.at<uint8_t>(o_w8), a.at<int>(o_we)));
+    }
+  }
+  ConvPlan pl;
+  MPN_TRY(conv_tc_plan_pair(ctx, p, pl, pair));
+  MPN_TRY(conv_tc_launch(ctx, p, pl));
+  if (plan_out) { plan_out[0] = pl.BN; plan_out[1] = pl.splitk; plan_out[2] = pl.mode; plan_out[3] = pl.pair; }
+  if (op == 0) MPN_TRY(mpn_nhwc_split_to_nchw_launch(ctx, ty, a.at<float>(o_y)));
+  MPN_CUDA(ctx, cudaMemcpyAsync(y, a.at<float>(o_y), 4 * ny, cudaMemcpyDeviceToHost, ctx->stream));
+  if (y_pool) {
+    MPN_TRY(mpn_nhwc_split_to_nchw_launch(ctx, p.pool, a.at<float>(o_p)));
+    MPN_CUDA(ctx, cudaMemcpyAsync(y_pool, a.at<float>(o_p), 4 * np, cudaMemcpyDeviceToHost, ctx->stream));
+  }
+  if (ctx->opt_fp8 == 1 && op != 2) MPN_TRY(mpn_ovf_copy_async(ctx, ctx->stream));
+  MPN_CUDA(ctx, cudaStreamSynchronize(ctx->stream));
+  return (ctx->opt_fp8 == 1 && op != 2) ? mpn_ovf_test(ctx) : MPN_OK;
 }
 
 int mpn_gemm_bench(mpn_ctx *ctx, int64_t M, int64_t N, int64_t K, int32_t iters, double *ms_per_launch, int32_t *bn,
diff --git a/multipathnet_b200/csrc/common.cuh b/multipathnet_b200/csrc/common.cuh
--- a/multipathnet_b200/csrc/common.cuh
+++ b/multipathnet_b200/csrc/common.cuh
@@ -27,6 +27,8 @@
   std::vector<ProfRec> prof;
   std::vector<cudaEvent_t> ev_pool;
   uint8_t tc_attr_set[32] = {0};
+  uint8_t tc_pair_attr_set[10] = {0};
+  int tc_clusters[10] = {0};
   void *nms_tie_ptr = nullptr; int nms_tie_n = 0;
   unsigned long long *tl_min = nullptr, *tl_max = nullptr; int tl_cap = 0, tl_n = 0, tl_on = 0;
   int opt_fc_w16 = -1;
diff --git a/multipathnet_b200/csrc/conv_gemm.cuh b/multipathnet_b200/csrc/conv_gemm.cuh
--- a/multipathnet_b200/csrc/conv_gemm.cuh
+++ b/multipathnet_b200/csrc/conv_gemm.cuh
@@ -36,11 +36,13 @@
   int splitk = 1, kb_per_split = 0;
   int mode = 0;
   int flat = 0;
+  int pair = 1;
   OperandScheme ops = OperandScheme::BF16X3;
   int valid = 0;
 };
 
 int conv_tc_plan(mpn_ctx *ctx, const ConvProblem &p, ConvPlan &plan);
+int conv_tc_plan_pair(mpn_ctx *ctx, const ConvProblem &p, ConvPlan &plan, int pair);
 int conv_tc_launch(mpn_ctx *ctx, const ConvProblem &p, const ConvPlan &plan);
 int conv_ref_launch(mpn_ctx *ctx, const ConvProblem &p);
 int conv_direct_nchw_launch(mpn_ctx *ctx, const float *x_nchw, int N, int Cin, int H, int W, const float *w,
diff --git a/multipathnet_b200/csrc/gemm_tc.cu b/multipathnet_b200/csrc/gemm_tc.cu
--- a/multipathnet_b200/csrc/gemm_tc.cu
+++ b/multipathnet_b200/csrc/gemm_tc.cu
@@ -2,6 +2,7 @@
 #include "wgmma.cuh"
 #include "fp8_e4m3.cuh"
 #include <algorithm>
+#include <vector>
 #include <stdlib.h>
 #include <string.h>
 
@@ -41,6 +42,8 @@
   int tn, th, tw;
   int tiles_img, tiles_h, tiles_w, tiles_n;
   int units;
+  int tiles_m;
+  int pair_units;
   const float *bias;
   const __nv_bfloat16 *res_hi, *res_lo; long long res_ld;
   __nv_bfloat16 *out_hi, *out_lo; long long out_ld;
@@ -101,6 +104,23 @@
 __device__ __forceinline__ void prefetch_tmap(const CUtensorMap *tm) {
   asm volatile("prefetch.tensormap [%0];" ::"l"(reinterpret_cast<uint64_t>(tm)) : "memory");
 }
+__device__ __forceinline__ void tma_load_2d_pair(uint32_t dst, const CUtensorMap *tm, uint32_t bar, int c0, int c1) {
+  asm volatile(
+      "cp.async.bulk.tensor.2d.shared::cluster.global.mbarrier::complete_tx::bytes.multicast::cluster [%0], [%1, {%3, %4}], [%2], %5;"
+      ::"r"(dst), "l"(reinterpret_cast<uint64_t>(tm)), "r"(bar), "r"(c0), "r"(c1), "h"((uint16_t)0x3) : "memory");
+}
+__device__ __forceinline__ uint32_t cluster_ctarank() { uint32_t r; asm volatile("mov.u32 %0, %%cluster_ctarank;" : "=r"(r)); return r; }
+__device__ __forceinline__ uint32_t cluster_id_x() { uint32_t r; asm volatile("mov.u32 %0, %%clusterid.x;" : "=r"(r)); return r; }
+__device__ __forceinline__ uint32_t cluster_count_x() { uint32_t r; asm volatile("mov.u32 %0, %%nclusterid.x;" : "=r"(r)); return r; }
+__device__ __forceinline__ uint32_t mapa_shared(uint32_t addr, uint32_t rank) {
+  uint32_t r; asm volatile("mapa.shared::cluster.u32 %0, %1, %2;" : "=r"(r) : "r"(addr), "r"(rank)); return r;
+}
+__device__ __forceinline__ void mbar_arrive_cluster(uint32_t cluster_bar) {
+  asm volatile("mbarrier.arrive.shared::cluster.b64 _, [%0];" ::"r"(cluster_bar) : "memory");
+}
+__device__ __forceinline__ void cluster_sync_all() {
+  asm volatile("barrier.cluster.arrive.release;\n\tbarrier.cluster.wait.acquire;" ::: "memory");
+}
 
 __device__ __forceinline__ uint64_t make_smem_desc(uint32_t saddr) {
   uint64_t d = 0;
@@ -138,7 +158,7 @@
 }
 
 struct UnitPos { int nt, twi, thi, tni, split; };
-__device__ __forceinline__ UnitPos unit_pos(const TcParams &p, int unit) {
+__host__ __device__ __forceinline__ UnitPos unit_pos(const TcParams &p, int unit) {
   UnitPos u;
   const int tile = unit / p.splitk;
   u.split = unit - tile * p.splitk;
@@ -146,6 +166,13 @@
   const int mt = tile / p.tiles_n;
   u.twi = mt % p.tiles_w; u.thi = (mt / p.tiles_w) % p.tiles_h; u.tni = mt / (p.tiles_w * p.tiles_h);
   return u;
+}
+__host__ __device__ __forceinline__ int pair_unit(int w, int rank, int tiles_n, int tiles_m) {
+  const int mt = 2 * (w / tiles_n) + rank;
+  return mt < tiles_m ? mt * tiles_n + w % tiles_n : -1;
+}
+__host__ __device__ constexpr int stage_tx_bytes(int BN, OperandScheme ops, bool has_tile) {
+  return stage_bytes(BN, ops) - (has_tile ? 0 : a_planes(ops) * a_tile_bytes(BN, ops));
 }
 __device__ __forceinline__ long long row_pixel(const TcParams &p, const UnitPos &u, int row, bool &ok, int *whn = nullptr) {
   const int lw = __ffs(p.tw) - 1, lh = __ffs(p.th) - 1;
@@ -295,7 +322,7 @@
   }
 }
 
-template <int BN, OperandScheme OPS = OperandScheme::BF16X3>
+template <int BN, OperandScheme OPS = OperandScheme::BF16X3, bool PAIR = false>
 __global__ void __launch_bounds__(TC_THREADS, 1)
 conv_gemm_tc_kernel(const __grid_constant__ CUtensorMap tmA_hi, const __grid_constant__ CUtensorMap tmA_lo,
                     const __grid_constant__ CUtensorMap tmB_hi, const __grid_constant__ CUtensorMap tmB_lo,
@@ -322,10 +349,11 @@
     tl_min_stamp(p.tl_min, 0);
     if (a_planes(OPS) == 1) { prefetch_tmap(&tmA_hi); prefetch_tmap(&tmB_hi); }
     else { prefetch_tmap(&tmA_hi); prefetch_tmap(&tmA_lo); prefetch_tmap(&tmB_hi); prefetch_tmap(&tmB_lo); }
-    for (int s = 0; s < S; ++s) { mbar_init(full_bar(s), 1); mbar_init(empty_bar(s), CONS_THREADS / 32); }
+    for (int s = 0; s < S; ++s) { mbar_init(full_bar(s), 1); mbar_init(empty_bar(s), (PAIR ? 2 : 1) * (CONS_THREADS / 32)); }
     asm volatile("fence.mbarrier_init.release.cluster;" ::: "memory");
   }
   __syncthreads();
+  if constexpr (PAIR) cluster_sync_all();
   asm volatile("griddepcontrol.wait;" ::: "memory");
   asm volatile("griddepcontrol.launch_dependents;" ::: "memory");
   if (tid == 0) tl_min_stamp(p.tl_min, 1);
@@ -334,8 +362,12 @@
     asm volatile("setmaxnreg.dec.sync.aligned.u32 24;" ::: "memory");
     if (tid == 0) {
       int it = 0;
-      for (int unit = (int)blockIdx.x; unit < p.units; unit += (int)gridDim.x) {
-        const UnitPos u = unit_pos(p, unit);
+      const int rank = PAIR ? (int)cluster_ctarank() : 0;
+      for (int w = PAIR ? (int)cluster_id_x() : (int)blockIdx.x; w < (PAIR ? p.pair_units : p.units);
+           w += PAIR ? (int)cluster_count_x() : (int)gridDim.x) {
+        const int unit = PAIR ? pair_unit(w, rank, p.tiles_n, p.tiles_m) : w;
+        const bool has_tile = unit >= 0;
+        const UnitPos u = unit_pos(p, has_tile ? unit : w % p.tiles_n);
         const int kb0 = u.split * p.kb_per_split, kb1 = min(num_kb, kb0 + p.kb_per_split);
         const int w_in0 = u.twi * p.tw * p.stride - p.pad, h_in0 = u.thi * p.th * p.stride - p.pad, n0 = u.tni * p.tn;
         const int b_row0 = u.nt * BN;
@@ -348,85 +380,108 @@
             const int ka = cb * BK + h * stage_k(BN, OPS), kk = kb * BK + h * stage_k(BN, OPS);
             mbar_wait(empty_bar(s), ph ^ 1u);
             const uint32_t sa = smem_base + (uint32_t)s * STAGE;
-            mbar_expect_tx(full_bar(s), (uint32_t)STAGE);
-            tma_load_4d(sa, &tmA_hi, full_bar(s), ka, w_in0 + kwi, h_in0 + khi, n0);
-            if (a_planes(OPS) == 2) tma_load_4d(sa + A_TILE, &tmA_lo, full_bar(s), ka, w_in0 + kwi, h_in0 + khi, n0);
-            tma_load_2d(sa + B_OFF, &tmB_hi, full_bar(s), kk, b_row0);
-            if (b_planes(OPS) == 2) tma_load_2d(sa + B_OFF + B_TILE_BYTES, &tmB_lo, full_bar(s), kk, b_row0);
+            mbar_expect_tx(full_bar(s), (uint32_t)stage_tx_bytes(BN, OPS, has_tile));
+            if (has_tile) {
+              tma_load_4d(sa, &tmA_hi, full_bar(s), ka, w_in0 + kwi, h_in0 + khi, n0);
+              if (a_planes(OPS) == 2) tma_load_4d(sa + A_TILE, &tmA_lo, full_bar(s), ka, w_in0 + kwi, h_in0 + khi, n0);
+            }
+            if constexpr (PAIR) {
+              const uint32_t half = (uint32_t)rank * (B_TILE_BYTES / 2);
+              tma_load_2d_pair(sa + B_OFF + half, &tmB_hi, full_bar(s), kk, b_row0 + rank * (BN / 2));
+              if (b_planes(OPS) == 2) tma_load_2d_pair(sa + B_OFF + B_TILE_BYTES + half, &tmB_lo, full_bar(s), kk, b_row0 + rank * (BN / 2));
+            } else {
+              tma_load_2d(sa + B_OFF, &tmB_hi, full_bar(s), kk, b_row0);
+              if (b_planes(OPS) == 2) tma_load_2d(sa + B_OFF + B_TILE_BYTES, &tmB_lo, full_bar(s), kk, b_row0);
+            }
           }
         }
       }
     }
-    return;
-  }
-
-  asm volatile("setmaxnreg.inc.sync.aligned.u32 240;" ::: "memory");
-  const int e = tid - 128;
-  const int g = e >> 7, wq = (e >> 5) & 3;
-  const uint32_t so = smem_base + (uint32_t)(S * STAGE + (e >> 5) * EPI_WARP_BYTES);
-  int it = 0;
-  for (int unit = (int)blockIdx.x; unit < p.units; unit += (int)gridDim.x) {
-    const UnitPos u = unit_pos(p, unit);
-    const int kb0 = u.split * p.kb_per_split, kb1 = min(num_kb, kb0 + p.kb_per_split);
-    float acc[BN / 2];
-#pragma unroll
-    for (int i = 0; i < BN / 2; ++i) acc[i] = 0.f;
-    if constexpr (OPS == OperandScheme::FP8X1) {
-      float part[BN / 2];
-#pragma unroll
-      for (int i = 0; i < BN / 2; ++i) part[i] = 0.f;
-      for (int kb = kb0; kb < kb1; ++kb, ++it) {
-        const int s = it % S; const uint32_t ph = (uint32_t)(it / S) & 1u;
-        mbar_wait(full_bar(s), ph);
-        if (it == 0 && e == 0) tl_min_stamp(p.tl_min, 2);
-        const uint32_t sa = smem_base + (uint32_t)s * STAGE;
-        const uint64_t a8 = make_smem_desc_64b(sa + (uint32_t)g * (A_TILE / 2));
-        const uint64_t b8 = make_smem_desc_64b(sa + B_OFF);
-#pragma unroll
-        for (int k = 0; k < BK / 32; ++k) {
-          wgmma_fence_acc(part);
+  } else {
+    asm volatile("setmaxnreg.inc.sync.aligned.u32 240;" ::: "memory");
+    const int e = tid - 128;
+    const int g = e >> 7, wq = (e >> 5) & 3;
+    const uint32_t so = smem_base + (uint32_t)(S * STAGE + (e >> 5) * EPI_WARP_BYTES);
+    auto release = [&](int s) {
+      if (lane == 0) {
+        mbar_arrive(empty_bar(s));
+        if constexpr (PAIR) mbar_arrive_cluster(mapa_shared(empty_bar(s), cluster_ctarank() ^ 1u));
+      }
+    };
+    int it = 0;
+    for (int w = PAIR ? (int)cluster_id_x() : (int)blockIdx.x; w < (PAIR ? p.pair_units : p.units);
+         w += PAIR ? (int)cluster_count_x() : (int)gridDim.x) {
+      const int unit = PAIR ? pair_unit(w, (int)cluster_ctarank(), p.tiles_n, p.tiles_m) : w;
+      if (PAIR && unit < 0) {
+        for (int i = 0; i < num_kb * KSTEPS; ++i, ++it) {
+          mbar_wait(full_bar(it % S), (uint32_t)(it / S) & 1u);
+          release(it % S);
+        }
+        continue;
+      }
+      const UnitPos u = unit_pos(p, unit);
+      const int kb0 = u.split * p.kb_per_split, kb1 = min(num_kb, kb0 + p.kb_per_split);
+      float acc[BN / 2];
+#pragma unroll
+      for (int i = 0; i < BN / 2; ++i) acc[i] = 0.f;
+      if constexpr (OPS == OperandScheme::FP8X1) {
+        float part[BN / 2];
+#pragma unroll
+        for (int i = 0; i < BN / 2; ++i) part[i] = 0.f;
+        for (int kb = kb0; kb < kb1; ++kb, ++it) {
+          const int s = it % S; const uint32_t ph = (uint32_t)(it / S) & 1u;
+          mbar_wait(full_bar(s), ph);
+          if (it == 0 && e == 0) tl_min_stamp(p.tl_min, 2);
+          const uint32_t sa = smem_base + (uint32_t)s * STAGE;
+          const uint64_t a8 = make_smem_desc_64b(sa + (uint32_t)g * (A_TILE / 2));
+          const uint64_t b8 = make_smem_desc_64b(sa + B_OFF);
+#pragma unroll
+          for (int k = 0; k < BK / 32; ++k) {
+            wgmma_fence_acc(part);
+            wgmma_fence();
+            wgmma_e4m3_nk32<BN>(part, a8 + (uint64_t)(2 * k), b8 + (uint64_t)(2 * k), 0u);
+            wgmma_commit();
+            wgmma_wait<0>();
+            wgmma_fence_acc(part);
+#pragma unroll
+            for (int i = 0; i < BN / 2; ++i) acc[i] += part[i];
+          }
+          release(s);
+        }
+      } else {
+        const int steps = (kb1 - kb0) * KSTEPS;
+        for (int i = 0; i < steps; ++i, ++it) {
+          const int s = it % S; const uint32_t ph = (uint32_t)(it / S) & 1u;
+          mbar_wait(full_bar(s), ph);
+          if (it == 0 && e == 0) tl_min_stamp(p.tl_min, 2);
+          const uint32_t sa = smem_base + (uint32_t)s * STAGE;
+          auto desc = [](uint32_t a) { return row_bytes(BN, OPS) == 64 ? make_smem_desc_64b(a) : make_smem_desc(a); };
+          const uint64_t a_hi = desc(sa + (uint32_t)g * (A_TILE / 2));
+          const uint64_t a_lo = desc(sa + A_TILE + (uint32_t)g * (A_TILE / 2));
+          const uint64_t b_hi = desc(sa + B_OFF);
+          const uint64_t b_lo = desc(sa + B_OFF + B_TILE_BYTES);
+          wgmma_fence_acc(acc);
           wgmma_fence();
-          wgmma_e4m3_nk32<BN>(part, a8 + (uint64_t)(2 * k), b8 + (uint64_t)(2 * k), 0u);
+          mma_kstep<BN, OPS>(acc, a_hi, a_lo, b_hi, b_lo, i == 0);
           wgmma_commit();
-          wgmma_wait<0>();
-          wgmma_fence_acc(part);
-#pragma unroll
-          for (int i = 0; i < BN / 2; ++i) acc[i] += part[i];
+          wgmma_wait<1>();
+          wgmma_fence_acc(acc);
+          if (i > 0) release((it - 1) % S);
         }
-        if (lane == 0) mbar_arrive(empty_bar(s));
-      }
-    } else {
-      const int steps = (kb1 - kb0) * KSTEPS;
-      for (int i = 0; i < steps; ++i, ++it) {
-        const int s = it % S; const uint32_t ph = (uint32_t)(it / S) & 1u;
-        mbar_wait(full_bar(s), ph);
-        if (it == 0 && e == 0) tl_min_stamp(p.tl_min, 2);
-        const uint32_t sa = smem_base + (uint32_t)s * STAGE;
-        auto desc = [](uint32_t a) { return row_bytes(BN, OPS) == 64 ? make_smem_desc_64b(a) : make_smem_desc(a); };
-        const uint64_t a_hi = desc(sa + (uint32_t)g * (A_TILE / 2));
-        const uint64_t a_lo = desc(sa + A_TILE + (uint32_t)g * (A_TILE / 2));
-        const uint64_t b_hi = desc(sa + B_OFF);
-        const uint64_t b_lo = desc(sa + B_OFF + B_TILE_BYTES);
+        wgmma_wait<0>();
         wgmma_fence_acc(acc);
-        wgmma_fence();
-        mma_kstep<BN, OPS>(acc, a_hi, a_lo, b_hi, b_lo, i == 0);
-        wgmma_commit();
-        wgmma_wait<1>();
-        wgmma_fence_acc(acc);
-        if (i > 0 && lane == 0) mbar_arrive(empty_bar((it - 1) % S));
-      }
-      wgmma_wait<0>();
-      wgmma_fence_acc(acc);
-      if (lane == 0) mbar_arrive(empty_bar((it - 1) % S));
-    }
-    if (e == 0) tl_max_stamp(p.tl_max, 0);
-    const uint32_t t_epi = (p.tl_max && e == 0) ? (uint32_t)gtimer() : 0u;
-    tile_epilogue<BN, OPS>(p, u, acc, g, wq, lane, so);
-    if (e == 0) {
-      tl_max_stamp(p.tl_max, 1);
-      if (p.tl_max) atomicAdd(p.tl_max + 3, (unsigned long long)((uint32_t)gtimer() - t_epi));
-    }
-  }
+        release((it - 1) % S);
+      }
+      if (e == 0) tl_max_stamp(p.tl_max, 0);
+      const uint32_t t_epi = (p.tl_max && e == 0) ? (uint32_t)gtimer() : 0u;
+      tile_epilogue<BN, OPS>(p, u, acc, g, wq, lane, so);
+      if (e == 0) {
+        tl_max_stamp(p.tl_max, 1);
+        if (p.tl_max) atomicAdd(p.tl_max + 3, (unsigned long long)((uint32_t)gtimer() - t_epi));
+      }
+    }
+  }
+  if constexpr (PAIR) cluster_sync_all();
 }
 
 
@@ -641,26 +696,48 @@
   constexpr int bslot = BN == 256 ? 2 : (BN == 128 ? 1 : 0);
   constexpr int slot = OPS == OperandScheme::FP16X2 ? 3 : (OPS == OperandScheme::BF16X1 ? 5 + bslot
                                                          : (OPS == OperandScheme::FP8X1 ? 8 + bslot : bslot));
-  if (!ctx->tc_attr_set[slot]) {
-    MPN_CUDA(ctx, cudaFuncSetAttribute(conv_gemm_tc_kernel<BN, OPS>, cudaFuncAttributeMaxDynamicSharedMemorySize, smem));
-    ctx->tc_attr_set[slot] = 1;
-  }
-  const long long units = (long long)pl.tiles_img * pl.tiles_h * pl.tiles_w * pl.tiles_n * pl.splitk;
+  const long long tiles_m = (long long)pl.tiles_img * pl.tiles_h * pl.tiles_w;
+  const long long units = tiles_m * pl.tiles_n * pl.splitk;
   MPN_CHECK_ARG(ctx, units > 0 && units < (1ll << 31), "conv_tc: grid size out of range");
+  MPN_CHECK_ARG(ctx, pl.pair == 1 || (pl.pair == 2 && pl.splitk == 1 && tiles_m >= 2), "conv_tc: CTA pairs need split-K 1 and two M tiles");
+  const bool pair = pl.pair == 2;
+  auto kernel = pair ? conv_gemm_tc_kernel<BN, OPS, true> : conv_gemm_tc_kernel<BN, OPS, false>;
+  uint8_t &attr_set = pair ? ctx->tc_pair_attr_set[slot] : ctx->tc_attr_set[slot];
+  if (!attr_set) {
+    MPN_CUDA(ctx, cudaFuncSetAttribute(kernel, cudaFuncAttributeMaxDynamicSharedMemorySize, smem));
+    attr_set = 1;
+  }
   TcParams tpu = tp;
-  tpu.units = (int)units;
+  tpu.units = (int)units; tpu.tiles_m = (int)tiles_m;
   cudaLaunchConfig_t cfg = {};
-  cfg.gridDim = dim3((unsigned)std::min<long long>(units, ctx->sm_count));
   cfg.blockDim = dim3(TC_THREADS); cfg.dynamicSmemBytes = (size_t)smem; cfg.stream = ctx->stream;
-  cudaLaunchAttribute attr[1];
+  cudaLaunchAttribute attr[2];
   int na = 0;
+  if (pair) {
+    attr[na].id = cudaLaunchAttributeClusterDimension;
+    attr[na].val.clusterDim.x = 2; attr[na].val.clusterDim.y = 1; attr[na].val.clusterDim.z = 1;
+    ++na;
+    if (!ctx->tc_clusters[slot]) {
+      cudaLaunchConfig_t q = cfg;
+      q.gridDim = dim3(2u * (unsigned)ctx->sm_count); q.attrs = attr; q.numAttrs = na;
+      int n = 0;
+      MPN_CUDA(ctx, cudaOccupancyMaxActiveClusters(&n, kernel, &q));
+      MPN_CHECK_ARG(ctx, n > 0, "conv_tc: no CTA pair of the engine fits on an SM pair");
+      ctx->tc_clusters[slot] = n;
+    }
+    const long long pair_units = (tiles_m + 1) / 2 * pl.tiles_n;
+    tpu.pair_units = (int)pair_units;
+    cfg.gridDim = dim3(2u * (unsigned)std::min<long long>(pair_units, ctx->tc_clusters[slot]));
+  } else {
+    cfg.gridDim = dim3((unsigned)std::min<long long>(units, ctx->sm_count));
+  }
   if (tc_use_pdl()) {
     attr[na].id = cudaLaunchAttributeProgrammaticStreamSerialization;
     attr[na].val.programmaticStreamSerializationAllowed = 1;
     ++na;
   }
   cfg.attrs = attr; cfg.numAttrs = na;
-  MPN_CUDA(ctx, cudaLaunchKernelEx(&cfg, conv_gemm_tc_kernel<BN, OPS>, pl.tmA_hi, pl.tmA_lo, pl.tmB_hi, pl.tmB_lo, tpu));
+  MPN_CUDA(ctx, cudaLaunchKernelEx(&cfg, kernel, pl.tmA_hi, pl.tmA_lo, pl.tmB_hi, pl.tmB_lo, tpu));
   MPN_LAUNCHED(ctx);
   return MPN_OK;
 }
@@ -712,7 +789,7 @@
   return 2.0 * (double)p.x.C * p.Cout * p.kh * p.kw * Ho * Wo * (double)p.y.N;
 }
 
-static int conv_tc_plan_impl(mpn_ctx *ctx, int sm_count, const ConvProblem &p, ConvPlan &pl, bool choose_only) {
+static int conv_tc_plan_impl(mpn_ctx *ctx, int sm_count, const ConvProblem &p, ConvPlan &pl, bool choose_only, int force_pair = 0) {
   pl.valid = 0;
   MPN_CHECK_ARG(ctx, choose_only || (p.x.hi && p.x.lo && ((p.w_hi && p.w_lo) || p.w16)), "conv_tc: operands must be split-bf16 (or an fp16 weight plane)");
   MPN_CHECK_ARG(ctx, !(p.w16 && p.bf16), "conv_tc: the bf16 numerics do not take an fp16 weight plane");
@@ -803,10 +880,15 @@
     pl.kb_per_split = (int)((num_kb + pl.splitk - 1) / pl.splitk);
     pl.splitk = (int)((num_kb + pl.kb_per_split - 1) / pl.kb_per_split);
   }
+  pl.pair = (pl.flat && pl.splitk == 1 && tiles_m >= 2) ? 2 : 1;
+  if (force_pair) {
+    MPN_CHECK_ARG(ctx, force_pair == 1 || (force_pair == 2 && pl.splitk == 1 && tiles_m >= 2), "conv_tc: CTA pairs need split-K 1 and two M tiles");
+    pl.pair = force_pair;
+  }
   if (choose_only) return MPN_OK;
   const long long Ktot = (long long)p.kh * p.kw * p.x.C;
   cuuint64_t bd[2] = {(cuuint64_t)Ktot, (cuuint64_t)p.Cout}, bs[1] = {(cuuint64_t)Ktot * 2};
-  cuuint32_t bb[2] = {(cuuint32_t)stage_k(pl.BN, pl.ops), (cuuint32_t)pl.BN}, be[2] = {1, 1};
+  cuuint32_t bb[2] = {(cuuint32_t)stage_k(pl.BN, pl.ops), (cuuint32_t)(pl.BN / pl.pair)}, be[2] = {1, 1};
   if (fp8) {
     const cuuint64_t C8 = (cuuint64_t)p.x.C;
     if (pl.flat) { strides[0] = C8; strides[1] = (cuuint64_t)P * C8; strides[2] = strides[1]; }
@@ -835,6 +917,10 @@
 }
 
 int conv_tc_plan(mpn_ctx *ctx, const ConvProblem &p, ConvPlan &pl) { return conv_tc_plan_impl(ctx, ctx->sm_count, p, pl, false); }
+int conv_tc_plan_pair(mpn_ctx *ctx, const ConvProblem &p, ConvPlan &pl, int pair) {
+  MPN_CHECK_ARG(ctx, pair == 1 || pair == 2, "conv_tc: the pair size is 1 or 2");
+  return conv_tc_plan_impl(ctx, ctx->sm_count, p, pl, false, pair);
+}
 
 int conv_tc_launch(mpn_ctx *ctx, const ConvProblem &p, const ConvPlan &pl) {
   MpnProfScope prof_scope__(ctx, MPN_CAT_CONV_TC);
@@ -905,3 +991,107 @@
   out[0] = pl.mode; out[1] = 1; out[2] = pl.BN; out[3] = pl.splitk; out[4] = 0; out[5] = pl.tn; out[6] = pl.th; out[7] = pl.tw;
   return MPN_OK;
 }
+
+extern "C" int mpn_debug_plan_pair(int64_t N, int64_t Cin, int64_t H, int64_t W, int64_t Cout, int32_t k, int32_t stride, int32_t pad,
+                                   int32_t per_roi, int32_t sm_count, int32_t *out) {
+  int32_t o[8];
+  if (!out) return MPN_ERR_ARG;
+  const int rc = mpn_debug_plan(N, Cin, H, W, Cout, k, stride, pad, per_roi, sm_count, o);
+  if (rc != MPN_OK) return rc;
+  ConvProblem p;
+  p.x.N = N; p.x.H = H; p.x.W = W; p.x.C = Cin; p.x.ld = Cin;
+  p.Cout = (int)Cout; p.kh = p.kw = k; p.stride = stride; p.pad = pad; p.m_invariant = per_roi ? 1 : 0;
+  p.y.N = N; p.y.H = (H + 2 * pad - k) / stride + 1; p.y.W = (W + 2 * pad - k) / stride + 1; p.y.C = Cout; p.y.ld = Cout;
+  ConvPlan pl;
+  MPN_TRY(conv_tc_plan_impl(nullptr, sm_count, p, pl, true));
+  out[0] = pl.pair;
+  return MPN_OK;
+}
+
+namespace {
+template <int BN, OperandScheme OPS>
+void pair_schedule_model(const ConvPlan &pl, int num_kb, int clusters, int64_t *out) {
+  constexpr int S = num_stages(BN, OPS), KSTEPS = kb_steps(BN, OPS);
+  constexpr int A_BYTES = a_planes(OPS) * a_tile_bytes(BN, OPS);
+  constexpr int B_HALF_BYTES = b_planes(OPS) * (BN / 2) * row_bytes(BN, OPS);
+  TcParams p;
+  memset(&p, 0, sizeof p);
+  p.tiles_img = pl.tiles_img; p.tiles_h = pl.tiles_h; p.tiles_w = pl.tiles_w; p.tiles_n = pl.tiles_n;
+  p.splitk = pl.splitk; p.kb_per_split = pl.kb_per_split;
+  const int tiles_m = pl.tiles_img * pl.tiles_h * pl.tiles_w;
+  p.units = tiles_m * pl.tiles_n;
+  const int pair_units = (tiles_m + 1) / 2 * pl.tiles_n;
+  std::vector<int> covered((size_t)p.units, 0);
+  int64_t seq_bad = 0, tx_bad = 0, rel_bad = 0, steps_max = 0, idle = 0;
+  for (int c = 0; c < clusters; ++c) {
+    std::vector<long long> seq[2]; std::vector<char> tile[2];
+    int cons_steps[2] = {0, 0};
+    for (int rank = 0; rank < 2; ++rank) {
+      for (int w = c; w < pair_units; w += clusters) {
+        const int unit = pair_unit(w, rank, p.tiles_n, tiles_m);
+        const UnitPos u = unit_pos(p, unit >= 0 ? unit : w % p.tiles_n);
+        const int kb0 = u.split * p.kb_per_split, kb1 = std::min(num_kb, kb0 + p.kb_per_split);
+        if (unit >= 0) ++covered[(size_t)unit]; else ++idle;
+        for (int kb = kb0; kb < kb1; ++kb)
+          for (int h = 0; h < KSTEPS; ++h) { seq[rank].push_back(((long long)w * num_kb + kb) * KSTEPS + h); tile[rank].push_back(unit >= 0); }
+        cons_steps[rank] += unit >= 0 ? (kb1 - kb0) * KSTEPS : num_kb * KSTEPS;
+      }
+    }
+    if (seq[0] != seq[1]) ++seq_bad;
+    const size_t n = std::min(seq[0].size(), seq[1].size());
+    steps_max = std::max<int64_t>(steps_max, (int64_t)n);
+    for (size_t i = 0; i < n; ++i)
+      for (int d = 0; d < 2; ++d) {
+        const int landed = (tile[d][i] ? A_BYTES : 0) + 2 * B_HALF_BYTES;
+        if (landed != stage_tx_bytes(BN, OPS, tile[d][i] != 0)) ++tx_bad;
+      }
+    std::vector<int> rel[2];
+    for (int d = 0; d < 2; ++d) rel[d].assign((size_t)std::max(cons_steps[0], cons_steps[1]) + 1, 0);
+    for (int r = 0; r < 2; ++r)
+      for (int it = 0; it < cons_steps[r]; ++it)
+        for (int d = 0; d < 2; ++d) rel[d][(size_t)it] += CONS_THREADS / 32;
+    for (int d = 0; d < 2; ++d) {
+      if (cons_steps[d] != (int)seq[d].size()) ++rel_bad;
+      for (int it = 0; it < (int)seq[d].size(); ++it) if (rel[d][(size_t)it] != 2 * (CONS_THREADS / 32)) ++rel_bad;
+    }
+    (void)S;
+  }
+  int64_t cover_bad = 0;
+  for (int v : covered) if (v != 1) ++cover_bad;
+  out[0] = pair_units; out[1] = steps_max; out[2] = seq_bad; out[3] = tx_bad; out[4] = rel_bad; out[5] = cover_bad; out[6] = idle;
+  out[7] = S;
+}
+}
+
+extern "C" int mpn_debug_pair_schedule(int64_t N, int64_t Cin, int64_t H, int64_t W, int64_t Cout, int32_t k, int32_t stride,
+                                       int32_t pad, int32_t per_roi, int32_t sm_count, int32_t scheme, int32_t clusters, int64_t *out) {
+  if (!out || clusters < 1 || scheme < 0 || scheme > 3 || N <= 0 || Cin <= 0 || Cin % 64 || H <= 0 || W <= 0 || Cout <= 0 || k <= 0 ||
+      stride < 1 || stride > 2 || pad < 0 || sm_count < 2)
+    return MPN_ERR_ARG;
+  ConvProblem p;
+  p.x.N = N; p.x.H = H; p.x.W = W; p.x.C = Cin; p.x.ld = Cin;
+  p.Cout = (int)Cout; p.kh = p.kw = k; p.stride = stride; p.pad = pad; p.m_invariant = per_roi ? 1 : 0;
+  p.y.N = N; p.y.H = (H + 2 * pad - k) / stride + 1; p.y.W = (W + 2 * pad - k) / stride + 1; p.y.C = Cout; p.y.ld = Cout;
+  if (p.y.H <= 0 || p.y.W <= 0) return MPN_ERR_ARG;
+  static const char w16_tag = 0;
+  if (scheme == 1) { p.w16 = &w16_tag; p.x.fmt = 1; }
+  p.bf16 = scheme == 2; p.fp8 = scheme == 3;
+  ConvPlan pl;
+  const int rc = conv_tc_plan_impl(nullptr, sm_count, p, pl, true);
+  if (rc != MPN_OK) return rc;
+  if (pl.splitk != 1 || (long long)pl.tiles_img * pl.tiles_h * pl.tiles_w < 2 || (scheme == 1 && pl.BN != 256)) return MPN_ERR_ARG;
+  const int num_kb = k * k * (int)(Cin / BK);
+  switch ((int)pl.ops * 4 + pl.BN / 64) {
+    case 0 * 4 + 1: pair_schedule_model<64, OperandScheme::BF16X3>(pl, num_kb, clusters, out); break;
+    case 0 * 4 + 2: pair_schedule_model<128, OperandScheme::BF16X3>(pl, num_kb, clusters, out); break;
+    case 0 * 4 + 4: pair_schedule_model<256, OperandScheme::BF16X3>(pl, num_kb, clusters, out); break;
+    case 1 * 4 + 4: pair_schedule_model<256, OperandScheme::FP16X2>(pl, num_kb, clusters, out); break;
+    case 2 * 4 + 1: pair_schedule_model<64, OperandScheme::BF16X1>(pl, num_kb, clusters, out); break;
+    case 2 * 4 + 2: pair_schedule_model<128, OperandScheme::BF16X1>(pl, num_kb, clusters, out); break;
+    case 2 * 4 + 4: pair_schedule_model<256, OperandScheme::BF16X1>(pl, num_kb, clusters, out); break;
+    case 3 * 4 + 1: pair_schedule_model<64, OperandScheme::FP8X1>(pl, num_kb, clusters, out); break;
+    case 3 * 4 + 2: pair_schedule_model<128, OperandScheme::FP8X1>(pl, num_kb, clusters, out); break;
+    default: return MPN_ERR_ARG;
+  }
+  return MPN_OK;
+}
```

New measurement: 420,700, median of 6. 1.02x the previous value.
